# zcablii/SM3Det

Hardware: NVIDIA H100
Metric: backbone images/sec @1024^2 (fwd+bwd) (higher is better)
Workload: dtype f32 (bf16 hi+lo split operands on wgmma, fp32 accumulate; SIMT fp32 elsewhere)

## Files before the change

### include/sm3det_b200.h

```cpp
#ifndef SM3DET_B200_H_
#define SM3DET_B200_H_

#include <stddef.h>
#include <stdint.h>

#ifdef __cplusplus
extern "C" {
#endif

#define SM3_ABI_VERSION 1

#define SM3_OK 0
#define SM3_ERR_INVALID_ARG (-1)
#define SM3_ERR_UNSUPPORTED_SHAPE (-2)
#define SM3_ERR_CUDA (-3)
#define SM3_ERR_WORKSPACE (-4)

int sm3_abi_version(void);
const char* sm3_last_error(void);
int sm3_device_supported(void);

enum { SM3_SCHED_DENSE = 0, SM3_SCHED_GROUPED = 1, SM3_SCHED_SPLITK = 2 };
enum {
  SM3_EPI_BIAS = 1,
  SM3_EPI_GELU = 2,
  SM3_EPI_DGELU = 4,
  SM3_EPI_COLSCALE = 8,
  SM3_EPI_ROWSCALE = 16,
  SM3_EPI_RESID = 32,
  SM3_EPI_ATOMIC = 64,
  SM3_EPI_AUXSTORE = 128,
  SM3_EPI_COLSUM = 256
};
typedef struct sm3_gemm_args {
  const float* A; int64_t a_stride_mn, a_stride_k;
  const float* B; int64_t b_stride_mn, b_stride_k, b_group_stride;
  const int32_t* a_row_index;
  const int32_t* b_k_index;
  const uint16_t* b_packed;
  int64_t b_packed_group_stride;
  const uint16_t* a_packed;
  int32_t M, N, K;
  int32_t tile_n;
  int32_t sched;
  int32_t k_splits, num_groups;
  const int32_t* tile_group;
  const int32_t* num_m_tiles;
  const int32_t* seg_begin;
  const int32_t* seg_end;
  float* D; int64_t ldd, d_group_stride;
  const float* bias; int64_t bias_group_stride;
  int32_t epilogue;
  float* aux_out; const float* aux_in; int64_t ld_aux;
  const float* col_scale; const float* row_scale;
  const float* resid; int64_t ld_resid;
  float* colsum; int64_t colsum_group_stride;
  int32_t mma_passes;
} sm3_gemm_args;
int sm3_gemm(const sm3_gemm_args* args, void* stream);
int64_t sm3_gemm_packed_elems(int32_t N, int32_t K);
int sm3_gemm_pack_b(const float* B, int64_t stride_mn, int64_t stride_k, int64_t group_stride, int32_t groups,
                    int32_t N, int32_t K, uint16_t* out, void* stream);
int64_t sm3_gemm_packed_act_elems(int64_t rows, int32_t cols, int32_t mn_major, int32_t tile);
int sm3_gemm_pack_act(const float* X, int64_t ld, const int32_t* row_index, int64_t rows, int32_t cols,
                      int32_t mn_major, int32_t tile, uint16_t* out, void* stream);
int32_t sm3_gemm_tile_n(int32_t N);
int sm3_gemm_pack_b_tile(const float* B, int64_t stride_mn, int64_t stride_k, int64_t group_stride, int32_t groups,
                         int32_t N, int32_t K, int32_t tile, uint16_t* out, void* stream);
size_t sm3_gemm_workspace_bytes(const sm3_gemm_args* args);

typedef struct sm3_ffn_args {
  const uint16_t* a1; const uint16_t* a2;
  const uint16_t* wa1; const uint16_t* wa2; const uint16_t* wb;
  const float* bias1;
  const float* bias2;
  const float* col_scale;
  const float* row_scale;
  const float* resid;
  float* out;
  float* aux_out;
  float* h_out;
  int32_t M, C, H4, chunk, mma_passes, mode;
  uint16_t* dh_mn; uint16_t* act_mn;
  float* db1;
  const float* h_in;
} sm3_ffn_args;
int32_t sm3_ffn_fused_chunk(int32_t mode, int32_t C);
int sm3_ffn_fused(const sm3_ffn_args* args, void* stream);
size_t sm3_ffn_fused_workspace_bytes(const sm3_ffn_args* args);

enum { SM3_LN_NHWC = 0, SM3_LN_PATCH2 = 1, SM3_LN_NCHW = 2 };
int sm3_layernorm_fwd(const float* x, const float* weight, const float* bias, float* y, float* stats,
                      int64_t tokens, int32_t C, float eps, int32_t out_mode, int32_t H, int32_t W, void* stream);
int sm3_layernorm_fwd_img(const float* x, const float* weight, const float* bias, uint16_t* img, float* y, float* stats,
                          int64_t T, int32_t C, float eps, void* stream);
int sm3_layernorm_bwd(const float* dy, const float* x, const float* stats, const float* weight, float* dx,
                      float* dweight, float* dbias, int64_t tokens, int32_t C, int32_t in_mode, int32_t H,
                      int32_t W, int32_t dx_accumulate, void* stream);

int sm3_stem_fwd(const float* x_nchw, const float* weight_t, const float* bias, const float* ln_weight,
                 const float* ln_bias, float* y, float* conv_out, float* stats, int32_t N, int32_t Cin,
                 int32_t H, int32_t W, int32_t ps, int32_t C0, float eps, void* stream);
int sm3_stem_wgrad(const float* x_nchw, const float* dconv, float* dweight_t, float* dbias, int32_t N,
                   int32_t Cin, int32_t H, int32_t W, int32_t ps, int32_t C0, void* stream);

int sm3_dwconv7_fwd(const float* x, const float* weight_t, const float* bias, const float* resid, float* y,
                    int32_t N, int32_t H, int32_t W, int32_t C, void* stream);
int sm3_dwconv7_wgrad(const float* x, const float* dy, float* dweight_t, float* dbias, int32_t N, int32_t H,
                      int32_t W, int32_t C, void* stream);
int sm3_dwconv7_ln_fwd(const float* x, const float* weight_t, const float* bias, const float* ln_weight,
                       const float* ln_bias, float* u, float* stats, float* v, uint16_t* img, int32_t N, int32_t H,
                       int32_t W, int32_t C, float eps, void* stream);

typedef struct sm3_router_args {
  const float* v; const float* proj_weight; const float* proj_bias; const float* sim_matrix;
  const float* temperature; const float* w_noise; const float* noise;
  int32_t T, C, P, E, k;
  int32_t* top_idx; float* top_gate; float* logits; float* top_vals; float* p_out;
  float* sigma; int32_t* top_idx_m;
  float* partials;
} sm3_router_args;
int sm3_moe_router_blocks(int32_t T);
int sm3_moe_router(const sm3_router_args* args, void* stream);
size_t sm3_moe_router_workspace_bytes(const sm3_router_args* args);

typedef struct sm3_plan_args {
  const float* partials; int32_t T, E, k, max_m_tiles;
  float* importance; float* load; float* loss;
  int32_t* counts; int32_t* seg_begin; int32_t* seg_end; int32_t* cursor;
  int32_t* tile_group; int32_t* num_m_tiles;
} sm3_plan_args;
int sm3_moe_plan(const sm3_plan_args* args, void* stream);
size_t sm3_moe_plan_workspace_bytes(const sm3_plan_args* args);
int sm3_moe_assign(const int32_t* top_idx, int32_t T, int32_t k, int32_t E, const int32_t* seg_begin,
                   int32_t* cursor, int32_t* slot_of, int32_t* pair_token, void* stream);
int sm3_moe_combine(const float* expert_out, const int32_t* slot_of, const int32_t* top_idx, const float* gate,
                    const float* gamma, const float* resid, const float* row_scale, float* out, float* y_opt,
                    int32_t T, int32_t C, int32_t k, void* stream);

typedef struct sm3_act_pack_args {
  const float* h; const float* da; int64_t R; int32_t W; int32_t mode;
  const int32_t* live_tiles; const int32_t* tile_group;
  float* out_f32; uint16_t* pack_k; uint16_t* pack_mn; int32_t mn_tile; float* colsum;
  uint16_t* pack_mn2; int32_t mn_tile2;
} sm3_act_pack_args;
int sm3_act_pack(const sm3_act_pack_args* args, void* stream);

int sm3_moe_combine_bwd(const float* dout, const float* expert_out, const int32_t* slot_of, const int32_t* top_idx,
                        const float* gate, const float* gamma, const float* row_scale, float* d_expert_out,
                        float* dgate, float* dgamma, int32_t T, int32_t C, int32_t k, void* stream);
typedef struct sm3_router_bwd_args {
  const float* p; const float* sim_matrix; const float* temperature;
  const int32_t* top_idx; const float* top_gate; const float* dgate; const float* logits;
  const float* importance; const float* loss_scale;
  int32_t T, P, E, k;
  float* dp; float* dsim_hat; float* dtemperature;
  const float* noise; const float* sigma; const float* top_vals; const int32_t* top_idx_m; const float* load;
  float* dr;
} sm3_router_bwd_args;
int sm3_moe_router_bwd(const sm3_router_bwd_args* args, void* stream);
int sm3_moe_router_bwd_finalize(const float* dsim_hat, const float* sim_matrix, float* dsim, int32_t P, int32_t E,
                                void* stream);
int sm3_colsum(const float* a, const float* b, const float* row_scale, const int32_t* seg_begin,
               const int32_t* seg_end, int32_t groups, float* out, int64_t rows, int32_t C, void* stream);
int sm3_gather_sum(const float* src, const int32_t* slot_of, const float* add, float* out, int32_t T, int32_t C,
                   int32_t k, void* stream);
int sm3_scale_rows(const float* x, const float* row_scale, const float* col_scale, float* out, int64_t rows,
                   int32_t C, void* stream);

int sm3_gather_rows_peer(const float* const* bases, const int32_t* const* token_lists, const int32_t* src_rank,
                         const int32_t* src_row, const float* scale, float* out, int64_t rows, int32_t C, void* stream);

typedef struct sm3_ep_plan_args {
  const int32_t* allm; const int32_t* tile_group_s; const int32_t* num_tiles_s; const int32_t* pair_token;
  int32_t W, me, E, R_s, cap;
  int32_t* src_rank; int32_t* src_slot; int32_t* tile_group; int32_t* num_tiles; int32_t* seg_begin; int32_t* seg_end;
  int32_t* comb_rank; int32_t* comb_row; int32_t* overflow;
} sm3_ep_plan_args;
int sm3_ep_plan(const sm3_ep_plan_args* args, void* stream);

int sm3_dwconv_fwd(const float* x, const float* weight_t, const float* bias, const float* resid, float* y, int32_t N,
                   int32_t H, int32_t W, int32_t C, int32_t ks, int32_t dil, void* stream);
int sm3_dwconv_wgrad(const float* x, const float* dy, float* dweight_t, float* dbias, int32_t N, int32_t H, int32_t W,
                     int32_t C, int32_t ks, int32_t dil, void* stream);
int sm3_colstat(const float* x, const float* sh1, const float* y, const float* sh2, const float* sc2, float* s1, float* s2,
                int64_t rows, int32_t C, void* stream);
int sm3_affine(const float* x1, const float* a1, const float* x2, const float* a2, const float* b, const float* add,
               float* out, int64_t rows, int32_t C, void* stream);
int sm3_mul(const float* a, const float* b, const float* add, float* out, int64_t n, void* stream);
int sm3_dropout(const float* x, float* out, int64_t n, float p, uint64_t seed, void* stream);
int sm3_dropout_dev(const float* x, float* out, int64_t n, float p, const uint64_t* seed_dev, void* stream);
int sm3_mlp_mid_fwd(const float* h, const float* weight_t, const float* bias, const float* mask, float* a, int32_t N,
                    int32_t H, int32_t W, int32_t C, float p, uint64_t seed, const uint64_t* seed_dev, void* stream);
int sm3_mlp_mid_bwd(const float* h, const float* weight_t, const float* bias, const float* da, const float* mask, float* dh,
                    float* dweight_t, float* dbias, int32_t N, int32_t H, int32_t W, int32_t C, float p, uint64_t seed,
                    const uint64_t* seed_dev, void* stream);
int sm3_lsk_agg(const float* a1, const float* a2, float* agg, int32_t* amax, int64_t T, int32_t Ch, void* stream);
int sm3_conv7_c2(const float* x, const float* w, const float* b, float* y, int32_t N, int32_t H, int32_t W, int32_t act,
                 void* stream);
int sm3_conv7_c2_wgrad(const float* x, const float* dpre, float* dw, float* db, int32_t N, int32_t H, int32_t W, void* stream);
int sm3_lsk_mix(const float* a1, const float* a2, const float* sig, float* out, int64_t T, int32_t Ch, void* stream);
int sm3_lsk_mix_bwd_sig(const float* dout, const float* a1, const float* a2, const float* sig, float* dpre, int64_t T,
                        int32_t Ch, void* stream);
int sm3_lsk_mix_bwd_in(const float* dout, const float* sig, const float* dagg, const int32_t* amax, float* da1, float* da2,
                       int64_t T, int32_t Ch, void* stream);
int sm3_im2col(const float* x, float* col, int32_t N, int32_t H, int32_t W, int32_t Cin, int32_t ks, int32_t stride,
               int32_t pad, int32_t Kp, int32_t nchw, void* stream);
int sm3_col2im(const float* dcol, float* dx, int32_t N, int32_t H, int32_t W, int32_t Cin, int32_t ks, int32_t stride,
               int32_t pad, int32_t Kp, int32_t nchw, void* stream);

// ... 11 lines not shown
```

### sm3det_b200/_lib.py

```python
import ctypes as C
import os
import threading

_LIB_PATH = os.path.join(os.path.dirname(os.path.abspath(__file__)), 'lib', 'libsm3det_b200.so')
_lock = threading.Lock()
_lib = None
LAUNCHES = 0

c_f32p = C.c_void_p
c_i32p = C.c_void_p
c_stream = C.c_void_p


class GemmArgs(C.Structure):
    _fields_ = [
        ('A', c_f32p), ('a_stride_mn', C.c_int64), ('a_stride_k', C.c_int64),
        ('B', c_f32p), ('b_stride_mn', C.c_int64), ('b_stride_k', C.c_int64), ('b_group_stride', C.c_int64),
        ('a_row_index', c_i32p), ('b_k_index', c_i32p), ('b_packed', C.c_void_p), ('b_packed_group_stride', C.c_int64), ('a_packed', C.c_void_p),
        ('M', C.c_int32), ('N', C.c_int32), ('K', C.c_int32),
        ('tile_n', C.c_int32), ('sched', C.c_int32), ('k_splits', C.c_int32), ('num_groups', C.c_int32),
        ('tile_group', c_i32p), ('num_m_tiles', c_i32p), ('seg_begin', c_i32p), ('seg_end', c_i32p),
        ('D', c_f32p), ('ldd', C.c_int64), ('d_group_stride', C.c_int64),
        ('bias', c_f32p), ('bias_group_stride', C.c_int64),
        ('epilogue', C.c_int32),
        ('aux_out', c_f32p), ('aux_in', c_f32p), ('ld_aux', C.c_int64),
        ('col_scale', c_f32p), ('row_scale', c_f32p),
        ('resid', c_f32p), ('ld_resid', C.c_int64),
        ('colsum', c_f32p), ('colsum_group_stride', C.c_int64),
        ('mma_passes', C.c_int32),
    ]


class RouterArgs(C.Structure):
    _fields_ = [
        ('v', c_f32p), ('proj_weight', c_f32p), ('proj_bias', c_f32p), ('sim_matrix', c_f32p),
        ('temperature', c_f32p), ('w_noise', c_f32p), ('noise', c_f32p),
        ('T', C.c_int32), ('C', C.c_int32), ('P', C.c_int32), ('E', C.c_int32), ('k', C.c_int32),
        ('top_idx', c_i32p), ('top_gate', c_f32p), ('logits', c_f32p), ('top_vals', c_f32p), ('p_out', c_f32p),
        ('sigma', c_f32p), ('top_idx_m', c_i32p),
        ('partials', c_f32p),
    ]


class PlanArgs(C.Structure):
    _fields_ = [
        ('partials', c_f32p), ('T', C.c_int32), ('E', C.c_int32), ('k', C.c_int32), ('max_m_tiles', C.c_int32),
        ('importance', c_f32p), ('load', c_f32p), ('loss', c_f32p),
        ('counts', c_i32p), ('seg_begin', c_i32p), ('seg_end', c_i32p), ('cursor', c_i32p),
        ('tile_group', c_i32p), ('num_m_tiles', c_i32p),
    ]


class FfnArgs(C.Structure):
    _fields_ = [
        ('a1', C.c_void_p), ('a2', C.c_void_p), ('wa1', C.c_void_p), ('wa2', C.c_void_p), ('wb', C.c_void_p),
        ('bias1', c_f32p), ('bias2', c_f32p), ('col_scale', c_f32p), ('row_scale', c_f32p), ('resid', c_f32p),
        ('out', c_f32p), ('aux_out', c_f32p), ('h_out', c_f32p),
        ('M', C.c_int32), ('C', C.c_int32), ('H4', C.c_int32), ('chunk', C.c_int32), ('mma_passes', C.c_int32),
        ('mode', C.c_int32),
        ('dh_mn', C.c_void_p), ('act_mn', C.c_void_p), ('db1', c_f32p), ('h_in', c_f32p),
    ]


class EpPlanArgs(C.Structure):
    _fields_ = [
        ('allm', c_i32p), ('tile_group_s', c_i32p), ('num_tiles_s', c_i32p), ('pair_token', c_i32p),
        ('W', C.c_int32), ('me', C.c_int32), ('E', C.c_int32), ('R_s', C.c_int32), ('cap', C.c_int32),
        ('src_rank', c_i32p), ('src_slot', c_i32p), ('tile_group', c_i32p), ('num_tiles', c_i32p),
        ('seg_begin', c_i32p), ('seg_end', c_i32p), ('comb_rank', c_i32p), ('comb_row', c_i32p), ('overflow', c_i32p),
    ]


_I32, _I64, _F32, _P = C.c_int32, C.c_int64, C.c_float, C.c_void_p
SIGNATURES = {
    'sm3_abi_version': [],
    'sm3_last_error': [],
    'sm3_device_supported': [],
    'sm3_gemm': [C.POINTER(GemmArgs), _P],
    'sm3_gemm_packed_elems': [_I32, _I32],
    'sm3_gemm_pack_b': [_P, _I64, _I64, _I64, _I32, _I32, _I32, _P, _P],
    'sm3_gemm_packed_act_elems': [_I64, _I32, _I32, _I32],
    'sm3_gemm_pack_act': [_P, _I64, _P, _I64, _I32, _I32, _I32, _P, _P],
    'sm3_gemm_tile_n': [_I32],
    'sm3_gemm_pack_b_tile': [_P, _I64, _I64, _I64, _I32, _I32, _I32, _I32, _P, _P],
    'sm3_gemm_workspace_bytes': [C.POINTER(GemmArgs)],
    'sm3_ffn_fused_chunk': [_I32, _I32],
    'sm3_ffn_fused': [C.POINTER(FfnArgs), _P],
    'sm3_ffn_fused_workspace_bytes': [C.POINTER(FfnArgs)],
    'sm3_moe_router_workspace_bytes': [C.POINTER(RouterArgs)],
    'sm3_moe_plan_workspace_bytes': [C.POINTER(PlanArgs)],
    'sm3_layernorm_fwd': [_P, _P, _P, _P, _P, _I64, _I32, _F32, _I32, _I32, _I32, _P],
    'sm3_layernorm_fwd_img': [_P, _P, _P, _P, _P, _P, _I64, _I32, _F32, _P],
    'sm3_layernorm_bwd': [_P, _P, _P, _P, _P, _P, _P, _I64, _I32, _I32, _I32, _I32, _I32, _P],
    'sm3_stem_fwd': [_P, _P, _P, _P, _P, _P, _P, _P, _I32, _I32, _I32, _I32, _I32, _I32, _F32, _P],
    'sm3_stem_wgrad': [_P, _P, _P, _P, _I32, _I32, _I32, _I32, _I32, _I32, _P],
    'sm3_dwconv7_fwd': [_P, _P, _P, _P, _P, _I32, _I32, _I32, _I32, _P],
    'sm3_dwconv7_wgrad': [_P, _P, _P, _P, _I32, _I32, _I32, _I32, _P],
    'sm3_dwconv7_ln_fwd': [_P, _P, _P, _P, _P, _P, _P, _P, _P, _I32, _I32, _I32, _I32, _F32, _P],
    'sm3_moe_router_bwd_finalize': [_P, _P, _P, _I32, _I32, _P],
    'sm3_moe_router_blocks': [_I32],
    'sm3_moe_router': [C.POINTER(RouterArgs), _P],
    'sm3_moe_plan': [C.POINTER(PlanArgs), _P],
    'sm3_moe_assign': [_P, _I32, _I32, _I32, _P, _P, _P, _P, _P],
    'sm3_moe_combine': [_P, _P, _P, _P, _P, _P, _P, _P, _P, _I32, _I32, _I32, _P],
    'sm3_moe_combine_bwd': [_P, _P, _P, _P, _P, _P, _P, _P, _P, _P, _I32, _I32, _I32, _P],
    'sm3_colsum': [_P, _P, _P, _P, _P, _I32, _P, _I64, _I32, _P],
    'sm3_gather_sum': [_P, _P, _P, _P, _I32, _I32, _I32, _P],
    'sm3_scale_rows': [_P, _P, _P, _P, _I64, _I32, _P],
    'sm3_moe_router_bwd': [_P, _P],
    'sm3_ep_plan': [C.POINTER(EpPlanArgs), _P],
    'sm3_gather_rows_peer': [_P, _P, _P, _P, _P, _P, _I64, _I32, _P],
    'sm3_upsample_add': [_P, _P, _P, _I32, _I32, _I32, _I32, _I32, _I32, _P],
    'sm3_upsample_add_bwd': [_P, _P, _I32, _I32, _I32, _I32, _I32, _I32, _P],
    'sm3_transpose_batched': [_P, _P, _I32, _I32, _I32, _P],
    'sm3_dwconv_fwd': [_P, _P, _P, _P, _P, _I32, _I32, _I32, _I32, _I32, _I32, _P],
    'sm3_dwconv_wgrad': [_P, _P, _P, _P, _I32, _I32, _I32, _I32, _I32, _I32, _P],
    'sm3_colstat': [_P, _P, _P, _P, _P, _P, _P, _I64, _I32, _P],
    'sm3_affine': [_P, _P, _P, _P, _P, _P, _P, _I64, _I32, _P],
    'sm3_mul': [_P, _P, _P, _P, _I64, _P],
    'sm3_dropout': [_P, _P, _I64, _F32, C.c_uint64, _P],
    'sm3_dropout_dev': [_P, _P, _I64, _F32, _P, _P],
    'sm3_mlp_mid_fwd': [_P, _P, _P, _P, _P, _I32, _I32, _I32, _I32, _F32, C.c_uint64, _P, _P],
    'sm3_mlp_mid_bwd': [_P, _P, _P, _P, _P, _P, _P, _P, _I32, _I32, _I32, _I32, _F32, C.c_uint64, _P, _P],
    'sm3_lsk_agg': [_P, _P, _P, _P, _I64, _I32, _P],
    'sm3_conv7_c2': [_P, _P, _P, _P, _I32, _I32, _I32, _I32, _P],
    'sm3_conv7_c2_wgrad': [_P, _P, _P, _P, _I32, _I32, _I32, _P],
    'sm3_lsk_mix': [_P, _P, _P, _P, _I64, _I32, _P],
    'sm3_lsk_mix_bwd_sig': [_P, _P, _P, _P, _P, _I64, _I32, _P],
    'sm3_lsk_mix_bwd_in': [_P, _P, _P, _P, _P, _P, _I64, _I32, _P],
    'sm3_im2col': [_P, _P, _I32, _I32, _I32, _I32, _I32, _I32, _I32, _I32, _I32, _P],
    'sm3_col2im': [_P, _P, _I32, _I32, _I32, _I32, _I32, _I32, _I32, _I32, _I32, _P],
}
_RESTYPES = {'sm3_last_error': C.c_char_p, 'sm3_gemm_packed_elems': C.c_int64, 'sm3_gemm_packed_act_elems': C.c_int64,
             'sm3_gemm_workspace_bytes': C.c_size_t, 'sm3_ffn_fused_workspace_bytes': C.c_size_t,
             'sm3_moe_router_workspace_bytes': C.c_size_t, 'sm3_moe_plan_workspace_bytes': C.c_size_t}


class ActPackArgs(C.Structure):
    _fields_ = [
        ('h', c_f32p), ('da', c_f32p), ('R', C.c_int64), ('W', C.c_int32), ('mode', C.c_int32),
        ('live_tiles', c_i32p), ('tile_group', c_i32p),
        ('out_f32', c_f32p), ('pack_k', C.c_void_p), ('pack_mn', C.c_void_p), ('mn_tile', C.c_int32), ('colsum', c_f32p),
        ('pack_mn2', C.c_void_p), ('mn_tile2', C.c_int32),
    ]


class RouterBwdArgs(C.Structure):
    _fields_ = [
        ('p', c_f32p), ('sim_matrix', c_f32p), ('temperature', c_f32p),
        ('top_idx', c_i32p), ('top_gate', c_f32p), ('dgate', c_f32p), ('logits', c_f32p),
        ('importance', c_f32p), ('loss_scale', c_f32p),
        ('T', C.c_int32), ('P', C.c_int32), ('E', C.c_int32), ('k', C.c_int32),
        ('dp', c_f32p), ('dsim_hat', c_f32p), ('dtemperature', c_f32p),
        ('noise', c_f32p), ('sigma', c_f32p), ('top_vals', c_f32p), ('top_idx_m', c_i32p), ('load', c_f32p),
        ('dr', c_f32p),
    ]


SIGNATURES['sm3_moe_router_bwd'] = [C.POINTER(RouterBwdArgs), _P]
SIGNATURES['sm3_act_pack'] = [C.POINTER(ActPackArgs), _P]


def library_path() -> str:
    return _LIB_PATH


def load():
    global _lib
    if _lib is not None:
        return _lib
    with _lock:
        if _lib is not None:
            return _lib
        if not os.path.isfile(_LIB_PATH):
            raise RuntimeError(
                f'sm3det_b200: CUDA library not built ({_LIB_PATH} missing). Run `make` at the repo root or '
                f'`python -c "import __graft_entry__ as g; g.build()"`. There is no CPU/PyTorch fallback.')
        lib = C.CDLL(_LIB_PATH)
        for name, argtypes in SIGNATURES.items():
            fn = getattr(lib, name)
            fn.argtypes = argtypes
            fn.restype = _RESTYPES.get(name, C.c_int)
# ... 13 lines not shown
```

### sm3det_b200/csrc/capi.cu

```cuda
#include "../../include/sm3det_b200.h"
#include "common.cuh"
#include "gemm_tc.cuh"
#include "kernels.h"
#include "ffn_fused.cuh"

using namespace sm3;

static inline cudaStream_t S(void* s) { return reinterpret_cast<cudaStream_t>(s); }

extern "C" {

int sm3_abi_version(void) { return SM3_ABI_VERSION; }
const char* sm3_last_error(void) { return sm3::last_error(); }

int sm3_device_supported(void) {
  int dev = 0, major = 0, minor = 0;
  if (cudaGetDevice(&dev) != cudaSuccess) return 0;
  if (cudaDeviceGetAttribute(&major, cudaDevAttrComputeCapabilityMajor, dev) != cudaSuccess) return 0;
  if (cudaDeviceGetAttribute(&minor, cudaDevAttrComputeCapabilityMinor, dev) != cudaSuccess) return 0;
  return (major == 9 && minor == 0) ? 1 : 0;
}

int sm3_gemm(const sm3_gemm_args* a, void* stream) {
  if (!a) { set_last_error("sm3_gemm: null args"); return SM3_ERR_INVALID_ARG; }
  gemm::Params p{};
  p.A = a->A; p.a_smn = a->a_stride_mn; p.a_sk = a->a_stride_k;
  p.B = a->B; p.b_smn = a->b_stride_mn; p.b_sk = a->b_stride_k; p.b_group_stride = a->b_group_stride;
  p.a_row_index = a->a_row_index; p.b_k_index = a->b_k_index;
  p.b_packed = a->b_packed; p.b_packed_group_stride = a->b_packed_group_stride; p.a_packed = a->a_packed;
  p.M = a->M; p.N = a->N; p.K = a->K; p.BN = a->tile_n;
  p.sched = a->sched; p.k_splits = a->k_splits; p.num_groups = a->num_groups;
  p.tile_group = a->tile_group; p.num_m_tiles_dev = a->num_m_tiles;
  p.seg_begin = a->seg_begin; p.seg_end = a->seg_end;
  p.D = a->D; p.ldd = a->ldd; p.d_group_stride = a->d_group_stride;
  p.bias = a->bias; p.bias_group_stride = a->bias_group_stride;
  p.epi = a->epilogue;
  p.aux_out = a->aux_out; p.aux_in = a->aux_in; p.ld_aux = a->ld_aux;
  p.col_scale = a->col_scale; p.row_scale = a->row_scale;
  p.resid = a->resid; p.ld_resid = a->ld_resid;
  p.colsum = a->colsum; p.colsum_group_stride = a->colsum_group_stride;
  p.passes = (a->mma_passes == 1) ? 1 : 3;
  return gemm::launch(p, S(stream));
}

int64_t sm3_gemm_packed_elems(int32_t N, int32_t K) { return gemm::packed_elems(N, K); }
int sm3_gemm_pack_b(const float* B, int64_t s_mn, int64_t s_k, int64_t group_stride, int32_t groups, int32_t N, int32_t K,
                    uint16_t* out, void* stream) {
  return gemm::pack_b(B, s_mn, s_k, group_stride, groups, N, K, out, S(stream));
}

int64_t sm3_gemm_packed_act_elems(int64_t rows, int32_t cols, int32_t mn_major, int32_t tile) {
  return gemm::packed_act_elems(rows, cols, mn_major, tile);
}
int sm3_gemm_pack_act(const float* X, int64_t ld, const int32_t* row_index, int64_t rows, int32_t cols, int32_t mn_major,
                      int32_t tile, uint16_t* out, void* stream) {
  return gemm::pack_act(X, ld, row_index, rows, cols, mn_major, tile, out, S(stream));
}
int32_t sm3_gemm_tile_n(int32_t N) { return gemm::pick_bn(N); }
int sm3_gemm_pack_b_tile(const float* B, int64_t s_mn, int64_t s_k, int64_t group_stride, int32_t groups, int32_t N, int32_t K,
                         int32_t tile, uint16_t* out, void* stream) {
  return gemm::pack_b(B, s_mn, s_k, group_stride, groups, N, K, out, S(stream), tile);
}
size_t sm3_gemm_workspace_bytes(const sm3_gemm_args*) { return 0; }

int32_t sm3_ffn_fused_chunk(int32_t mode, int32_t C) { return (mode >= 0 && mode <= 3) ? ffn::chain_chunk(mode, C) : 0; }
size_t sm3_ffn_fused_workspace_bytes(const sm3_ffn_args*) { return 0; }
int sm3_ffn_fused(const sm3_ffn_args* a, void* stream) {
  if (!a) { set_last_error("sm3_ffn_fused: null args"); return SM3_ERR_INVALID_ARG; }
  ffn::ChainParams p{};
  p.a1 = a->a1; p.a2 = a->a2; p.wa1 = a->wa1; p.wa2 = a->wa2; p.wb = a->wb;
  p.bias1 = a->bias1; p.bias2 = a->bias2; p.col_scale = a->col_scale; p.row_scale = a->row_scale; p.resid = a->resid;
  p.out = a->out; p.aux_out = a->aux_out; p.h_out = a->h_out;
  p.dh_mn = a->dh_mn; p.act_mn = a->act_mn; p.db1 = a->db1; p.h_in = a->h_in;
  p.M = a->M; p.C = a->C; p.H4 = a->H4; p.HC = a->chunk; p.passes = a->mma_passes; p.mode = a->mode;
  return ffn::chain(p, S(stream));
}

int sm3_layernorm_fwd(const float* x, const float* w, const float* b, float* y, float* stats, int64_t T, int32_t C,
                      float eps, int32_t out_mode, int32_t H, int32_t W, void* stream) {
  return layernorm_fwd(x, w, b, y, stats, T, C, eps, out_mode, H, W, S(stream));
}
int sm3_layernorm_fwd_img(const float* x, const float* w, const float* b, uint16_t* img, float* y, float* stats, int64_t T,
                          int32_t C, float eps, void* stream) {
  return layernorm_fwd_img(x, w, b, img, y, stats, T, C, eps, S(stream));
}
int sm3_layernorm_bwd(const float* dy, const float* x, const float* stats, const float* w, float* dx, float* dw,
                      float* db, int64_t T, int32_t C, int32_t in_mode, int32_t H, int32_t W, int32_t dx_accum,
                      void* stream) {
  return layernorm_bwd(dy, x, stats, w, dx, dw, db, T, C, in_mode, H, W, dx_accum, S(stream));
}
int sm3_stem_fwd(const float* x, const float* wt, const float* bias, const float* lnw, const float* lnb, float* y,
                 float* conv_out, float* stats, int32_t N, int32_t Cin, int32_t H, int32_t W, int32_t ps, int32_t C0,
                 float eps, void* stream) {
  return stem_fwd(x, wt, bias, lnw, lnb, y, conv_out, stats, N, Cin, H, W, ps, C0, eps, S(stream));
}
int sm3_stem_wgrad(const float* x, const float* du, float* dwt, float* dbias, int32_t N, int32_t Cin, int32_t H,
                   int32_t W, int32_t ps, int32_t C0, void* stream) {
  return stem_wgrad(x, du, dwt, dbias, N, Cin, H, W, ps, C0, S(stream));
}
int sm3_dwconv7_fwd(const float* x, const float* wt, const float* bias, const float* resid, float* y, int32_t N,
                    int32_t H, int32_t W, int32_t C, void* stream) {
  return dwconv7_fwd(x, wt, bias, resid, y, N, H, W, C, S(stream));
}
int sm3_dwconv7_wgrad(const float* x, const float* dy, float* dwt, float* dbias, int32_t N, int32_t H, int32_t W,
                      int32_t C, void* stream) {
  return dwconv7_wgrad(x, dy, dwt, dbias, N, H, W, C, S(stream));
}
int sm3_dwconv7_ln_fwd(const float* x, const float* wt, const float* bias, const float* lnw, const float* lnb, float* u,
                       float* stats, float* v, uint16_t* img, int32_t N, int32_t H, int32_t W, int32_t C, float eps,
                       void* stream) {
  return dwconv7_ln_fwd(x, wt, bias, lnw, lnb, u, stats, v, img, N, H, W, C, eps, S(stream));
}

int sm3_moe_router_blocks(int32_t T) { return router_blocks(T); }
int sm3_moe_router(const sm3_router_args* a, void* stream) {
  if (!a) { set_last_error("sm3_moe_router: null args"); return SM3_ERR_INVALID_ARG; }
  RouterArgs r{};
  r.v = a->v; r.wp = a->proj_weight; r.bp = a->proj_bias; r.sim = a->sim_matrix; r.temperature = a->temperature;
  r.w_noise = a->w_noise; r.noise = a->noise;
  r.T = a->T; r.C = a->C; r.P = a->P; r.E = a->E; r.k = a->k;
  r.top_idx = a->top_idx; r.top_gate = a->top_gate; r.logits = a->logits; r.top_vals = a->top_vals; r.p_out = a->p_out; r.sigma = a->sigma; r.top_idx_m = a->top_idx_m;
  r.partials = a->partials; r.nblocks = router_blocks(a->T);
  return moe_router(r, S(stream));
}
size_t sm3_moe_router_workspace_bytes(const sm3_router_args* a) {
  return a ? (size_t)router_blocks(a->T) * 3u * (size_t)a->E * sizeof(float) : 0;
}
size_t sm3_moe_plan_workspace_bytes(const sm3_plan_args* a) {
  return a ? (size_t)(2 * a->E + 1) * sizeof(float) + (size_t)(4 * a->E + a->max_m_tiles + 1) * sizeof(int32_t) : 0;
}
int sm3_moe_plan(const sm3_plan_args* a, void* stream) {
  if (!a) { set_last_error("sm3_moe_plan: null args"); return SM3_ERR_INVALID_ARG; }
  PlanArgs p{};
  p.partials = a->partials; p.nblocks = router_blocks(a->T);
  p.T = a->T; p.E = a->E; p.k = a->k; p.max_m_tiles = a->max_m_tiles;
  p.importance = a->importance; p.load = a->load; p.loss = a->loss;
  p.counts = a->counts; p.seg_begin = a->seg_begin; p.seg_end = a->seg_end; p.cursor = a->cursor;
  p.tile_group = a->tile_group; p.num_m_tiles = a->num_m_tiles;
  return moe_plan(p, S(stream));
}
int sm3_moe_assign(const int32_t* top_idx, int32_t T, int32_t k, int32_t E, const int32_t* seg_begin, int32_t* cursor,
                   int32_t* slot_of, int32_t* pair_token, void* stream) {
  return moe_assign(top_idx, T, k, E, seg_begin, cursor, slot_of, pair_token, S(stream));
}
int sm3_moe_combine(const float* o, const int32_t* slot_of, const int32_t* top_idx, const float* gate,
                    const float* gamma, const float* resid, const float* row_scale, float* out, float* y_opt,
                    int32_t T, int32_t C, int32_t k, void* stream) {
  return moe_combine(o, slot_of, top_idx, gate, gamma, resid, row_scale, out, y_opt, T, C, k, S(stream));
}

int sm3_act_pack(const sm3_act_pack_args* a, void* stream) {
  if (!a) { set_last_error("sm3_act_pack: null args"); return SM3_ERR_INVALID_ARG; }
  ActPackArgs r{};
  r.h = a->h; r.da = a->da; r.R = a->R; r.W = a->W; r.mode = a->mode; r.live_tiles = a->live_tiles; r.tile_group = a->tile_group;
  r.out_f32 = a->out_f32; r.pack_k = a->pack_k; r.pack_mn = a->pack_mn; r.mn_tile = a->mn_tile; r.colsum = a->colsum;
  r.pack_mn2 = a->pack_mn2; r.mn_tile2 = a->mn_tile2;
  return act_pack(r, S(stream));
}
int sm3_moe_combine_bwd(const float* dout, const float* o, const int32_t* slot_of, const int32_t* top_idx,
                        const float* gate, const float* gamma, const float* row_scale, float* d_o, float* dgate,
                        float* dgamma, int32_t T, int32_t C, int32_t k, void* stream) {
  return moe_combine_bwd(dout, o, slot_of, top_idx, gate, gamma, row_scale, d_o, dgate, dgamma, T, C, k, S(stream));
}
int sm3_moe_router_bwd(const sm3_router_bwd_args* a, void* stream) {
  if (!a) { set_last_error("sm3_moe_router_bwd: null args"); return SM3_ERR_INVALID_ARG; }
  RouterBwdArgs r{};
  r.p = a->p; r.sim = a->sim_matrix; r.temperature = a->temperature; r.top_idx = a->top_idx; r.top_gate = a->top_gate;
  r.dgate = a->dgate; r.logits = a->logits; r.importance = a->importance; r.loss_scale = a->loss_scale;
  r.T = a->T; r.P = a->P; r.E = a->E; r.k = a->k; r.dp = a->dp; r.dsim_hat = a->dsim_hat; r.dtemperature = a->dtemperature;
  r.noise = a->noise; r.sigma = a->sigma; r.top_vals = a->top_vals; r.top_idx_m = a->top_idx_m; r.load = a->load; r.dr = a->dr;
  return moe_router_bwd(r, S(stream));
}
int sm3_moe_router_bwd_finalize(const float* dsim_hat, const float* sim, float* dsim, int32_t P, int32_t E, void* stream) {
  return moe_router_bwd_finalize(dsim_hat, sim, dsim, P, E, S(stream));
}
int sm3_colsum(const float* a, const float* b, const float* rs, const int32_t* seg_begin, const int32_t* seg_end,
               int32_t G, float* out, int64_t rows, int32_t C, void* stream) {
  return colsum(a, b, rs, seg_begin, seg_end, G, out, rows, C, S(stream));
}
int sm3_gather_sum(const float* src, const int32_t* slot_of, const float* add, float* out, int32_t T, int32_t C,
                   int32_t k, void* stream) {
  return gather_sum(src, slot_of, add, out, T, C, k, S(stream));
}
int sm3_scale_rows(const float* x, const float* rs, const float* cs, float* out, int64_t rows, int32_t C, void* stream) {
  return scale_rows(x, rs, cs, out, rows, C, S(stream));
}

int sm3_gather_rows_peer(const float* const* bases, const int32_t* const* token_lists, const int32_t* src_rank,
                         const int32_t* src_row, const float* scale, float* out, int64_t rows, int32_t C, void* stream) {
  return gather_rows_peer(bases, reinterpret_cast<const int* const*>(token_lists), src_rank, src_row, scale, out, rows, C, S(stream));
}
int sm3_dwconv_fwd(const float* x, const float* wt, const float* bias, const float* resid, float* y, int32_t N, int32_t H,
                   int32_t W, int32_t C, int32_t ks, int32_t dil, void* stream) {
// ... 88 lines not shown
```

### sm3det_b200/csrc/ffn_fused.cu

```cuda
#define SM3_GEMM_KERNEL_IMPL
#include "gemm_tc.cuh"
#include "ffn_fused.cuh"
#include "kernels.h"

namespace sm3 {
namespace ffn {
using namespace gemm;

constexpr int THREADS = 384;
constexpr int W_PROD_A = 0, W_PROD_B = 1, EPI0 = 4, NE = 8;
constexpr int CONS_REGS = 232, PROD_REGS = 40;
constexpr uint32_t SMEM_LIMIT = 232448u - 1024u;
constexpr uint32_t STAGING = NE * EPI_STAGE_BYTES;
constexpr uint32_t BARS = 256;

struct Layout {
  uint32_t a, ones, a2, wa, wb, act, act2, stage, cs, bar, total;
  uint32_t a_tile, wa_chunk, wa_stage, wb_stage, act_bytes;
  int sa, sb;
};

struct ChainK { ChainParams p; Layout L; int m_tiles, nch; };

__device__ __forceinline__ void bulk_g2s(uint32_t dst, const void* src, uint32_t bytes, uint32_t bar) {
// ... 48 lines not shown
  auto wa_empty = [&](int s) { return bar + 32u + 8u * s; };
  auto wb_full = [&](int s) { return bar + 48u + 8u * s; };
  auto wb_empty = [&](int s) { return bar + 64u + 8u * s; };
  const int warp = threadIdx.x >> 5, lane = threadIdx.x & 31;
  constexpr int NA = (MODE == 1 || MODE == 2) ? 2 : 1;
  constexpr bool WGRAD_IMG = MODE >= 2;

  if (threadIdx.x == 0) {
    mbar_init(a_full, 1); mbar_init(a_empty, NE);
    for (int s = 0; s < 2; ++s) { mbar_init(wa_full(s), 1); mbar_init(wa_empty(s), NE); mbar_init(wb_full(s), 1); mbar_init(wb_empty(s), NE); }
    asm volatile("fence.mbarrier_init.release.cluster;" ::: "memory");
  }
  __syncthreads();
  const int nch = k.nch;
  constexpr int kbc = C / 32;

  if (warp < EPI0) {
    asm volatile("setmaxnreg.dec.sync.aligned.u32 %0;" ::"n"(PROD_REGS));
    if (warp == W_PROD_A && lane == 0) {
      uint32_t n_t = 0, n_w = 0;
      for (int t = blockIdx.x; t < k.m_tiles; t += gridDim.x, ++n_t) {
        mbar_wait(a_empty, (n_t & 1u) ^ 1u);
        if ((p.debug & 8) && n_t > 0) { mbar_arrive(a_full); goto weights; }
        expect_tx(a_full, NA * L.a_tile);
        bulk_g2s(sb0 + L.a, reinterpret_cast<const uint8_t*>(MODE == 3 ? p.a2 : p.a1) + (long long)t * L.a_tile, L.a_tile, a_full);
        if (NA == 2) bulk_g2s(sb0 + L.a + L.a_tile, reinterpret_cast<const uint8_t*>(p.a2) + (long long)t * L.a_tile, L.a_tile, a_full);
      weights:
        for (int j = 0; j < nch; ++j, ++n_w) {
          const int s = n_w % L.sa;
          mbar_wait(wa_empty(s), ((n_w / L.sa) & 1u) ^ 1u);
          if ((p.debug & 4) && n_w >= (uint32_t)L.sa) { mbar_arrive(wa_full(s)); continue; }
          expect_tx(wa_full(s), L.wa_stage);
          const uint32_t dst = sb0 + L.wa + s * L.wa_stage;
          bulk_g2s(dst, reinterpret_cast<const uint8_t*>(MODE == 3 ? p.wa2 : p.wa1) + (long long)j * L.wa_chunk, L.wa_chunk, wa_full(s));
          if (NA == 2) bulk_g2s(dst + L.wa_chunk, reinterpret_cast<const uint8_t*>(p.wa2) + (long long)j * L.wa_chunk, L.wa_chunk, wa_full(s));
        }
      }
    } else if (warp == W_PROD_B && lane == 0) {
      uint32_t n = 0;
      for (int t = blockIdx.x; t < k.m_tiles; t += gridDim.x) {
        for (int j = 0; j < nch; ++j, ++n) {
          const int s = n % L.sb;
          mbar_wait(wb_empty(s), ((n / L.sb) & 1u) ^ 1u);
          if ((p.debug & 4) && n >= (uint32_t)L.sb) { mbar_arrive(wb_full(s)); continue; }
          expect_tx(wb_full(s), L.wb_stage);
          bulk_g2s(sb0 + L.wb + s * L.wb_stage, reinterpret_cast<const uint8_t*>(p.wb) + (long long)j * L.wb_stage, L.wb_stage, wb_full(s));
        }
      }
    }
  } else {
    asm volatile("setmaxnreg.inc.sync.aligned.u32 %0;" ::"n"(CONS_REGS));
    const int e = warp - EPI0, g = e >> 2, wq = warp & 3;
    const uint32_t slab = (uint32_t)g * WG_A_BYTES;
    const uint32_t stage_base = sb0 + L.stage + (uint32_t)e * EPI_STAGE_BYTES;
    const int rl = lane >> 2, c4 = (lane & 3) * 4;
    const int r_lo = g * 64 + wq * 16 + rl;
    auto wg_bar = [&]() { asm volatile("bar.sync %0, 128;" ::"r"(1 + g) : "memory"); };
    float acc_h[HC / 2], acc_d[HC / 2], acc_o[C / 2];
    uint32_t n_c = 0, n_b = 0, n_t = 0;
    auto gemm_a = [&](uint32_t nc) {
      const int s = nc % L.sa;
      mbar_wait(wa_full(s), (nc / L.sa) & 1u);
      const uint32_t wst = sb0 + L.wa + s * L.wa_stage;
#pragma unroll
      for (int q = 0; q < NA; ++q) {
        uint64_t da = make_smem_desc(sb0 + L.a + q * L.a_tile + slab, false), db = make_smem_desc(wst + q * L.wa_chunk, false);
        for (int kb = 0; kb < kbc; ++kb) {
          if (q == 0 && MODE != 3) {
            mma3<HC>(acc_h, da, da + 512u, db, db + HC * 4u, kb > 0 ? 1u : 0u, p.passes);
            mma3<HC>(acc_h, da + 2u, da + 514u, db + 2u, db + HC * 4u + 2u, 1u, p.passes);
          } else {
            mma3<HC>(acc_d, da, da + 512u, db, db + HC * 4u, kb > 0 ? 1u : 0u, p.passes);
            mma3<HC>(acc_d, da + 2u, da + 514u, db + 2u, db + HC * 4u + 2u, 1u, p.passes);
          }
          da += 1024u; db += HC * 8u;
        }
      }
    };
    const uint32_t cs_base = sb0 + L.cs;
    auto cons_bar = [&]() { asm volatile("bar.sync 3, 256;" ::: "memory"); };
    if constexpr (WGRAD_IMG) {
      for (int i = threadIdx.x - EPI0 * 32; i < p.H4; i += 256) asm volatile("st.shared.f32 [%0], %1;" ::"r"(cs_base + 4u * i), "f"(0.f) : "memory");
      cons_bar();
    }
    const long long R_pad = ((long long)p.M + 31) / 32 * 32;
    for (int t = blockIdx.x; t < k.m_tiles; t += gridDim.x, ++n_t) {
      mbar_wait(a_full, n_t & 1u);
      wg::fence();
      gemm_a(n_c);
      wg::commit();
      for (int j = 0; j < nch; ++j, ++n_c) {
        if constexpr (MODE == 3) {
#pragma unroll
          for (int q = 0; q < HC / 8; ++q)
#pragma unroll
            for (int h = 0; h < 2; ++h) {
              const long long row = (long long)t * 128 + r_lo + 8 * h;
              const float2 x = row < p.M ? __ldg(reinterpret_cast<const float2*>(p.h_in + row * p.H4 + (long long)j * HC + 8 * q + 2 * (lane & 3)))
                                         : make_float2(0.f, 0.f);
              acc_h[4 * q + 2 * h] = x.x; acc_h[4 * q + 2 * h + 1] = x.y;
            }
        }
        wg::wait<0>();
        if constexpr (MODE != 3) wg::fence_operand(acc_h);
        if constexpr (MODE != 0) wg::fence_operand(acc_d);
        __syncwarp();
        if (lane == 0) {
          mbar_arrive(wa_empty(n_c % L.sa));
          if (j > 0) mbar_arrive(wb_empty((n_b - 1) % L.sb));
          if (j == nch - 1) mbar_arrive(a_empty);
        }
        const float* b1 = p.bias1 + (long long)j * HC;
        if constexpr (WGRAD_IMG) {
          const long long wrow0 = (long long)t * 128 + g * 64 + wq * 16;
#pragma unroll
          for (int qp = 0; qp < HC / 16; ++qp) {
            float cs4[4];
#pragma unroll
            for (int qq = 0; qq < 2; ++qq) {
              const int q = 2 * qp + qq;
              const int kk = 8 * q + 2 * (lane & 3);
              const float2 bv = MODE == 3 ? make_float2(0.f, 0.f) : __ldg(reinterpret_cast<const float2*>(b1 + kk));
              cs4[2 * qq] = 0.f; cs4[2 * qq + 1] = 0.f;
#pragma unroll
              for (int h = 0; h < 2; ++h) {
                const int r = r_lo + 8 * h;
                float y[2], a[2];
#pragma unroll
                for (int e = 0; e < 2; ++e) {
                  const float x = MODE == 3 ? acc_h[4 * q + 2 * h + e] : acc_h[4 * q + 2 * h + e] + (e ? bv.y : bv.x);
                  float Phi, ex;
                  phi_parts(x, Phi, ex);
                  a[e] = x * Phi;
                  y[e] = acc_d[4 * q + 2 * h + e] * fmaf(x * 0.39894228040143267794f, ex, Phi);
                }
                if (wrow0 + rl + 8 * h < p.M) { cs4[2 * qq] += y[0]; cs4[2 * qq + 1] += y[1]; }
                uint32_t hi, lo;
                split2(y[0], y[1], hi, lo);
                const uint32_t o = sb0 + L.act + (uint32_t)(kk >> 5) * 16384u + kmajor_sw64_offset((uint32_t)r, (uint32_t)((kk & 31) >> 3)) +
                                   (uint32_t)(kk & 7) * 2u;
                asm volatile("st.shared.b32 [%0], %1;" ::"r"(o), "r"(hi) : "memory");
                asm volatile("st.shared.b32 [%0], %1;" ::"r"(o + 8192u), "r"(lo) : "memory");
                const uint32_t so = stage_base + (uint32_t)((rl + 8 * h) * EPI_STAGE_ROW_FLOATS + 8 * qq + 2 * (lane & 3)) * 4u;
                asm volatile("st.shared.v2.f32 [%0], {%1, %2};" ::"r"(so), "f"(y[0]), "f"(y[1]) : "memory");
                asm volatile("st.shared.v2.f32 [%0], {%1, %2};" ::"r"(so + 16u * EPI_STAGE_ROW_FLOATS * 4u), "f"(a[0]), "f"(a[1]) : "memory");
              }
            }
            const float csum = colsum16(cs4, lane);
            const int col = j * HC + 16 * qp;
            if ((lane & 4) == 0)
              asm volatile("red.shared.add.f32 [%0], %1;" ::"r"(cs_base + 4u * (uint32_t)(col + 8 * ((lane >> 4) & 1) + 2 * (lane & 3) + ((lane >> 3) & 1))),
                           "f"(csum) : "memory");
            __syncwarp();
            const int sr = lane >> 1, sc = 8 * (lane & 1);
            const long long row = wrow0 + sr;
            if (row < R_pad) {
              float dv8[8], av8[8];
              float4 x0, x1, z0, z1;
              const uint32_t ro = stage_base + (uint32_t)(sr * EPI_STAGE_ROW_FLOATS + sc) * 4u;
              asm volatile("ld.shared.v4.f32 {%0, %1, %2, %3}, [%4];" : "=f"(x0.x), "=f"(x0.y), "=f"(x0.z), "=f"(x0.w) : "r"(ro) : "memory");
              asm volatile("ld.shared.v4.f32 {%0, %1, %2, %3}, [%4];" : "=f"(x1.x), "=f"(x1.y), "=f"(x1.z), "=f"(x1.w) : "r"(ro + 16u) : "memory");
              asm volatile("ld.shared.v4.f32 {%0, %1, %2, %3}, [%4];" : "=f"(z0.x), "=f"(z0.y), "=f"(z0.z), "=f"(z0.w)
                           : "r"(ro + 16u * EPI_STAGE_ROW_FLOATS * 4u) : "memory");
              asm volatile("ld.shared.v4.f32 {%0, %1, %2, %3}, [%4];" : "=f"(z1.x), "=f"(z1.y), "=f"(z1.z), "=f"(z1.w)
                           : "r"(ro + 16u * EPI_STAGE_ROW_FLOATS * 4u + 16u) : "memory");
              const bool live = row < p.M;
              dv8[0] = x0.x; dv8[1] = x0.y; dv8[2] = x0.z; dv8[3] = x0.w; dv8[4] = x1.x; dv8[5] = x1.y; dv8[6] = x1.z; dv8[7] = x1.w;
              av8[0] = z0.x; av8[1] = z0.y; av8[2] = z0.z; av8[3] = z0.w; av8[4] = z1.x; av8[5] = z1.y; av8[6] = z1.z; av8[7] = z1.w;
              uint32_t dh_[4], dl_[4], ah_[4], al_[4];
#pragma unroll
              for (int e = 0; e < 4; ++e) {
                split2(live ? dv8[2 * e] : 0.f, live ? dv8[2 * e + 1] : 0.f, dh_[e], dl_[e]);
                split2(live ? av8[2 * e] : 0.f, live ? av8[2 * e + 1] : 0.f, ah_[e], al_[e]);
              }
              constexpr uint32_t PB = 8192u;
              const int n = col + sc;
              const long long blk = ((long long)(n >> 7) * (R_pad >> 5) + (row >> 5)) * (2LL * PB);
              const uint32_t o = mnmajor_sw128_offset((uint32_t)(row & 31), (uint32_t)((n & 127) >> 3));
              uint8_t* dimg = reinterpret_cast<uint8_t*>(p.dh_mn) + blk + o;
              uint8_t* aimg = reinterpret_cast<uint8_t*>(p.act_mn) + blk + o;
              *reinterpret_cast<uint4*>(dimg) = make_uint4(dh_[0], dh_[1], dh_[2], dh_[3]);
              *reinterpret_cast<uint4*>(dimg + PB) = make_uint4(dl_[0], dl_[1], dl_[2], dl_[3]);
              *reinterpret_cast<uint4*>(aimg) = make_uint4(ah_[0], ah_[1], ah_[2], ah_[3]);
              *reinterpret_cast<uint4*>(aimg + PB) = make_uint4(al_[0], al_[1], al_[2], al_[3]);
            }
            __syncwarp();
          }
        } else {
#pragma unroll
          for (int q = 0; q < HC / 8; ++q) {
            const int kk = 8 * q + 2 * (lane & 3);
            const float2 bv = __ldg(reinterpret_cast<const float2*>(b1 + kk));
#pragma unroll
            for (int h = 0; h < 2; ++h) {
              const int r = r_lo + 8 * h;
              const float x0 = acc_h[4 * q + 2 * h] + bv.x, x1 = acc_h[4 * q + 2 * h + 1] + bv.y;
              if (MODE == 0 && p.h_out) {
                const long long row = (long long)t * 128 + r;
                if (row < p.M) *reinterpret_cast<float2*>(p.h_out + row * p.H4 + (long long)j * HC + kk) = make_float2(x0, x1);
              }
              float y0, y1;
              if (p.debug & 1) { y0 = x0; y1 = x1; }
              else if constexpr (MODE == 0) { y0 = gelu_fast(x0); y1 = gelu_fast(x1); }
              else { y0 = acc_d[4 * q + 2 * h] * gelu_grad_fast(x0); y1 = acc_d[4 * q + 2 * h + 1] * gelu_grad_fast(x1); }
              if (p.debug & 2) continue;
              uint32_t hi, lo;
              split2(y0, y1, hi, lo);
              const uint32_t o = sb0 + L.act + (uint32_t)(kk >> 5) * 16384u + kmajor_sw64_offset((uint32_t)r, (uint32_t)((kk & 31) >> 3)) +
                                 (uint32_t)(kk & 7) * 2u;
              asm volatile("st.shared.b32 [%0], %1;" ::"r"(o), "r"(hi) : "memory");
              asm volatile("st.shared.b32 [%0], %1;" ::"r"(o + 8192u), "r"(lo) : "memory");
            }
          }
        }
        fence_proxy_async_smem();
        wg_bar();
        const int s = n_b % L.sb;
        mbar_wait(wb_full(s), (n_b / L.sb) & 1u);
        wg::fence();
        {
          uint64_t da = make_smem_desc(sb0 + L.act + slab, false), db = make_smem_desc(sb0 + L.wb + s * L.wb_stage, false);
          const uint64_t blo = (uint64_t)(C * 4);
#pragma unroll
          for (int kb = 0; kb < HC / 32; ++kb) {
            mma3<C>(acc_o, da, da + 512u, db, db + blo, (j > 0 || kb > 0) ? 1u : 0u, p.passes);
            mma3<C>(acc_o, da + 2u, da + 514u, db + 2u, db + blo + 2u, 1u, p.passes);
            da += 1024u; db += 2u * blo;
          }
        }
        ++n_b;
        if (j + 1 < nch) gemm_a(n_c + 1);
        wg::commit();
      }
      wg::wait<0>();
      wg::fence_operand(acc_o);
      __syncwarp();
      if (lane == 0) mbar_arrive(wb_empty((n_b - 1) % L.sb));
      const long long row0 = (long long)t * 128 + g * 64 + wq * 16;
#pragma unroll
      for (int c = 0; c < C / 16; ++c) {
        const int n = c * 16 + c4;
        float4 rr[2];
#pragma unroll
        for (int it = 0; it < 2; ++it) {
          const long long row = row0 + it * 8 + rl;
          rr[it] = (p.resid && row < p.M) ? ldg_f4(p.resid + row * C + n) : make_float4(0.f, 0.f, 0.f, 0.f);
        }
        __syncwarp();
#pragma unroll
        for (int qq = 0; qq < 2; ++qq)
#pragma unroll
          for (int h = 0; h < 2; ++h)
            asm volatile("st.shared.v2.f32 [%0], {%1, %2};"
                         ::"r"(stage_base + (uint32_t)((rl + 8 * h) * EPI_STAGE_ROW_FLOATS + 8 * qq + 2 * (lane & 3)) * 4u),
                           "f"(acc_o[8 * c + 4 * qq + 2 * h]), "f"(acc_o[8 * c + 4 * qq + 2 * h + 1]) : "memory");
        __syncwarp();
        float4 bv = make_float4(0.f, 0.f, 0.f, 0.f), sv = make_float4(1.f, 1.f, 1.f, 1.f);
        if (p.bias2) bv = ldg_f4(p.bias2 + n);
        if (p.col_scale) sv = ldg_f4(p.col_scale + n);
#pragma unroll
        for (int it = 0; it < 2; ++it) {
          const int rr_ = it * 8 + rl;
          const long long row = row0 + rr_;
          if (row >= p.M) continue;
          float4 x;
          asm volatile("ld.shared.v4.f32 {%0, %1, %2, %3}, [%4];" : "=f"(x.x), "=f"(x.y), "=f"(x.z), "=f"(x.w)
                       : "r"(stage_base + (uint32_t)(rr_ * EPI_STAGE_ROW_FLOATS + c4) * 4u) : "memory");
          x.x += bv.x; x.y += bv.y; x.z += bv.z; x.w += bv.w;
          if (p.aux_out) *reinterpret_cast<float4*>(p.aux_out + row * C + n) = x;
          x.x *= sv.x; x.y *= sv.y; x.z *= sv.z; x.w *= sv.w;
          if (p.row_scale) { const float rs = __ldg(p.row_scale + row); x.x *= rs; x.y *= rs; x.z *= rs; x.w *= rs; }
          x.x += rr[it].x; x.y += rr[it].y; x.z += rr[it].z; x.w += rr[it].w;
          *reinterpret_cast<float4*>(p.out + row * C + n) = x;
        }
      }
    }
    if constexpr (WGRAD_IMG) {
      cons_bar();
      for (int i = threadIdx.x - EPI0 * 32; i < p.H4; i += 256) {
        float v;
        asm volatile("ld.shared.f32 %0, [%1];" : "=f"(v) : "r"(cs_base + 4u * i) : "memory");
        atomicAdd(p.db1 + i, v);
      }
    }
  }
}

static bool chain_layout(int mode, int C, int HC, int sa, int sb, Layout& L) {
  const uint32_t nA = (mode == 1 || mode == 2) ? 2 : 1;
  L.a_tile = (uint32_t)(C / 32) * 16384u;
  L.wa_chunk = (uint32_t)(C / 32) * HC * 128u;
  L.wa_stage = nA * L.wa_chunk;
  L.wb_stage = (uint32_t)(HC / 32) * C * 128u;
  L.act_bytes = (uint32_t)(HC / 32) * 16384u;
  L.sa = sa; L.sb = sb;
  uint32_t o = 0;
  L.a = o; o += nA * L.a_tile;
  L.ones = 0; L.a2 = L.a + L.a_tile;
  L.wa = o; o += sa * L.wa_stage;
  L.wb = o; o += sb * L.wb_stage;
  L.act = o; o += L.act_bytes;
  L.act2 = 0;
  L.stage = o; o += STAGING;
  L.cs = o; o += mode >= 2 ? (uint32_t)(4 * C) * 4u : 0u;
  L.bar = o; o += BARS;
  L.total = o + 1024u;
  return L.total <= SMEM_LIMIT + 1024u;
}

static bool pick_chain(int mode, int C, int HC_req, int& HC, Layout& L) {
  static const int cand[][3] = {{64, 2, 2}, {32, 2, 2}, {64, 2, 1}, {32, 2, 1}, {32, 1, 1}};
  if (C % 32 != 0 || C < 32 || C > 256) return false;
  if ((mode == 2 && C > 128) || (mode == 3 && C != 192)) return false;
  for (auto& c : cand)
    if ((HC_req == 0 || c[0] == HC_req) && chain_layout(mode, C, c[0], c[1], c[2], L)) { HC = c[0]; return true; }
  return false;
}

int chain_chunk(int mode, int C) {
  int HC = 0; Layout L;
  return pick_chain(mode, C, 0, HC, L) ? HC : 0;
}

static bool aligned16(const void* q) { return (reinterpret_cast<uintptr_t>(q) & 15u) == 0; }

int chain(const ChainParams& p, cudaStream_t stream) {
  SM3_REQUIRE(p.mode >= 0 && p.mode <= 3, SM3_ERR_INVALID_ARG, "ffn chain: mode");
  SM3_REQUIRE((p.mode == 3 || (p.a1 && p.wa1)) && p.wb && p.bias1 && p.out && (p.mode == 0 || (p.a2 && p.wa2)), SM3_ERR_INVALID_ARG,
              "ffn chain: null operand");
  SM3_REQUIRE(p.mode < 2 || (p.dh_mn && p.act_mn && p.db1 && (p.mode == 2 || p.h_in)), SM3_ERR_INVALID_ARG,
              "ffn chain: modes 2 / 3 need dh_mn, act_mn, db1 (and h_in in mode 3)");
  SM3_REQUIRE(p.M > 0 && p.H4 > 0 && p.C > 0, SM3_ERR_INVALID_ARG, "ffn chain: bad shape");
  ChainK k{};
  k.p = p;
  int HC = 0;
  SM3_REQUIRE(p.HC == 32 || p.HC == 64, SM3_ERR_INVALID_ARG, "ffn chain: chunk must be 32 or 64 (sm3_ffn_fused_chunk), got %d", p.HC);
  SM3_REQUIRE(pick_chain(p.mode, p.C, p.HC, HC, k.L), SM3_ERR_UNSUPPORTED_SHAPE, "ffn chain: C=%d with chunk %d does not fit shared memory (mode %d)", p.C, p.HC, p.mode);
  SM3_REQUIRE(p.H4 % HC == 0 && p.C % 16 == 0, SM3_ERR_UNSUPPORTED_SHAPE, "ffn chain: H4=%d not a multiple of the chunk %d", p.H4, HC);
// ... 43 lines not shown
```

### sm3det_b200/csrc/gemm_tc.cu

```cuda
#define SM3_GEMM_KERNEL_IMPL
#include "gemm_tc.cuh"
#include <mutex>

namespace sm3 {
const char* last_error();
namespace gemm {

int pick_bn(int N) {
  static const int cand[] = {128, 96, 64, 32};
  for (int bn : cand)
    if (N % bn == 0) return bn;
  if (N <= 0 || N % 8) return 0;
  int best = 0, best_tiles = 0;
  for (int bn : cand) {
    const int tiles = (N + bn - 1) / bn;
    if (!best || tiles < best_tiles || (tiles == best_tiles && tiles * bn < best_tiles * best)) { best = bn; best_tiles = tiles; }
  }
  return best;
}

static bool aligned16(const void* p) { return (reinterpret_cast<uintptr_t>(p) & 15u) == 0; }

long long packed_elems(int N, int K) {
  const long long kblocks = (K + BK - 1) / BK;
// ... 4 lines not shown

__global__ void __launch_bounds__(256) pack_b_kernel(const float* __restrict__ B, long long s_mn, long long s_k,
                                                    long long group_stride, int N, int rows, int K, int BN,
                                                    uint16_t* __restrict__ out, long long out_group_stride,
                                                    long long chunks_per_group) {
  const long long i = (long long)blockIdx.x * blockDim.x + threadIdx.x;
  if (i >= chunks_per_group) return;
  const int g = blockIdx.y;
  const int kblocks = (K + BK - 1) / BK;
  const int n = (int)(i % rows);
  const long long r = i / rows;
  const int c = (int)(r % 4), kb = (int)(r / 4);
  const bool live = n < N;
  const float* src = B + (long long)g * group_stride + (long long)n * s_mn;
  uint32_t hi[4], lo[4];
#pragma unroll
  for (int e = 0; e < 8; e += 2) {
    float v[2];
#pragma unroll
    for (int q = 0; q < 2; ++q) {
      const int k = kb * BK + c * 8 + e + q;
      v[q] = (live && k < K) ? __ldg(src + (long long)k * s_k) : 0.f;
    }
    const uint32_t u0 = __float_as_uint(v[0]), u1 = __float_as_uint(v[1]);
    hi[e / 2] = __byte_perm(u0, u1, 0x7632);
    const uint32_t r0 = __float_as_uint(v[0] - __uint_as_float(u0 & 0xFFFF0000u)) + 0x8000u;
    const uint32_t r1 = __float_as_uint(v[1] - __uint_as_float(u1 & 0xFFFF0000u)) + 0x8000u;
    lo[e / 2] = __byte_perm(r0, r1, 0x7632);
  }
  const int nt = n / BN, row = n % BN;
  uint8_t* tile = reinterpret_cast<uint8_t*>(out + (long long)g * out_group_stride) +
                  ((long long)nt * kblocks + kb) * ((long long)BN * 128);
  const uint32_t o = kmajor_sw64_offset((uint32_t)row, (uint32_t)c);
  *reinterpret_cast<uint4*>(tile + o) = make_uint4(hi[0], hi[1], hi[2], hi[3]);
  *reinterpret_cast<uint4*>(tile + (long long)BN * 64 + o) = make_uint4(lo[0], lo[1], lo[2], lo[3]);
}

int pack_b(const float* B, long long s_mn, long long s_k, long long group_stride, int groups, int N, int K,
           uint16_t* out, cudaStream_t stream, int tile) {
  SM3_REQUIRE(B && out && N > 0 && K > 0 && groups >= 1, SM3_ERR_INVALID_ARG, "gemm pack: bad argument");
  const int BN = tile > 0 ? tile : pick_bn(N);
  SM3_REQUIRE(BN > 0 && BN % 8 == 0 && BN <= 256 && (tile > 0 ? N % BN == 0 : N % 8 == 0), SM3_ERR_UNSUPPORTED_SHAPE,
              "gemm pack: N=%d has no tile width (tile=%d)", N, tile);
  SM3_REQUIRE((reinterpret_cast<uintptr_t>(out) & 15u) == 0, SM3_ERR_INVALID_ARG, "gemm pack: output must be 16B aligned");
  const long long kblocks = (K + BK - 1) / BK;
  const int rows = (N + BN - 1) / BN * BN;
  const long long chunks = (long long)rows * kblocks * 4;
  dim3 grid((unsigned)((chunks + 255) / 256), (unsigned)groups);
  pack_b_kernel<<<grid, 256, 0, stream>>>(B, s_mn, s_k, group_stride, N, rows, K, BN, out, packed_elems(N, K), chunks);
  return check_launch("pack_b_kernel");
}

long long packed_act_elems(long long rows, int cols, int mn_major, int tile) {
  if (!mn_major) {
    const long long rt = (rows + tile - 1) / tile, kb = (cols + BK - 1) / BK;
    return rt * kb * 2 * (long long)tile * BK;
  }
  const long long ct = (cols + tile - 1) / tile, kb = (rows + BK - 1) / BK;
  return ct * kb * 2 * (long long)(plane_bytes(tile, true) / 2);
}

__global__ void __launch_bounds__(256) pack_act_k_kernel(const float* __restrict__ X, long long ld, const int* __restrict__ row_index,
                                                        long long rows, int K, int tile, uint16_t* __restrict__ out,
                                                        long long chunks) {
  const long long i = (long long)blockIdx.x * blockDim.x + threadIdx.x;
  if (i >= chunks) return;
  const int kblocks = (K + BK - 1) / BK;
  const int cpr = kblocks * 4;
  const long long row = i / cpr;
  const int cc = (int)(i % cpr), kb = cc >> 2, c = cc & 3;
  long long src_row = row < rows ? row : -1;
  if (src_row >= 0 && row_index) src_row = __ldg(row_index + row);
  float v[8];
#pragma unroll
  for (int e = 0; e < 8; ++e) v[e] = 0.f;
  if (src_row >= 0) {
    const int k = kb * BK + c * 8;
    const float* src = X + src_row * ld + k;
    if (k + 8 <= K) { const float4 a = ldg_f4(src), b = ldg_f4(src + 4); v[0] = a.x; v[1] = a.y; v[2] = a.z; v[3] = a.w; v[4] = b.x; v[5] = b.y; v[6] = b.z; v[7] = b.w; }
    else { for (int e = 0; e < 8; ++e) if (k + e < K) v[e] = __ldg(src + e); }
  }
  uint32_t hi[4], lo[4];
#pragma unroll
  for (int e = 0; e < 8; e += 2) {
    const uint32_t u0 = __float_as_uint(v[e]), u1 = __float_as_uint(v[e + 1]);
    hi[e / 2] = __byte_perm(u0, u1, 0x7632);
    const uint32_t r0 = __float_as_uint(v[e] - __uint_as_float(u0 & 0xFFFF0000u)) + 0x8000u;
    const uint32_t r1 = __float_as_uint(v[e + 1] - __uint_as_float(u1 & 0xFFFF0000u)) + 0x8000u;
    lo[e / 2] = __byte_perm(r0, r1, 0x7632);
  }
  const long long rt = row / tile; const int rr = (int)(row % tile);
  uint8_t* img = reinterpret_cast<uint8_t*>(out) + (rt * kblocks + kb) * ((long long)tile * 128);
  const uint32_t o = kmajor_sw64_offset((uint32_t)rr, (uint32_t)c);
  *reinterpret_cast<uint4*>(img + o) = make_uint4(hi[0], hi[1], hi[2], hi[3]);
  *reinterpret_cast<uint4*>(img + (long long)tile * 64 + o) = make_uint4(lo[0], lo[1], lo[2], lo[3]);
}

__global__ void __launch_bounds__(256) pack_act_mn_kernel(const float* __restrict__ X, long long ld, const int* __restrict__ row_index,
                                                         long long rows, int W, int tile, uint16_t* __restrict__ out,
                                                         long long chunks, long long rows_pad) {
  const long long i = (long long)blockIdx.x * blockDim.x + threadIdx.x;
  if (i >= chunks) return;
  const int ct = (W + tile - 1) / tile;
  const int cpr = ct * (tile / 8);
  const long long r = i / cpr;
  const int cc = (int)(i % cpr);
  const int mt = cc / (tile / 8), mc = cc % (tile / 8);
  const int col = mt * tile + mc * 8;
  long long src_row = r < rows ? r : -1;
  if (src_row >= 0 && row_index) src_row = __ldg(row_index + r);
  float4 a = make_float4(0.f, 0.f, 0.f, 0.f), b = a;
  if (src_row >= 0 && col + 8 <= W) { const float* src = X + src_row * ld + col; a = ldg_f4(src); b = ldg_f4(src + 4); }
  const float v[8] = {a.x, a.y, a.z, a.w, b.x, b.y, b.z, b.w};
  uint32_t hi[4], lo[4];
#pragma unroll
  for (int e = 0; e < 8; e += 2) {
    const uint32_t u0 = __float_as_uint(v[e]), u1 = __float_as_uint(v[e + 1]);
    hi[e / 2] = __byte_perm(u0, u1, 0x7632);
    const uint32_t r0 = __float_as_uint(v[e] - __uint_as_float(u0 & 0xFFFF0000u)) + 0x8000u;
    const uint32_t r1 = __float_as_uint(v[e + 1] - __uint_as_float(u1 & 0xFFFF0000u)) + 0x8000u;
    lo[e / 2] = __byte_perm(r0, r1, 0x7632);
  }
  const long long kblocks = rows_pad / BK;
  const long long kb = r / BK; const uint32_t k = (uint32_t)(r % BK);
  const uint32_t pb = plane_bytes(tile, true);
  uint8_t* img = reinterpret_cast<uint8_t*>(out) + ((long long)mt * kblocks + kb) * (2LL * pb);
  const uint32_t o = mnmajor_sw128_offset(k, (uint32_t)mc);
  *reinterpret_cast<uint4*>(img + o) = make_uint4(hi[0], hi[1], hi[2], hi[3]);
  *reinterpret_cast<uint4*>(img + pb + o) = make_uint4(lo[0], lo[1], lo[2], lo[3]);
}

int pack_act(const float* X, long long ld, const int* row_index, long long rows, int cols, int mn_major, int tile,
             uint16_t* out, cudaStream_t stream) {
  SM3_REQUIRE(X && out && rows > 0 && cols > 0, SM3_ERR_INVALID_ARG, "gemm pack_act: bad argument");
  SM3_REQUIRE(tile >= 32 && tile <= 256 && tile % 32 == 0, SM3_ERR_INVALID_ARG, "gemm pack_act: tile=%d", tile);
  SM3_REQUIRE(aligned16(X) && aligned16(out) && ld % 4 == 0 && cols % 4 == 0, SM3_ERR_INVALID_ARG, "gemm pack_act: alignment");
  if (!mn_major) {
    const long long rt = (rows + tile - 1) / tile, kb = (cols + BK - 1) / BK;
    const long long chunks = rt * tile * kb * 4;
    pack_act_k_kernel<<<(unsigned)((chunks + 255) / 256), 256, 0, stream>>>(X, ld, row_index, rows, cols, tile, out, chunks);
  } else {
    SM3_REQUIRE(cols % 8 == 0, SM3_ERR_UNSUPPORTED_SHAPE, "gemm pack_act: MN-major needs cols%%8==0");
    const long long rows_pad = (rows + BK - 1) / BK * BK;
    const long long ct = (cols + tile - 1) / tile;
    const long long chunks = rows_pad * ct * (tile / 8);
    pack_act_mn_kernel<<<(unsigned)((chunks + 255) / 256), 256, 0, stream>>>(X, ld, row_index, rows, cols, tile, out, chunks, rows_pad);
  }
  return check_launch("pack_act");
}

int launch(Params p, cudaStream_t stream) {
  if (p.b_packed && !p.B) p.B = reinterpret_cast<const float*>(p.b_packed);
  if (p.a_packed && !p.A) p.A = reinterpret_cast<const float*>(p.a_packed);
  SM3_REQUIRE(p.A && p.B && p.D, SM3_ERR_INVALID_ARG, "gemm: null operand");
  SM3_REQUIRE(p.M > 0 && p.N > 0 && p.K >= 0, SM3_ERR_INVALID_ARG, "gemm: bad shape %d %d %d", p.M, p.N, p.K);
  SM3_REQUIRE((p.a_smn == 1) != (p.a_sk == 1) || (p.a_smn == 1 && p.M == 1), SM3_ERR_INVALID_ARG,
              "gemm: A needs exactly one unit stride");
  const bool packed = p.b_packed != nullptr;
  const bool apacked = p.a_packed != nullptr;
  if (packed && !apacked) { p.b_smn = p.K; p.b_sk = 1; }
  if (apacked) {
    const bool amn = (p.a_smn == 1 && p.a_sk != 1);
    if (amn) { p.b_smn = 1; p.b_sk = p.N; } else { p.b_smn = p.K; p.b_sk = 1; }
  }
  SM3_REQUIRE((p.b_smn == 1) != (p.b_sk == 1), SM3_ERR_INVALID_ARG, "gemm: B needs exactly one unit stride");
  const bool a_mn = (p.a_smn == 1 && p.a_sk != 1), b_mn = (p.b_smn == 1 && p.b_sk != 1);
  if (p.BN == 0) p.BN = pick_bn(p.N);
  SM3_REQUIRE(p.BN >= 32 && p.BN <= MAX_BN && p.BN % 32 == 0 && p.N % 8 == 0, SM3_ERR_UNSUPPORTED_SHAPE,
              "gemm: N=%d has no tile width (N a multiple of 8, tile width a multiple of 32 <= 128)", p.N);
  SM3_REQUIRE(aligned16(p.A) && aligned16(p.B) && aligned16(p.D), SM3_ERR_INVALID_ARG, "gemm: pointers must be 16B aligned");
  if (!a_mn) SM3_REQUIRE(p.a_smn % 4 == 0 && p.K % 4 == 0, SM3_ERR_UNSUPPORTED_SHAPE, "gemm: K-major A needs K%%4==0, lda%%4==0");
  else       SM3_REQUIRE(p.a_sk % 4 == 0 && p.M % 8 == 0, SM3_ERR_UNSUPPORTED_SHAPE, "gemm: MN-major A needs M%%8==0, lda%%4==0");
  if (!b_mn) SM3_REQUIRE(p.b_smn % 4 == 0 && p.K % 4 == 0, SM3_ERR_UNSUPPORTED_SHAPE, "gemm: K-major B needs K%%4==0, ldb%%4==0");
  else       SM3_REQUIRE(p.b_sk % 4 == 0, SM3_ERR_UNSUPPORTED_SHAPE, "gemm: MN-major B needs ldb%%4==0");
  SM3_REQUIRE(!(p.a_row_index && a_mn), SM3_ERR_INVALID_ARG, "gemm: row gather needs K-major A");
  SM3_REQUIRE(!(p.b_k_index && !b_mn), SM3_ERR_INVALID_ARG, "gemm: k gather needs MN-major B");
  SM3_REQUIRE(p.ldd % 4 == 0, SM3_ERR_UNSUPPORTED_SHAPE, "gemm: ldd%%4");
  if (p.epi & (EPI_GELU | EPI_AUXSTORE)) SM3_REQUIRE(!p.aux_out || (aligned16(p.aux_out) && p.ld_aux % 4 == 0), SM3_ERR_INVALID_ARG, "gemm: aux_out");
  if (p.epi & EPI_DGELU) SM3_REQUIRE(p.aux_in && aligned16(p.aux_in) && p.ld_aux % 4 == 0, SM3_ERR_INVALID_ARG, "gemm: aux_in");
  if (p.epi & EPI_BIAS) SM3_REQUIRE(p.bias && aligned16(p.bias) && p.bias_group_stride % 4 == 0, SM3_ERR_INVALID_ARG, "gemm: bias");
  if (p.epi & EPI_COLSCALE) SM3_REQUIRE(p.col_scale && aligned16(p.col_scale), SM3_ERR_INVALID_ARG, "gemm: col_scale");
  if (p.epi & EPI_ROWSCALE) SM3_REQUIRE(p.row_scale, SM3_ERR_INVALID_ARG, "gemm: row_scale");
  if (p.epi & EPI_COLSUM) SM3_REQUIRE(p.colsum && aligned16(p.colsum) && p.colsum_group_stride % 4 == 0, SM3_ERR_INVALID_ARG, "gemm: colsum");
  if (p.epi & EPI_RESID) SM3_REQUIRE(p.resid && aligned16(p.resid) && p.ld_resid % 4 == 0, SM3_ERR_INVALID_ARG, "gemm: resid");

  p.n_tiles = (p.N + p.BN - 1) / p.BN;
  p.m_tiles = (p.M + BM - 1) / BM;
  if (p.sched == SCHED_DENSE) {
    p.k_splits = 1; p.num_groups = 1;
    p.num_tiles = p.m_tiles * p.n_tiles;
  } else if (p.sched == SCHED_GROUPED) {
    SM3_REQUIRE(p.tile_group && p.num_m_tiles_dev, SM3_ERR_INVALID_ARG, "gemm: grouped schedule needs tile map");
    p.k_splits = 1;
    p.num_tiles = p.m_tiles * p.n_tiles;
  } else if (p.sched == SCHED_SPLITK) {
    SM3_REQUIRE(p.k_splits >= 1 && p.num_groups >= 1, SM3_ERR_INVALID_ARG, "gemm: split-K needs k_splits/num_groups");
    SM3_REQUIRE((p.epi & EPI_ATOMIC) || p.k_splits == 1, SM3_ERR_INVALID_ARG, "gemm: split-K>1 needs EPI_ATOMIC");
    p.num_tiles = p.num_groups * p.m_tiles * p.n_tiles * p.k_splits;
  } else {
    SM3_REQUIRE(false, SM3_ERR_INVALID_ARG, "gemm: bad schedule %d", p.sched);
  }
  {
    const long long a_ext = apacked ? 0 : a_mn ? (long long)p.K * p.a_sk : (long long)(p.a_row_index ? (1LL << 31) / (p.a_smn ? p.a_smn : 1) : p.M) * p.a_smn;
    const long long b_ext = packed ? 0 : b_mn ? (long long)(p.b_k_index ? 1 : p.K) * p.b_sk + p.N : (long long)p.N * p.b_smn;
    SM3_REQUIRE(a_ext < (1LL << 32) && b_ext < (1LL << 32), SM3_ERR_UNSUPPORTED_SHAPE, "gemm: operand larger than 2^32 elements");
  }
  p.nstages = STAGES; p.stage_bytes = STAGE_BYTES;
  if (apacked) {
    const unsigned sb = (16384u + 2u * plane_bytes(p.BN, b_mn) + 1023u) & ~1023u;
    int ns = (int)((unsigned)(STAGES * STAGE_BYTES) / sb);
    if (ns > MAX_STAGES) ns = MAX_STAGES;
    if (ns >= STAGES) { p.nstages = ns; p.stage_bytes = sb; }
  }
  int grid = persistent_grid_sms();
  if (grid > p.num_tiles) grid = p.num_tiles;
  if (grid < 1) grid = 1;
#define SM3_GEMM_LAUNCH_E(AMN, BMN, BPK, APK, EPIT)                                                                             \
  do {                                                                                                                          \
    cudaFuncSetAttribute(gemm_bf16x3_kernel<AMN, BMN, BPK, APK, EPIT>, cudaFuncAttributeMaxDynamicSharedMemorySize, (int)SMEM_BYTES); \
    gemm_bf16x3_kernel<AMN, BMN, BPK, APK, EPIT><<<grid, NUM_THREADS, SMEM_BYTES, stream>>>(p);                                     \
  } while (0)
#define SM3_GEMM_LAUNCH(AMN, BMN, BPK, APK) SM3_GEMM_LAUNCH_E(AMN, BMN, BPK, APK, -1)
  if (apacked) {
    SM3_REQUIRE(packed && a_mn == b_mn && p.BN == pick_bn(p.N) && !p.a_row_index && !p.b_k_index, SM3_ERR_INVALID_ARG,
                "gemm: packed A needs packed B of the same majorness (gathers are applied by the pack kernels)");
    SM3_REQUIRE(aligned16(p.a_packed) && aligned16(p.b_packed) && (p.b_packed_group_stride % 8) == 0, SM3_ERR_INVALID_ARG,
                "gemm: packed operands must be 16B aligned");
    constexpr int E_FFN2_TRAIN = EPI_BIAS | EPI_COLSCALE | EPI_RESID | EPI_AUXSTORE, E_FFN2_EVAL = EPI_BIAS | EPI_COLSCALE | EPI_RESID;
    if (a_mn) {
      if (p.epi == EPI_ATOMIC) SM3_GEMM_LAUNCH_E(true, true, true, true, EPI_ATOMIC);
      else if (p.epi == (EPI_ATOMIC | EPI_ROWSCALE)) SM3_GEMM_LAUNCH_E(true, true, true, true, EPI_ATOMIC | EPI_ROWSCALE);
      else SM3_GEMM_LAUNCH(true, true, true, true);
    } else {
      if (p.epi == 0) SM3_GEMM_LAUNCH_E(false, false, true, true, 0);
      else if (p.epi == EPI_BIAS) SM3_GEMM_LAUNCH_E(false, false, true, true, EPI_BIAS);
      else if (p.epi == E_FFN2_TRAIN) SM3_GEMM_LAUNCH_E(false, false, true, true, E_FFN2_TRAIN);
      else if (p.epi == E_FFN2_EVAL) SM3_GEMM_LAUNCH_E(false, false, true, true, E_FFN2_EVAL);
      else SM3_GEMM_LAUNCH(false, false, true, true);
    }
  }
  else if (packed) {
    SM3_REQUIRE(!a_mn && p.sched != SCHED_SPLITK && p.BN == pick_bn(p.N), SM3_ERR_INVALID_ARG,
                "gemm: packed B needs K-major A, a dense/grouped schedule and the default tile width");
    SM3_REQUIRE((reinterpret_cast<uintptr_t>(p.b_packed) & 15u) == 0 && (p.b_packed_group_stride % 8) == 0,
                SM3_ERR_INVALID_ARG, "gemm: packed B must be 16B aligned");
    SM3_GEMM_LAUNCH(false, false, true, false);
  }
  else if (!a_mn && !b_mn) SM3_GEMM_LAUNCH(false, false, false, false);
  else if (!a_mn && b_mn) SM3_GEMM_LAUNCH(false, true, false, false);
  else if (a_mn && b_mn) SM3_GEMM_LAUNCH(true, true, false, false);
  else SM3_REQUIRE(false, SM3_ERR_UNSUPPORTED_SHAPE, "gemm: MN-major A with K-major B is not instantiated");
#undef SM3_GEMM_LAUNCH_E
#undef SM3_GEMM_LAUNCH
  return check_launch("gemm_bf16x3_kernel");
}

}
}
```

### sm3det_b200/csrc/gemm_tc.cuh

```cuda
#pragma once
#include <type_traits>
#include "common.cuh"

namespace sm3 {
namespace gemm {

constexpr int BM = 128;
constexpr int BK = 32;
constexpr int MAX_BN = 128;
constexpr int STAGES = 6;
constexpr int NUM_CONS_WARPS = 8;
constexpr int NUM_PROD_WARPS = 8;
constexpr int FIRST_PROD_WARP = 8;
constexpr int NUM_THREADS = (NUM_CONS_WARPS + NUM_PROD_WARPS) * 32;
constexpr int CONS_REGS = 144, PROD_REGS = 112;
constexpr int MAX_UNITS = 4;

constexpr uint32_t OFF_A_HI = 0;
constexpr uint32_t OFF_A_LO = 8192;
constexpr uint32_t OFF_B_HI = 16384;
constexpr uint32_t OFF_B_LO = 24576;
constexpr uint32_t STAGE_BYTES = 32768;
constexpr uint32_t WG_A_BYTES = 4096;
constexpr int MAX_STAGES = 8;
constexpr uint32_t BAR_BYTES = 256;
constexpr int EPI_CW = 16;
constexpr uint32_t EPI_STAGE_ROW_FLOATS = EPI_CW + 4;
constexpr uint32_t EPI_STAGE_BYTES = 32 * EPI_STAGE_ROW_FLOATS * 4;
constexpr int MAX_EPI_WARPS = 8;
constexpr int COLSUM_SMEM_COLS = 3072;
constexpr uint32_t SMEM_BYTES = STAGES * STAGE_BYTES + BAR_BYTES + MAX_EPI_WARPS * EPI_STAGE_BYTES + COLSUM_SMEM_COLS * 4 + 1024;

enum Sched : int { SCHED_DENSE = 0, SCHED_GROUPED = 1, SCHED_SPLITK = 2 };

enum Epi : int {
  EPI_BIAS = 1,
  EPI_GELU = 2,
  EPI_DGELU = 4,
  EPI_COLSCALE = 8,
  EPI_ROWSCALE = 16,
  EPI_RESID = 32,
  EPI_ATOMIC = 64,
  EPI_AUXSTORE = 128,
  EPI_COLSUM = 256,
};

struct Params {
  const float* A; long long a_smn, a_sk;
  const float* B; long long b_smn, b_sk; long long b_group_stride;
  const int* a_row_index;
  const int* b_k_index;
  const uint16_t* b_packed; long long b_packed_group_stride;
  const uint16_t* a_packed;
  int M, N, K, BN;
  int sched;
  int num_tiles;
  int m_tiles, n_tiles, k_splits, num_groups;
  const int* tile_group;
  const int* num_m_tiles_dev;
  const int* seg_begin;
  const int* seg_end;
  float* D; long long ldd; long long d_group_stride;
  const float* bias; long long bias_group_stride;
  int epi;
  float* aux_out; const float* aux_in; long long ld_aux;
  const float* col_scale; const float* row_scale;
  const float* resid; long long ld_resid;
  float* colsum; long long colsum_group_stride;
  int passes;
  int nstages; unsigned stage_bytes;
  int debug;
};

__host__ __device__ inline uint32_t kmajor_sw64_offset(uint32_t row, uint32_t chunk) {
  return (row >> 3) * 512u + (row & 7u) * 64u + ((chunk ^ ((row >> 1) & 3u)) << 4);
}
__host__ __device__ inline uint32_t mnmajor_sw128_offset(uint32_t k, uint32_t mn_chunk ) {
  const uint32_t g = mn_chunk >> 3, cc = mn_chunk & 7u;
  return (g * 4u + (k >> 3)) * 1024u + (k & 7u) * 128u + ((cc ^ (k & 7u)) << 4);
}
constexpr uint32_t MN_LBO_BYTES = 4096;
constexpr uint32_t MN_SBO_BYTES = 1024;
constexpr uint32_t K_SBO_BYTES = 512;
__host__ __device__ inline uint32_t plane_bytes(int width, bool mn_major) {
  return mn_major ? (uint32_t)((width + 63) / 64) * 4096u : (uint32_t)width * 64u;
}

__host__ __device__ inline uint64_t make_smem_desc(uint32_t smem_addr, bool mn_major) {
  uint64_t d = 0;
  d |= (uint64_t)((smem_addr >> 4) & 0x3FFFu);
  if (mn_major) {
    d |= (uint64_t)((MN_LBO_BYTES >> 4) & 0x3FFFu) << 16;
    d |= (uint64_t)((MN_SBO_BYTES >> 4) & 0x3FFFu) << 32;
    d |= (uint64_t)1 << 62;
  } else {
    d |= (uint64_t)1 << 16;
    d |= (uint64_t)((K_SBO_BYTES >> 4) & 0x3FFFu) << 32;
    d |= (uint64_t)2 << 62;
  }
  return d;
}
#if defined(__CUDACC__) && defined(SM3_GEMM_KERNEL_IMPL)
}
}
#include "wgmma.cuh"
namespace sm3 {
namespace gemm {
__device__ __forceinline__ uint32_t smem_u32(const void* p) {
  return static_cast<uint32_t>(__cvta_generic_to_shared(p));
}
__device__ __forceinline__ void mbar_init(uint32_t bar, uint32_t count) {
  asm volatile("mbarrier.init.shared::cta.b64 [%0], %1;" ::"r"(bar), "r"(count) : "memory");
}
__device__ __forceinline__ void mbar_arrive(uint32_t bar) {
  asm volatile("mbarrier.arrive.shared::cta.b64 _, [%0];" ::"r"(bar) : "memory");
}
__device__ __forceinline__ bool mbar_try_wait(uint32_t bar, uint32_t parity) {
  uint32_t ok;
  asm volatile(
      "{\n\t.reg .pred p;\n\t"
      "mbarrier.try_wait.parity.shared::cta.b64 p, [%1], %2;\n\t"
      "selp.u32 %0, 1, 0, p;\n\t}"
      : "=r"(ok) : "r"(bar), "r"(parity) : "memory");
  return ok != 0;
}
__device__ __forceinline__ void mbar_wait(uint32_t bar, uint32_t parity) {
  if (mbar_try_wait(bar, parity)) return;
  const long long t0 = clock64();
  while (!mbar_try_wait(bar, parity)) {
    if (clock64() - t0 > 20000000000LL) __trap();
  }
}
__device__ __forceinline__ void fence_proxy_async_smem() {
  asm volatile("fence.proxy.async.shared::cta;" ::: "memory");
}
struct Tile {
  int m0, n0, group, k_begin, k_end;
  __device__ __forceinline__ int nkb() const { return (k_end - k_begin + BK - 1) / BK; }
};

__device__ __forceinline__ int total_tiles(const Params& p) {
  if (p.sched == SCHED_GROUPED) return __ldg(p.num_m_tiles_dev) * p.n_tiles;
  return p.num_tiles;
}

__device__ __forceinline__ Tile decode_tile(const Params& p, int t) {
  Tile tl;
  if (p.sched == SCHED_SPLITK) {
    const int s = t % p.k_splits;
    int rest = t / p.k_splits;
    const int nt = rest % p.n_tiles; rest /= p.n_tiles;
    const int mt = rest % p.m_tiles;
    tl.group = rest / p.m_tiles;
    tl.m0 = mt * BM; tl.n0 = nt * p.BN;
    int b = 0, e = p.K;
    if (p.seg_begin) { b = __ldg(p.seg_begin + tl.group); e = __ldg(p.seg_end + tl.group); }
    int len = e - b; if (len < 0) len = 0;
    int chunk = (len + p.k_splits - 1) / p.k_splits;
    chunk = (chunk + BK - 1) / BK * BK;
    tl.k_begin = b + s * chunk;
    tl.k_end = min(e, tl.k_begin + chunk);
    if (tl.k_end < tl.k_begin) tl.k_end = tl.k_begin;
  } else {
    const int mt = t / p.n_tiles, nt = t % p.n_tiles;
    tl.m0 = mt * BM; tl.n0 = nt * p.BN;
    tl.group = (p.sched == SCHED_GROUPED) ? __ldg(p.tile_group + mt) : 0;
    tl.k_begin = 0; tl.k_end = p.K;
  }
  return tl;
}

__device__ __forceinline__ void split4(const float4& x, uint32_t& h01, uint32_t& h23, uint32_t& l01,
                                       uint32_t& l23) {
  const uint32_t u0 = __float_as_uint(x.x), u1 = __float_as_uint(x.y);
  const uint32_t u2 = __float_as_uint(x.z), u3 = __float_as_uint(x.w);
  h01 = __byte_perm(u0, u1, 0x7632);
  h23 = __byte_perm(u2, u3, 0x7632);
  const uint32_t r0 = __float_as_uint(x.x - __uint_as_float(u0 & 0xFFFF0000u)) + 0x8000u;
  const uint32_t r1 = __float_as_uint(x.y - __uint_as_float(u1 & 0xFFFF0000u)) + 0x8000u;
  const uint32_t r2 = __float_as_uint(x.z - __uint_as_float(u2 & 0xFFFF0000u)) + 0x8000u;
  const uint32_t r3 = __float_as_uint(x.w - __uint_as_float(u3 & 0xFFFF0000u)) + 0x8000u;
  l01 = __byte_perm(r0, r1, 0x7632);
  l23 = __byte_perm(r2, r3, 0x7632);
}

template <bool A_MN, bool B_MN, bool B_PACKED, bool A_PACKED, int EPI_T>
__global__ void __launch_bounds__(NUM_THREADS, 1) gemm_bf16x3_kernel(const __grid_constant__ Params p) {
  const int EPI = (EPI_T >= 0) ? EPI_T : p.epi;
  extern __shared__ uint8_t smem_raw[];
  const uint32_t smem_base = (smem_u32(smem_raw) + 1023u) & ~1023u;
  const uint32_t bar_base = smem_base + STAGES * STAGE_BYTES;
  auto full_bar = [&](int s) { return bar_base + 8u * s; };
  auto empty_bar = [&](int s) { return bar_base + 64u + 8u * s; };
  const int NST = p.nstages;
  const uint32_t STB = p.stage_bytes;

  const int warp = threadIdx.x >> 5, lane = threadIdx.x & 31;

  if (threadIdx.x == 0) {
    for (int s = 0; s < NST; ++s) { mbar_init(full_bar(s), A_PACKED ? 1 : NUM_PROD_WARPS + (B_PACKED ? 1 : 0)); mbar_init(empty_bar(s), NUM_CONS_WARPS); }
    asm volatile("fence.mbarrier_init.release.cluster;" ::: "memory");
  }
  __syncthreads();

  const int ntiles = total_tiles(p);

  if (warp < NUM_CONS_WARPS) {
    asm volatile("setmaxnreg.inc.sync.aligned.u32 %0;" ::"n"(CONS_REGS));
    constexpr int NE = NUM_CONS_WARPS;
    const int wg = warp >> 2;
    const int nchunks = p.BN / EPI_CW;
    const uint32_t stage_base = bar_base + BAR_BYTES + (uint32_t)warp * EPI_STAGE_BYTES;
    const int rl = lane >> 2, c4 = (lane & 3) * 4;
    const uint32_t cs_base = bar_base + BAR_BYTES + MAX_EPI_WARPS * EPI_STAGE_BYTES;
    const bool cs_smem = (EPI & EPI_COLSUM) && p.N <= COLSUM_SMEM_COLS;
    int cs_group = -1;
    const int e_tid = warp * 32 + lane;
    auto epi_bar = []() { asm volatile("bar.sync 1, %0;" ::"n"(NE * 32) : "memory"); };
    auto cs_flush = [&](int group) {
      epi_bar();
      if (group >= 0) {
        float* cd = p.colsum + (long long)group * p.colsum_group_stride;
        for (int n = e_tid; n < p.N; n += NE * 32) {
          float sv;
          asm volatile("ld.shared.f32 %0, [%1];" : "=f"(sv) : "r"(cs_base + 4u * n) : "memory");
          if (sv != 0.f) atomicAdd(cd + n, sv);
        }
      }
      for (int n = e_tid; n < p.N; n += NE * 32)
        asm volatile("st.shared.f32 [%0], %1;" ::"r"(cs_base + 4u * n), "f"(0.f) : "memory");
      epi_bar();
    };
    if (cs_smem) cs_flush(-1);
    int stage = 0; uint32_t phase = 0;
    constexpr uint32_t a_kstep = A_MN ? 2u * MN_SBO_BYTES : 32u;
    constexpr uint32_t b_kstep = B_MN ? 2u * MN_SBO_BYTES : 32u;
    const uint32_t b_lo_off = B_PACKED ? OFF_B_HI + plane_bytes(p.BN, B_MN) : OFF_B_LO;
    float acc[MAX_BN / 2];
    for (int t = blockIdx.x; t < ntiles; t += gridDim.x) {
      const Tile tl = decode_tile(p, t);
      const int nkb = tl.nkb();
      if (nkb == 0) continue;
      if (cs_smem && tl.group != cs_group) { if (cs_group >= 0) cs_flush(cs_group); cs_group = tl.group; }
      const int row0 = tl.m0 + wg * 64 + (warp & 3) * 16;
      float4 rr[2], rn[2];
      auto load_resid = [&](int c_, float4 (&dst)[2]) {
        const int n_ = tl.n0 + c_ * EPI_CW + c4;
#pragma unroll
        for (int it = 0; it < 2; ++it) {
          const int row = row0 + it * 8 + rl;
          dst[it] = (row < p.M && n_ < p.N) ? ldg_f4(p.resid + (long long)row * p.ld_resid + n_) : make_float4(0.f, 0.f, 0.f, 0.f);
        }
      };
      if (EPI & EPI_RESID) load_resid(0, rr);

      int prev = -1;
      auto mainloop = [&](auto bn_c) {
        constexpr int N = decltype(bn_c)::value;
        for (int kb = 0; kb < nkb; ++kb) {
          mbar_wait(full_bar(stage), phase);
          wg::fence();
          const uint32_t sb = smem_base + stage * STB + (uint32_t)wg * WG_A_BYTES;
          const uint32_t sbb = smem_base + stage * STB;
#pragma unroll
          for (int j = 0; j < BK / 16; ++j) {
            const uint64_t ahi = make_smem_desc(sb + OFF_A_HI + j * a_kstep, A_MN);
            const uint64_t alo = make_smem_desc(sb + OFF_A_LO + j * a_kstep, A_MN);
            const uint64_t bhi = make_smem_desc(sbb + OFF_B_HI + j * b_kstep, B_MN);
            const uint64_t blo = make_smem_desc(sbb + b_lo_off + j * b_kstep, B_MN);
            if (!(p.debug & 4)) {
              const uint32_t accum = (kb > 0 || j > 0) ? 1u : 0u;
              if (p.passes == 1) {
                wg::mma<N, A_MN, B_MN>(acc, ahi, bhi, accum);
              } else {
                wg::mma<N, A_MN, B_MN>(acc, alo, bhi, accum);
                wg::mma<N, A_MN, B_MN>(acc, ahi, blo, 1u);
                wg::mma<N, A_MN, B_MN>(acc, ahi, bhi, 1u);
              }
            }
          }
          wg::commit();
          if (prev >= 0) {
            wg::wait<1>();
            __syncwarp();
            if (lane == 0) mbar_arrive(empty_bar(prev));
          }
          prev = stage;
          if (++stage == NST) { stage = 0; phase ^= 1u; }
        }
      };
      switch (p.BN) {
        case 32: mainloop(std::integral_constant<int, 32>{}); break;
        case 64: mainloop(std::integral_constant<int, 64>{}); break;
        case 96: mainloop(std::integral_constant<int, 96>{}); break;
        default: mainloop(std::integral_constant<int, 128>{}); break;
      }
      wg::wait<0>();
      wg::fence_operand(acc);
      __syncwarp();
      if (lane == 0) mbar_arrive(empty_bar(prev));
      if (p.debug & 4) {
#pragma unroll
        for (int i = 0; i < MAX_BN / 2; ++i) acc[i] = 0.f;
      }

      float* dbase = p.D + (long long)tl.group * p.d_group_stride;
      const float* bias = p.bias ? p.bias + (long long)tl.group * p.bias_group_stride : nullptr;
#pragma unroll
      for (int c = 0; c < MAX_BN / EPI_CW; ++c) {
        if (c >= nchunks) break;
        __syncwarp();
#pragma unroll
        for (int qq = 0; qq < 2; ++qq)
#pragma unroll
          for (int h = 0; h < 2; ++h)
            asm volatile("st.shared.v2.f32 [%0], {%1, %2};"
                         ::"r"(stage_base + (uint32_t)((rl + 8 * h) * EPI_STAGE_ROW_FLOATS + 8 * qq + 2 * (lane & 3)) * 4u),
                           "f"(acc[8 * c + 4 * qq + 2 * h]), "f"(acc[8 * c + 4 * qq + 2 * h + 1]) : "memory");
        if ((EPI & EPI_RESID) && c + 1 < nchunks) load_resid(c + 1, rn);
        __syncwarp();
        const int n = tl.n0 + c * EPI_CW + c4;
        const bool n_ok = n < p.N;
        float4 bv = make_float4(0.f, 0.f, 0.f, 0.f), sv = make_float4(1.f, 1.f, 1.f, 1.f);
        if ((EPI & EPI_BIAS) && n_ok) bv = ldg_f4(bias + n);
        if ((EPI & EPI_COLSCALE) && n_ok) sv = ldg_f4(p.col_scale + n);
        float4 cs = make_float4(0.f, 0.f, 0.f, 0.f);
#pragma unroll
        for (int it = 0; it < 2; ++it) {
          const int r = it * 8 + rl;
          const int row = row0 + r;
          if (row >= p.M || !n_ok) continue;
          float4 x;
          asm volatile("ld.shared.v4.f32 {%0, %1, %2, %3}, [%4];"
                       : "=f"(x.x), "=f"(x.y), "=f"(x.z), "=f"(x.w)
                       : "r"(stage_base + (uint32_t)(r * EPI_STAGE_ROW_FLOATS + c4) * 4u) : "memory");
          x.x += bv.x; x.y += bv.y; x.z += bv.z; x.w += bv.w;
          if ((EPI & (EPI_AUXSTORE | EPI_GELU)) && p.aux_out)
            *reinterpret_cast<float4*>(p.aux_out + (long long)row * p.ld_aux + n) = x;
          if (EPI & EPI_GELU) { x.x = gelu_fast(x.x); x.y = gelu_fast(x.y); x.z = gelu_fast(x.z); x.w = gelu_fast(x.w); }
          if (EPI & EPI_DGELU) {
            const float4 h = ldg_f4(p.aux_in + (long long)row * p.ld_aux + n);
            x.x *= gelu_grad_fast(h.x); x.y *= gelu_grad_fast(h.y); x.z *= gelu_grad_fast(h.z); x.w *= gelu_grad_fast(h.w);
          }
          x.x *= sv.x; x.y *= sv.y; x.z *= sv.z; x.w *= sv.w;
          if (EPI & EPI_ROWSCALE) { const float rs = __ldg(p.row_scale + row); x.x *= rs; x.y *= rs; x.z *= rs; x.w *= rs; }
          if (EPI & EPI_RESID) { x.x += rr[it].x; x.y += rr[it].y; x.z += rr[it].z; x.w += rr[it].w; }
          cs.x += x.x; cs.y += x.y; cs.z += x.z; cs.w += x.w;
          float* dst = dbase + (long long)row * p.ldd + n;
          if (EPI & EPI_ATOMIC) {
            asm volatile("red.global.add.v4.f32 [%0], {%1, %2, %3, %4};" ::"l"(dst), "f"(x.x), "f"(x.y), "f"(x.z), "f"(x.w) : "memory");
          } else {
            *reinterpret_cast<float4*>(dst) = x;
          }
        }
        if (EPI & EPI_RESID) {
#pragma unroll
          for (int it = 0; it < 2; ++it) rr[it] = rn[it];
        }
        if (EPI & EPI_COLSUM) {
#pragma unroll
          for (int o = 4; o < 32; o <<= 1) {
            cs.x += __shfl_xor_sync(0xffffffffu, cs.x, o); cs.y += __shfl_xor_sync(0xffffffffu, cs.y, o);
            cs.z += __shfl_xor_sync(0xffffffffu, cs.z, o); cs.w += __shfl_xor_sync(0xffffffffu, cs.w, o);
          }
          if (lane < 4 && n_ok) {
            if (cs_smem) {
              const uint32_t sa = cs_base + 4u * (uint32_t)n;
              asm volatile("red.shared.add.f32 [%0], %1;" ::"r"(sa), "f"(cs.x) : "memory");
              asm volatile("red.shared.add.f32 [%0], %1;" ::"r"(sa + 4u), "f"(cs.y) : "memory");
              asm volatile("red.shared.add.f32 [%0], %1;" ::"r"(sa + 8u), "f"(cs.z) : "memory");
              asm volatile("red.shared.add.f32 [%0], %1;" ::"r"(sa + 12u), "f"(cs.w) : "memory");
            } else {
              float* cd = p.colsum + (long long)tl.group * p.colsum_group_stride + n;
              asm volatile("red.global.add.v4.f32 [%0], {%1, %2, %3, %4};" ::"l"(cd), "f"(cs.x), "f"(cs.y), "f"(cs.z), "f"(cs.w) : "memory");
            }
          }
        }
      }
    }
    if (cs_smem && cs_group >= 0) cs_flush(cs_group);
  } else {
    asm volatile("setmaxnreg.dec.sync.aligned.u32 %0;" ::"n"(PROD_REGS));
    if (A_PACKED) {
      if (warp == FIRST_PROD_WARP && lane == 0) {
        const uint32_t a_bytes = 2u * plane_bytes(BM, A_MN), b_bytes = 2u * plane_bytes(p.BN, B_MN);
        const long long kblocks = (p.K + BK - 1) / BK;
        int stage = 0; uint32_t phase = 0;
        for (int t = blockIdx.x; t < ntiles; t += gridDim.x) {
          const Tile tl = decode_tile(p, t);
          const int nkb = tl.nkb();
          if (nkb == 0) continue;
          const long long kb0 = tl.k_begin / BK;
          const uint8_t* srcA = reinterpret_cast<const uint8_t*>(p.a_packed) + ((long long)(tl.m0 / BM) * kblocks + kb0) * a_bytes;
          const uint8_t* srcB = reinterpret_cast<const uint8_t*>(p.b_packed + (long long)tl.group * p.b_packed_group_stride) +
                                ((long long)(tl.n0 / p.BN) * kblocks + kb0) * b_bytes;
          for (int kb = 0; kb < nkb; ++kb) {
            mbar_wait(empty_bar(stage), phase ^ 1u);
            const uint32_t sb = smem_base + stage * STB;
            asm volatile("mbarrier.arrive.expect_tx.shared::cta.b64 _, [%0], %1;" ::"r"(full_bar(stage)), "r"(a_bytes + b_bytes) : "memory");
            asm volatile("cp.async.bulk.shared::cluster.global.mbarrier::complete_tx::bytes [%0], [%1], %2, [%3];"
                         ::"r"(sb + OFF_A_HI), "l"(srcA + (long long)kb * a_bytes), "r"(a_bytes), "r"(full_bar(stage)) : "memory");
            asm volatile("cp.async.bulk.shared::cluster.global.mbarrier::complete_tx::bytes [%0], [%1], %2, [%3];"
                         ::"r"(sb + OFF_B_HI), "l"(srcB + (long long)kb * b_bytes), "r"(b_bytes), "r"(full_bar(stage)) : "memory");
            if (++stage == NST) { stage = 0; phase ^= 1u; }
          }
        }
      }
    } else {
    const int wq = warp - FIRST_PROD_WARP;
    constexpr int units_a = 16;
    const int segs_b = (p.BN + 127) / 128;
    const int units_b = B_PACKED ? 0 : (B_MN ? 16 * segs_b : p.BN / 8);
    const int units = units_a + units_b;
    const uint32_t st_k = (uint32_t)((lane >> 2) * 64 + ((((uint32_t)lane & 3u) ^ (((uint32_t)lane >> 3) & 3u)) << 4));
    const uint32_t kr_lane = (uint32_t)lane >> 4, j_lane = (uint32_t)lane & 15u;

    constexpr int MU = B_PACKED ? (16 + NUM_PROD_WARPS - 1) / NUM_PROD_WARPS : MAX_UNITS;
    uint32_t off[MU];
    uint32_t vmask = 0;
    const float* baseB = p.B;
    const uint16_t* packB = nullptr;
    int t_cur = blockIdx.x - gridDim.x, kb_cur = 0, nkb_cur = 0, k_begin = 0, k_end = 0;
    const uint32_t adv_a = A_MN ? (uint32_t)(BK * p.a_sk) : (uint32_t)BK;
    const uint32_t adv_b = B_MN ? (uint32_t)(BK * p.b_sk) : (uint32_t)BK;
    const bool b_gather = B_MN && (p.b_k_index != nullptr);

    auto setup_tile = [&](const Tile& tl) {
      k_begin = tl.k_begin; k_end = tl.k_end;
      baseB = p.B + (long long)tl.group * p.b_group_stride;
      if (B_PACKED) {
        const long long kblocks = (p.K + BK - 1) / BK;
        packB = p.b_packed + (long long)tl.group * p.b_packed_group_stride +
                ((long long)(tl.n0 / p.BN) * kblocks) * (2LL * p.BN * BK);
      }
      vmask = 0;
#pragma unroll
      for (int i = 0; i < MU; ++i) {
        const int u = wq + NUM_PROD_WARPS * i;
        off[i] = 0;
        if (u >= units) continue;
        const bool is_a = u < units_a;
        const int ul = is_a ? u : u - units_a;
        const int mn0 = is_a ? tl.m0 : tl.n0;
        const int mn_lim = is_a ? p.M : p.N;
        if (is_a ? !A_MN : !B_MN) {
          const long long s_mn = is_a ? p.a_smn : p.b_smn;
          const int row = mn0 + 8 * ul + (lane >> 2);
          if (row >= mn_lim) continue;
          long long ridx = row;
          if (is_a && p.a_row_index) { ridx = __ldg(p.a_row_index + row); if (ridx < 0) continue; }
          off[i] = (uint32_t)(ridx * s_mn + tl.k_begin + 8 * (lane & 3));
          vmask |= 1u << i;
        } else {
          const int segs = is_a ? 1 : segs_b;
          const int pi = (segs == 2) ? (ul >> 1) : ul, seg = (segs == 2) ? (ul & 1) : 0;
          const int mnl = seg * 128 + 8 * (int)j_lane;
          const int tile_w = is_a ? BM : p.BN;
          if (mnl + 8 > tile_w || mn0 + mnl + 8 > mn_lim) continue;
          const long long s_k = is_a ? p.a_sk : p.b_sk;
          const int koff = 2 * pi + (int)kr_lane;
          off[i] = (!is_a && b_gather) ? (uint32_t)(mn0 + mnl)
                                       : (uint32_t)((long long)(tl.k_begin + koff) * s_k + mn0 + mnl);
          vmask |= 1u << i;
        }
      }
    };
    auto advance = [&]() -> bool {
      if (kb_cur + 1 < nkb_cur) { ++kb_cur; return true; }
      for (t_cur += gridDim.x; t_cur < ntiles; t_cur += gridDim.x) {
        const Tile tl = decode_tile(p, t_cur);
        nkb_cur = tl.nkb();
        if (nkb_cur > 0) { kb_cur = 0; setup_tile(tl); return true; }
      }
      return false;
    };

    auto load_kb = [&](float4 (&r)[MU][2]) {
      const int k0 = k_begin + kb_cur * BK;
      const int kl = k0 + 8 * (lane & 3);
      const bool kin0 = (kl + 4 <= k_end), kin1 = (kl + 8 <= k_end);
#pragma unroll
      for (int i = 0; i < MU; ++i) {
        r[i][0] = make_float4(0.f, 0.f, 0.f, 0.f);
        r[i][1] = make_float4(0.f, 0.f, 0.f, 0.f);
        const int u = wq + NUM_PROD_WARPS * i;
        if (u >= units) continue;
        const bool is_a = u < units_a;
        const float* base = is_a ? p.A : baseB;
        const bool ok = (vmask >> i) & 1u;
        if (is_a ? !A_MN : !B_MN) {
          if (ok && kin0) r[i][0] = ldg_f4(base + off[i]);
          if (ok && kin1) r[i][1] = ldg_f4(base + off[i] + 4);
        } else {
          const int ul = is_a ? u : u - units_a;
          const int pi = (!is_a && segs_b == 2) ? (ul >> 1) : ul;
          const int k = k0 + 2 * pi + (int)kr_lane;
          if (ok && k < k_end) {
            const float* src = base + off[i];
            if (!is_a && b_gather) {
              const int kk = __ldg(p.b_k_index + k);
              src = (kk >= 0) ? base + (long long)kk * p.b_sk + off[i] : nullptr;
            }
            if (src) { r[i][0] = ldg_f4(src); r[i][1] = ldg_f4(src + 4); }
          }
        }
        off[i] += is_a ? adv_a : ((!is_a && b_gather) ? 0u : adv_b);
      }
    };

    auto store_kb = [&](const float4 (&r)[MU][2], uint32_t sb) {
#pragma unroll
      for (int i = 0; i < MU; ++i) {
        const int u = wq + NUM_PROD_WARPS * i;
        if (u >= units) continue;
        const bool is_a = u < units_a;
        const int ul = is_a ? u : u - units_a;
        uint4 hi, lo;
        split4(r[i][0], hi.x, hi.y, lo.x, lo.y);
        split4(r[i][1], hi.z, hi.w, lo.z, lo.w);
        uint32_t o;
        if (is_a ? !A_MN : !B_MN) {
          o = (uint32_t)ul * 512u + st_k;
        } else {
          const int segs = is_a ? 1 : segs_b;
          const uint32_t pi = (segs == 2) ? (uint32_t)(ul >> 1) : (uint32_t)ul;
          const uint32_t seg = (segs == 2) ? (uint32_t)(ul & 1) : 0u;
          const uint32_t k = 2u * pi + kr_lane;
          const uint32_t mc = seg * 16u + j_lane;
          o = ((mc >> 3) * 4u + (k >> 3)) * 1024u + (k & 7u) * 128u + (((mc & 7u) ^ (k & 7u)) << 4);
        }
        const uint32_t dst_hi = sb + (is_a ? OFF_A_HI : OFF_B_HI) + o;
        const uint32_t dst_lo = sb + (is_a ? OFF_A_LO : OFF_B_LO) + o;
        asm volatile("st.shared.v4.b32 [%0], {%1, %2, %3, %4};"
                     ::"r"(dst_hi), "r"(hi.x), "r"(hi.y), "r"(hi.z), "r"(hi.w) : "memory");
        asm volatile("st.shared.v4.b32 [%0], {%1, %2, %3, %4};"
// ... 73 lines not shown
```

### sm3det_b200/functional.py

```python
import torch
from torch.autograd import Function

from . import ops
from .moe_routing import Routing, route, router_backward
from .ops import (EPI_AUXSTORE, EPI_COLSCALE, EPI_DGELU, EPI_GELU, EPI_RESID, EPI_ROWSCALE, LN_NCHW, LN_NHWC, LN_PATCH2)


def _zeros_like_param(p):
    return torch.zeros(p.shape, device=p.device, dtype=torch.float32)


def _taps(w):
    return w.reshape(w.shape[0], -1).t().contiguous()


def _taps_flipped(w):
    return w.flip(2, 3).reshape(w.shape[0], -1).t().contiguous()


@ops.captures_precision
class StemFn(Function):
    @staticmethod
    def forward(ctx, x, w, b, lnw, lnb, eps, ps):
        C0 = w.shape[0]
        wt = w.reshape(C0, -1).t().contiguous()
        train = any(ctx.needs_input_grad)
        x = x.contiguous().float()
        y, conv, stats = ops.stem_fwd(x, wt, b, lnw, lnb, eps, ps, save=train)
        if train:
            ctx.save_for_backward(x, conv, stats, lnw)
            ctx.ps = ps
            ctx.wshape = tuple(w.shape)
        return y

    @staticmethod
    def backward(ctx, dy):
        x, conv, stats, lnw = ctx.saved_tensors
        dy = dy.contiguous()
        C0 = lnw.shape[0]
        T = conv.numel() // C0
        dlnw, dlnb = _zeros_like_param(lnw), _zeros_like_param(lnw)
        du = ops.layernorm_bwd(dy, conv, stats, lnw, dlnw, dlnb, tokens=T, C=C0)
        N, Cin, H, W = x.shape
        ps = ctx.ps
        K = Cin * ps * ps
        Kp = (K + 31) // 32 * 32
        if C0 % 8 == 0:
            col, _, _ = ops.im2col(x, N=N, H=H, W=W, Cin=Cin, ks=ps, stride=ps, pad=0, Kp=Kp, nchw=True)
            dw2 = torch.zeros((C0, Kp), device=x.device, dtype=torch.float32)
            ops.linear_wgrad(du, col, dw2)
            db = torch.zeros((C0,), device=x.device, dtype=torch.float32)
            ops.colsum(du, db, rows=T, Cc=C0)
            dw = dw2[:, :K].reshape(C0, ps, ps, Cin).permute(0, 3, 1, 2).contiguous()
            return None, dw, db, dlnw, dlnb, None, None
        dwt = torch.zeros((K, C0), device=x.device, dtype=torch.float32)
        db = torch.zeros((C0,), device=x.device, dtype=torch.float32)
        ops.stem_wgrad(x, du, dwt, db, ctx.ps)
        dw = dwt.t().reshape(ctx.wshape).contiguous()
        return None, dw, db, dlnw, dlnb, None, None


@ops.captures_precision
class DownsampleFn(Function):
    @staticmethod
    def forward(ctx, x, lnw, lnb, w, b, eps):
        N, H, W, C = x.shape
        Co = w.shape[0]
        T = N * H * W
        train = any(ctx.needs_input_grad)
        xn = torch.empty((T // 4, 4 * C), device=x.device, dtype=torch.float32)
        _, stats = ops.layernorm_fwd(x, lnw, lnb, eps, tokens=T, C=C, out=xn, out_mode=LN_PATCH2, H=H, W=W,
                                     save_stats=train)
        w2 = w.permute(0, 2, 3, 1).reshape(Co, 4 * C).contiguous()
        y = ops.linear_fwd(xn, w2, b, packed=ops.pack_weight(w2, transposed=False))
        if train:
            ctx.save_for_backward(x, stats, xn, lnw, w2)
            ctx.dims = (N, H, W, C, Co)
        return y.view(N, H // 2, W // 2, Co)

    @staticmethod
    def backward(ctx, dy):
        x, stats, xn, lnw, w2 = ctx.saved_tensors
        N, H, W, C, Co = ctx.dims
        T = N * H * W
        dy2 = dy.contiguous().view(T // 4, Co)
        dxn = ops.linear_dgrad(dy2, w2, packed=ops.pack_weight(w2, transposed=True))
        dw2 = torch.zeros_like(w2)
        ops.linear_wgrad(dy2, xn, dw2)
        db = torch.zeros((Co,), device=x.device, dtype=torch.float32)
        ops.colsum(dy2, db, rows=T // 4, Cc=Co)
        dlnw, dlnb = _zeros_like_param(lnw), _zeros_like_param(lnw)
        dx = ops.layernorm_bwd(dxn, x, stats, lnw, dlnw, dlnb, tokens=T, C=C, in_mode=LN_PATCH2, H=H, W=W)
        dw = dw2.view(Co, 2, 2, C).permute(0, 3, 1, 2).contiguous()
        return dx.view(N, H, W, C), dlnw, dlnb, dw, db, None


@ops.captures_precision
class OutNormFn(Function):
    @staticmethod
    def forward(ctx, x, w, b, eps):
        N, H, W, C = x.shape
        T = N * H * W
        train = any(ctx.needs_input_grad)
        y = torch.empty((N, C, H, W), device=x.device, dtype=torch.float32)
        _, stats = ops.layernorm_fwd(x, w, b, eps, tokens=T, C=C, out=y, out_mode=LN_NCHW, H=H, W=W, save_stats=train)
        if train:
            ctx.save_for_backward(x, stats, w)
        return y

    @staticmethod
    def backward(ctx, dy):
        x, stats, w = ctx.saved_tensors
        N, H, W, C = x.shape
        dw, db = _zeros_like_param(w), _zeros_like_param(w)
        dx = ops.layernorm_bwd(dy.contiguous(), x, stats, w, dw, db, tokens=N * H * W, C=C, in_mode=LN_NCHW, H=H, W=W)
        return dx.view(N, H, W, C), dw, db, None


def _block_front(x, dww, dwb, lnw, lnb, eps, train):
    N, H, W, C = x.shape
    u = ops.dwconv7(x, _taps(dww), dwb)
    v, stats = ops.layernorm_fwd(u, lnw, lnb, eps, tokens=N * H * W, C=C, save_stats=train)
    return u, v.view(N * H * W, C), stats


def _block_front_bwd(dv, dout, x, u, stats, dww, lnw):
    N, H, W, C = x.shape
    T = N * H * W
    dlnw, dlnb = _zeros_like_param(lnw), _zeros_like_param(lnw)
    du = ops.layernorm_bwd(dv, u, stats, lnw, dlnw, dlnb, tokens=T, C=C).view(N, H, W, C)
    dx = ops.dwconv7(du, _taps_flipped(dww), None, resid=dout)
    ddwt = torch.zeros((49, C), device=x.device, dtype=torch.float32)
    ddwb = torch.zeros((C,), device=x.device, dtype=torch.float32)
    ops.dwconv7_wgrad(x, du, ddwt, ddwb)
    ddww = ddwt.t().reshape(C, 1, 7, 7).contiguous()
    return dx, ddww, ddwb, dlnw, dlnb


def _dense_ffn(x, v, v_img, b1, w1, w2, b2, gamma, row_scale, resid, packs, keep):
    N, H, W, C = x.shape
    T = N * H * W
    fused = packs.get('fused')
    if fused is not None:
        want_h = keep and fused.get('bwd_mode') != 2
        res = ops.ffn_fused_fwd(v_img, packs['w1_c'][0], packs['w2_n'][0], b1, b2, T=T, C=C, chunk=fused['fwd'],
                                gamma=gamma, row_scale=row_scale, resid=resid, want_aux=keep, want_h=want_h)
        return res[0], (res[2] if want_h else None), res[1]
    h = ops.linear_fwd(v, w1, b1, packed=packs.get('w1'))
    a_k, _, _ = ops.act_pack(h, rows=T, width=4 * C, mode=ops.ACT_GELU, want_k=True)
    y2 = torch.empty((T, C), device=x.device, dtype=torch.float32) if keep else None
    epi = (EPI_COLSCALE | (EPI_RESID if resid is not None else 0) | (EPI_ROWSCALE if row_scale is not None else 0)
           | (EPI_AUXSTORE if keep else 0))
    out = ops.linear_fwd(None, w2, b2, rows=T, a_packed=a_k, epilogue=epi, aux_out=y2, col_scale=gamma,
                         row_scale=row_scale, resid=resid, packed=packs.get('w2'))
    return out, (h if keep else None), y2


@ops.captures_precision
class DenseBlockFn(Function):

    @staticmethod
    def forward(ctx, x, dww, dwb, lnw, lnb, w1, b1, w2, b2, gamma, row_scale, eps, packs):
        N, H, W, C = x.shape
        T = N * H * W
        train = any(ctx.needs_input_grad) and packs.get('grad', True)
        fused = packs.get('fused')
        ctx.shortcut = packs.get('shortcut', True)
        resid = x.view(T, C) if ctx.shortcut else None
        ctx.checkpoint = train and packs.get('checkpoint', False)
        if ctx.checkpoint:
            _, _, v, v_img = ops.dwconv7_ln(x, _taps(dww), dwb, lnw, lnb, eps, want_v=fused is None, want_img=fused is not None)
            out, _, _ = _dense_ffn(x, v, v_img, b1, w1, w2, b2, gamma, row_scale, resid, packs, keep=False)
            ctx.save_for_backward(x, dww, dwb, lnw, lnb, w1, b1, w2, b2, gamma, row_scale)
            ctx.eps = eps
            ctx.packs = packs
            return out.view(N, H, W, C)
        if fused is not None:
            u = ops.dwconv7(x, _taps(dww), dwb)
            v_img, v, stats = ops.layernorm_fwd_img(u, lnw, lnb, eps, tokens=T, C=C, save_stats=train, want_f32=train)
        else:
            u, v, stats = _block_front(x, dww, dwb, lnw, lnb, eps, train)
            v_img = None
        out, h, y2 = _dense_ffn(x, v, v_img, b1, w1, w2, b2, gamma, row_scale, resid, packs, keep=train)
        if train:
            if (fused or {}).get('bwd_mode') != 2:
                v_img = None
            ctx.save_for_backward(x, u, stats, v, v_img, h, y2, dww, lnw, w1, b1, w2, gamma, row_scale)
            ctx.packs = packs
        return out.view(N, H, W, C)

    @staticmethod
    def _recompute(ctx, x, dww, dwb, lnw, lnb, w1, b1, w2, b2, gamma, rs):
        N, H, W, C = x.shape
        want_img = ctx.packs.get('fused') is not None
        u, stats, v, v_img = ops.dwconv7_ln(x, _taps(dww), dwb, lnw, lnb, ctx.eps, want_u=True, want_stats=True, want_v=True,
                                            want_img=want_img)
        resid = x.view(N * H * W, C) if ctx.shortcut else None
        _, h, y2 = _dense_ffn(x, v, v_img, b1, w1, w2, b2, gamma, rs, resid, ctx.packs, keep=True)
        return u, stats, v, v_img, h, y2

    @staticmethod
    def backward(ctx, dout):
        if ctx.checkpoint:
            x, dww, dwb, lnw, lnb, w1, b1, w2, b2, gamma, rs = ctx.saved_tensors
            u, stats, v, v_img, h, y2 = DenseBlockFn._recompute(ctx, x, dww, dwb, lnw, lnb, w1, b1, w2, b2, gamma, rs)
        else:
            x, u, stats, v, v_img, h, y2, dww, lnw, w1, b1, w2, gamma, rs = ctx.saved_tensors
        N, H, W, C = x.shape
        T = N * H * W
        dout = dout.contiguous()
        dz = dout.view(T, C)
        dev = x.device
        if rs is None:
            csum, dgamma = ops.colstat(dz, rows=T, Cc=C, y=y2)
        else:
            dgamma = torch.zeros((C,), device=dev, dtype=torch.float32)
            ops.colsum(dz, dgamma, rows=T, Cc=C, b=y2, row_scale=rs)
            csum = torch.zeros((C,), device=dev, dtype=torch.float32)
            ops.colsum(dz, csum, rows=T, Cc=C, row_scale=rs)
        db2 = csum * gamma
        db1 = torch.zeros((4 * C,), device=dev, dtype=torch.float32)
        dzs = dz if rs is None else ops.scale_rows(dz, row_scale=rs)
        fused = ctx.packs.get('fused') or {}
        if fused.get('bwd_mode'):
            dz_img = ops.pack_act(dzs, rows=T, cols=C, mn_major=False)
            w1_cb = ctx.packs.get('w1_cb')
            dv, dh_mn, a_mn = ops.ffn_fused_bwd(v_img, dz_img, None if w1_cb is None else w1_cb[0], ctx.packs['w2g_t'][0],
                                                ctx.packs['w1_tn'][0], b1, T=T, C=C, chunk=fused['bwd'],
                                                want_wgrad_images=True, db1=db1, h=h if fused['bwd_mode'] == 3 else None)
            del dz_img, h
        else:
            w2g = ops.scale_rows(w2, row_scale=gamma)
            da = ops.linear_dgrad(dz, w2g, epilogue=(EPI_ROWSCALE if rs is not None else 0), row_scale=rs,
                                  packed=ops.pack_weight(w2g, transposed=True))
            dh_k, dh_mn, a_mn = ops.act_pack(h, rows=T, width=4 * C, mode=ops.ACT_BWD, da=da, want_k=True, mn_tile=128,
                                          mn_tile2=ops._pick_bn(4 * C), colsum=db1)
            del da
        dw2 = torch.zeros_like(w2)
        ops.linear_wgrad(dzs, None, dw2, rows=T, row_scale=gamma, x_packed=a_mn)
        del a_mn
        dw1 = torch.zeros_like(w1)
        ops.linear_wgrad(None, v, dw1, rows=T, dy_packed=dh_mn)
        if not fused.get('bwd_mode'):
            dv = ops.linear_dgrad(None, w1, rows=T, a_packed=dh_k, packed=ctx.packs.get('w1_t'))
        dx, ddww, ddwb, dlnw, dlnb = _block_front_bwd(dv, dout if ctx.shortcut else None, x, u, stats, dww, lnw)
        return dx, ddww, ddwb, dlnw, dlnb, dw1, db1, dw2, db2, dgamma, None, None, None


def stack_expert_params(params):
    base = params[0]
    step = base.numel() * base.element_size()
    if all(p.is_contiguous() and p.data_ptr() == base.data_ptr() + i * step for i, p in enumerate(params)):
        return
    with torch.no_grad():
        flat = torch.stack([p.data for p in params]).contiguous()
        for i, p in enumerate(params):
            p.data = flat[i]


def _moe_experts(v, row_index, grouped, w1, b1, w2, b2, R, packs, out=None):
    C = v.shape[1]
    h = ops.linear_fwd(v, w1, b1, row_index=row_index, rows=R, grouped=grouped, w_group_stride=4 * C * C,
                       bias_group_stride=4 * C, packed=packs.get('w1'))
    a_k, _, _ = ops.act_pack(h, rows=R, width=4 * C, mode=ops.ACT_GELU, want_k=True, live_tiles=grouped[1])
    o = ops.linear_fwd(None, w2, b2, rows=R, a_packed=a_k, grouped=grouped, w_group_stride=4 * C * C,
                       bias_group_stride=C, packed=packs.get('w2'), out=out)
    return h, o


def _moe_experts_bwd(d_o, v, h, row_index, grouped, segs, w1, w2, G, packs, dx_out=None):
    R, C = d_o.shape
    dev = d_o.device
    da = ops.linear_dgrad(d_o, w2, grouped=grouped, w_group_stride=4 * C * C, packed=packs.get('w2_t'))
    db1s = torch.zeros((G, 4 * C), device=dev, dtype=torch.float32)
    dh_k, dh_mn, a_mn = ops.act_pack(h, rows=R, width=4 * C, mode=ops.ACT_BWD, da=da, want_k=True, mn_tile=128,
                                      mn_tile2=ops._pick_bn(4 * C), colsum=db1s, live_tiles=grouped[1], tile_group=grouped[0])
    del da
    dw2s = torch.zeros((G, C, 4 * C), device=dev, dtype=torch.float32)
    ops.linear_wgrad(d_o, None, dw2s, rows=R, segs=segs, num_groups=G, x_packed=a_mn)
    del a_mn
    db2s = torch.zeros((G, C), device=dev, dtype=torch.float32)
    ops.colsum(d_o, db2s, rows=R, Cc=C, segs=segs, groups=G)
    dw1s = torch.zeros((G, 4 * C, C), device=dev, dtype=torch.float32)
    ops.linear_wgrad(None, v, dw1s, rows=R, x_row_index=row_index, segs=segs, num_groups=G, dy_packed=dh_mn)
    dxp = torch.empty((R, C), device=dev, dtype=torch.float32) if dx_out is None else dx_out
    ops.linear_dgrad(None, w1, rows=R, a_packed=dh_k, out=dxp, grouped=grouped, w_group_stride=4 * C * C,
                     packed=packs.get('w1_t'))
    return dxp, dw1s, db1s, dw2s, db2s


@ops.captures_precision
class MoEBlockFn(Function):

    @staticmethod
    def forward(ctx, x, dww, dwb, lnw, lnb, gamma, wp, bp, sim, tau, w_noise, row_scale, noise, eps, E, k, record, packs,
                *experts):
        N, H, W, C = x.shape
        T = N * H * W
        w1s, b1s, w2s, b2s = experts[0:E], experts[E:2 * E], experts[2 * E:3 * E], experts[3 * E:4 * E]
        train = any(ctx.needs_input_grad)
        ctx.checkpoint = train and packs.get('checkpoint', False)
        if ctx.checkpoint:
            _, _, v, _ = ops.dwconv7_ln(x, _taps(dww), dwb, lnw, lnb, eps, want_v=True)
        else:
            u, v, stats = _block_front(x, dww, dwb, lnw, lnb, eps, train)
        rt = route(v, wp, bp, sim, tau, w_noise, noise, E, k, save=train and not ctx.checkpoint)
        h, o = _moe_experts(v, rt.pair_token, rt.grouped, w1s[0], b1s[0], w2s[0], b2s[0], rt.rows, packs)
        ctx.shortcut = packs.get('shortcut', True)
        out, y = ops.moe_combine(o, rt.slot_of, rt.top_idx, rt.top_gate, gamma, x.view(T, C) if ctx.shortcut else None,
                                 row_scale, T=T, Cc=C, k=k, want_y=record is not None)
        if record is not None:
            record.append(dict(v=v, y=y, **rt.record()))
        if ctx.checkpoint:
            rt.save(ctx, x, dww, dwb, lnw, lnb, gamma, row_scale, w1s[0], b1s[0], w2s[0], b2s[0])
            ctx.eps = eps
        elif train:
            rt.save(ctx, x, u, stats, v, h, o, dww, lnw, gamma, row_scale, w1s[0], w2s[0])
        ctx.packs = packs
        return out.view(N, H, W, C), rt.loss.reshape(())

    @staticmethod
    def backward(ctx, dout, dloss):
        if ctx.checkpoint:
            (x, dww, dwb, lnw, lnb, gamma, rs, w1, b1, w2, b2), rt = Routing.load(ctx)
            u, stats, v, _ = ops.dwconv7_ln(x, _taps(dww), dwb, lnw, lnb, ctx.eps, want_u=True, want_stats=True, want_v=True)
            rt.rerun_router(v)
            h, o = _moe_experts(v, rt.pair_token, rt.grouped, w1, b1, w2, b2, rt.rows, ctx.packs)
        else:
            (x, u, stats, v, h, o, dww, lnw, gamma, rs, w1, w2), rt = Routing.load(ctx)
        N, H, W, C = x.shape
        T = N * H * W
        E, k = rt.E, rt.k
        dev = x.device
        dout = dout.contiguous()
        dz = dout.view(T, C)
        d_o = torch.zeros((rt.rows, C), device=dev, dtype=torch.float32)
        dgamma = torch.zeros((C,), device=dev, dtype=torch.float32)
        dgate = ops.moe_combine_bwd(dz, o, rt.slot_of, rt.top_idx, rt.top_gate, gamma, rs, d_o, dgamma, T=T, Cc=C, k=k)
        dxp, dw1s, db1s, dw2s, db2s = _moe_experts_bwd(d_o, v, h, rt.pair_token, rt.grouped, rt.segs, w1, w2, E, ctx.packs)
        dv_r, dwp, dbp, dsim, dtau, dwn = router_backward(rt, v, dgate, dloss, wp_t=ctx.packs.get('wp_t'))
        dv = ops.gather_sum(dxp, rt.slot_of, dv_r, T=T, Cc=C, k=k)
        dx, ddww, ddwb, dlnw, dlnb = _block_front_bwd(dv, dout if ctx.shortcut else None, x, u, stats, dww, lnw)
        grads_e = [dw1s[e] for e in range(E)] + [db1s[e] for e in range(E)] + [dw2s[e] for e in range(E)] + \
                  [db2s[e] for e in range(E)]
        return (dx, ddww, ddwb, dlnw, dlnb, dgamma, dwp, dbp, dsim, dtau, dwn, None, None, None, None, None, None, None,
                *grads_e)


@ops.captures_precision
class DAGateFn(Function):

    @staticmethod
    def forward(ctx, y, x, s, row_scale):
        N, H, W, C = y.shape
        y, x = y.contiguous(), x.contiguous()
        hw = H * W
        out = torch.empty_like(x)
        sc = s if row_scale is None else s * row_scale.view(N, hw)[:, :1]
        sc = sc.contiguous()
        for n in range(N):
            ops.affine(y[n].view(hw, C), a1=sc[n], add=x[n].view(hw, C), out=out[n].view(hw, C))
        ctx.save_for_backward(y, sc, s, row_scale)
        return out

    @staticmethod
    def backward(ctx, d):
        y, sc, s, rs = ctx.saved_tensors
        N, H, W, C = y.shape
        hw = H * W
        d = d.contiguous()
        dy = torch.empty_like(y)
        dsc = torch.zeros((N, C), device=y.device, dtype=torch.float32)
        for n in range(N):
            ops.affine(d[n].view(hw, C), a1=sc[n], out=dy[n].view(hw, C))
            ops.colsum(d[n].view(hw, C), dsc[n], rows=hw, Cc=C, b=y[n].view(hw, C))
        ds = dsc if rs is None else dsc * rs.view(N, hw)[:, :1]
        return dy, d, ds, None


@ops.captures_precision
class SampleMeanFn(Function):

    @staticmethod
    def forward(ctx, y):
        N, H, W, C = y.shape
        y = y.contiguous()
        m = torch.zeros((N, C), device=y.device, dtype=torch.float32)
        for n in range(N):
            ops.colsum(y[n].view(H * W, C), m[n], rows=H * W, Cc=C)
        ctx.shape = (N, H, W, C)
        return m / float(H * W)

    @staticmethod
    def backward(ctx, dm):
        N, H, W, C = ctx.shape
        return (dm / float(H * W)).view(N, 1, 1, C).expand(N, H, W, C).contiguous()
```

### sm3det_b200/ops.py

```python
import ctypes as C
import ctypes as _ct
from typing import Optional

import torch

from . import _lib

SCHED_DENSE, SCHED_GROUPED, SCHED_SPLITK = 0, 1, 2
EPI_BIAS, EPI_GELU, EPI_DGELU, EPI_COLSCALE, EPI_ROWSCALE, EPI_RESID, EPI_ATOMIC, EPI_AUXSTORE, EPI_COLSUM = 1, 2, 4, 8, 16, 32, 64, 128, 256
LN_NHWC, LN_PATCH2, LN_NCHW = 0, 1, 2


import contextlib
import threading

_tls = threading.local()


def current_passes() -> int:
    return getattr(_tls, 'passes', 3)


@contextlib.contextmanager
def precision_scope(passes: int):
    if passes not in (1, 3):
        raise ValueError('mma passes must be 3 (fp32-accurate split-bf16) or 1 (bf16 operands)')
    prev = current_passes()
    _tls.passes = passes
    try:
        yield
    finally:
        _tls.passes = prev


def autocast_passes(module=None) -> int:
    import torch as _t
    return 1 if (getattr(module, 'amp', False) or _t.is_autocast_enabled()) else 3


def captures_precision(cls):
    fwd, bwd = cls.forward, cls.backward

    def forward(ctx, *args, **kwargs):
        ctx._mma_passes = current_passes()
        return fwd(ctx, *args, **kwargs)

    def backward(ctx, *grads):
        with precision_scope(ctx._mma_passes):
            return bwd(ctx, *grads)

    cls.forward = staticmethod(forward)
    cls.backward = staticmethod(backward)
    return cls


def _stream():
    return torch.cuda.current_stream().cuda_stream


def _p(t: Optional[torch.Tensor], dtype=torch.float32):
    if t is None:
        return None
    if not t.is_cuda:
        raise RuntimeError('sm3det_b200 ops need CUDA tensors (no CPU fallback exists)')
    if t.dtype != dtype:
        raise TypeError(f'expected {dtype}, got {t.dtype}')
    if not t.is_contiguous():
        raise ValueError('expected a contiguous tensor')
    return t.data_ptr()


def _pi(t):
    return _p(t, torch.int32)


def _pick_bn(n: int) -> int:
    for bn in (128, 96, 64, 32):
        if n % bn == 0:
            return bn
    if n > 0 and n % 8 == 0:
        return min((128, 96, 64, 32), key=lambda bn: (-(-n // bn), -(-n // bn) * bn))
    raise ValueError(f'N={n} has no GEMM tile width (multiple of 8)')


def _n_tiles(n: int) -> int:
    return -(-n // _pick_bn(n))


def num_sms() -> int:
    return torch.cuda.get_device_properties(torch.cuda.current_device()).multi_processor_count


def gemm(*, A, a_smn, a_sk, B, b_smn, b_sk, M, N, K, D, ldd, b_group_stride=0, a_row_index=None, b_k_index=None,
         sched=SCHED_DENSE, k_splits=1, num_groups=1, tile_group=None, num_m_tiles=None, seg_begin=None,
         seg_end=None, d_group_stride=0, bias=None, bias_group_stride=0, epilogue=0, aux_out=None, aux_in=None,
         ld_aux=0, col_scale=None, row_scale=None, resid=None, ld_resid=0, tile_n=0, b_packed=None,
         b_packed_group_stride=0, colsum=None, colsum_group_stride=0, a_packed=None):
    lib = _lib.load()
    a = _lib.GemmArgs()
    a.A = _p(A); a.a_stride_mn = a_smn; a.a_stride_k = a_sk
    a.b_packed = None if b_packed is None else _p(b_packed, torch.int16); a.b_packed_group_stride = b_packed_group_stride
    a.a_packed = None if a_packed is None else _p(a_packed, torch.int16)
    a.B = _p(B); a.b_stride_mn = b_smn; a.b_stride_k = b_sk; a.b_group_stride = b_group_stride
    a.a_row_index = _pi(a_row_index); a.b_k_index = _pi(b_k_index)
    a.M, a.N, a.K = M, N, K
    a.tile_n = tile_n; a.sched = sched; a.k_splits = k_splits; a.num_groups = num_groups
    a.tile_group = _pi(tile_group); a.num_m_tiles = _pi(num_m_tiles)
    a.seg_begin = _pi(seg_begin); a.seg_end = _pi(seg_end)
    a.D = _p(D); a.ldd = ldd; a.d_group_stride = d_group_stride
    a.bias = _p(bias); a.bias_group_stride = bias_group_stride
    a.epilogue = epilogue
    a.aux_out = _p(aux_out); a.aux_in = _p(aux_in); a.ld_aux = ld_aux
    a.col_scale = _p(col_scale); a.row_scale = _p(row_scale)
    a.resid = _p(resid); a.ld_resid = ld_resid
    a.colsum = _p(colsum); a.colsum_group_stride = colsum_group_stride
    a.mma_passes = current_passes()
    _lib.check(lib.sm3_gemm(C.byref(a), _stream()), 'sm3_gemm')
    return D


def pack_weight(w, *, transposed: bool, groups: int = 1, out=None, tile: int = 0):
    lib = _lib.load()
    n_, k_ = w.shape[-2], w.shape[-1]
    if transposed:
        N, K, s_mn, s_k = k_, n_, 1, k_
    else:
        N, K, s_mn, s_k = n_, k_, k_, 1
    per = lib.sm3_gemm_packed_elems(N, K)
    if out is None or out.numel() != groups * per:
        out = torch.empty((groups * per,), device=w.device, dtype=torch.int16)
    if tile:
        _lib.check(lib.sm3_gemm_pack_b_tile(_p(w), s_mn, s_k, n_ * k_, groups, N, K, tile, out.data_ptr(), _stream()),
                   'sm3_gemm_pack_b_tile')
    else:
        _lib.check(lib.sm3_gemm_pack_b(_p(w), s_mn, s_k, n_ * k_, groups, N, K, out.data_ptr(), _stream()), 'sm3_gemm_pack_b')
    return out, per


def pack_act(x, *, rows, cols, mn_major, tile=128, row_index=None, ld=None):
    lib = _lib.load()
    n = lib.sm3_gemm_packed_act_elems(rows, cols, 1 if mn_major else 0, tile)
    out = torch.empty((n,), device=x.device, dtype=torch.int16)
    _lib.check(lib.sm3_gemm_pack_act(_p(x), cols if ld is None else ld, _pi(row_index), rows, cols, 1 if mn_major else 0, tile,
                                     out.data_ptr(), _stream()), 'sm3_gemm_pack_act')
    return out


ACT_GELU, ACT_DGELU, ACT_COPY, ACT_BWD = 0, 1, 2, 3


FFN_FWD, FFN_BWD_DX, FFN_BWD_IMG, FFN_BWD_IMG_H = 0, 1, 2, 3


def ffn_chunk(mode: int, C: int) -> int:
    import os
    if os.environ.get('SM3_FUSED_FFN', '1') == '0':
        return 0
    if mode >= FFN_BWD_IMG and os.environ.get('SM3_FUSED_FFN_BWD', '1') == '0':
        return 0
    return int(_lib.load().sm3_ffn_fused_chunk(mode, C))


def _ffn_args(*, T, C, chunk, mode, a1, wa1, b1, a2=None, wa2=None, wb=None):
    a = _lib.FfnArgs()
    a.a1 = _p(a1, torch.int16); a.a2 = None if a2 is None else _p(a2, torch.int16)
    a.wa1 = _p(wa1, torch.int16); a.wa2 = None if wa2 is None else _p(wa2, torch.int16)
    a.wb = None if wb is None else _p(wb, torch.int16)
    a.bias1 = _p(b1)
    a.M, a.C, a.H4, a.chunk, a.mma_passes, a.mode = T, C, 4 * C, chunk, current_passes(), mode
    return a


def ffn_fused_fwd(v_img, w1_img, w2_img, b1, b2, *, T, C, chunk, gamma=None, row_scale=None, resid=None, want_aux=False,
                  want_h=False):
    lib = _lib.load()
    out = torch.empty((T, C), device=b1.device, dtype=torch.float32)
    aux = torch.empty((T, C), device=b1.device, dtype=torch.float32) if want_aux else None
    h = torch.empty((T, 4 * C), device=b1.device, dtype=torch.float32) if want_h else None
    a = _ffn_args(T=T, C=C, chunk=chunk, mode=FFN_FWD, a1=v_img, wa1=w1_img, b1=b1, wb=w2_img)
    a.bias2 = _p(b2); a.col_scale = _p(gamma); a.row_scale = _p(row_scale); a.resid = _p(resid)
    a.out = _p(out); a.aux_out = _p(aux); a.h_out = _p(h)
    _lib.check(lib.sm3_ffn_fused(_ct.byref(a), _stream()), 'sm3_ffn_fused(fwd)')
    return (out, aux, h) if want_h else (out, aux)


def ffn_fused_bwd(v_img, dz_img, w1_img, w2gt_img, w1t_img, b1, *, T, C, chunk, want_wgrad_images=False, db1=None, h=None):
    lib = _lib.load()
    out = torch.empty((T, C), device=b1.device, dtype=torch.float32)
    if not want_wgrad_images:
        a = _ffn_args(T=T, C=C, chunk=chunk, mode=FFN_BWD_DX, a1=v_img, a2=dz_img, wa1=w1_img, wa2=w2gt_img, b1=b1, wb=w1t_img)
        a.out = _p(out)
        _lib.check(lib.sm3_ffn_fused(_ct.byref(a), _stream()), 'sm3_ffn_fused(bwd)')
        return out
    if db1 is None:
        raise ValueError('ffn_fused_bwd: want_wgrad_images needs db1')
    n = lib.sm3_gemm_packed_act_elems(T, 4 * C, 1, 128)
    dh_mn = torch.empty((n,), device=b1.device, dtype=torch.int16)
    a_mn = torch.empty((n,), device=b1.device, dtype=torch.int16)
    mode = FFN_BWD_IMG if h is None else FFN_BWD_IMG_H
    a = _ffn_args(T=T, C=C, chunk=chunk, mode=mode, a1=v_img if h is None else dz_img, a2=dz_img,
                  wa1=w1_img if h is None else w2gt_img, wa2=w2gt_img, b1=b1, wb=w1t_img)
    a.out = _p(out); a.dh_mn = dh_mn.data_ptr(); a.act_mn = a_mn.data_ptr(); a.db1 = _p(db1); a.h_in = _p(h)
    _lib.check(lib.sm3_ffn_fused(_ct.byref(a), _stream()), 'sm3_ffn_fused(bwd)')
    return out, dh_mn, a_mn


def fused_cost(name, *a, **kw):
    T, Cc = kw['T'], kw['C']
    unit = 2.0 * T * Cc * 4 * Cc
    wbytes = 2 * 4.0 * 4 * Cc * Cc
    if name == 'ffn_fused_fwd':
        return 2 * unit, (3 + (1 if kw.get('want_aux') else 0) + (4 if kw.get('want_h') else 0)) * 4.0 * T * Cc + wbytes, (T, Cc, 'fwd')
    if not kw.get('want_wgrad_images'):
        return 2 * unit, 3 * 4.0 * T * Cc + 2 * wbytes, (T, Cc, 'bwd-dv')
    h = kw.get('h') is not None
    return 2 * unit, (8 + (16 if h else 4) + 32) * float(T * Cc) + 2 * wbytes, (T, Cc, 'bwd-img-h' if h else 'bwd-img')


def act_pack(h, *, rows, width, mode, da=None, want_k=False, mn_tile=0, want_f32=False, colsum=None, live_tiles=None,
             tile_group=None, mn_tile2=0):
    lib = _lib.load()
    dev = h.device
    a = _lib.ActPackArgs()
    pk = pm = of = None
    if want_k:
        pk = torch.empty((lib.sm3_gemm_packed_act_elems(rows, width, 0, 128),), device=dev, dtype=torch.int16)
    if mn_tile:
        pm = torch.empty((lib.sm3_gemm_packed_act_elems(rows, width, 1, mn_tile),), device=dev, dtype=torch.int16)
    if want_f32:
        of = torch.empty((rows, width), device=dev, dtype=torch.float32)
    a.h = _p(h); a.da = _p(da); a.R = rows; a.W = width; a.mode = mode
    a.live_tiles = _pi(live_tiles); a.tile_group = _pi(tile_group)
    a.out_f32 = _p(of); a.pack_k = None if pk is None else pk.data_ptr(); a.pack_mn = None if pm is None else pm.data_ptr()
    a.mn_tile = mn_tile; a.colsum = _p(colsum)
    pm2 = None
    if mode == ACT_BWD:
        pm2 = torch.empty((lib.sm3_gemm_packed_act_elems(rows, width, 1, mn_tile2),), device=dev, dtype=torch.int16)
        a.pack_mn2 = pm2.data_ptr(); a.mn_tile2 = mn_tile2
    _lib.check(lib.sm3_act_pack(C.byref(a), _stream()), 'sm3_act_pack')
    if mode == ACT_BWD:
        return pk, pm, pm2
    return pk, pm, of


import os as _os
PACK_A_MIN_K = int(_os.environ.get('SM3_PACK_A_MIN_K', '96'))
PACK_W_MIN_TILES = int(_os.environ.get('SM3_PACK_W_MIN_TILES', '2'))


def _pack_a_pays(N, K):
    return K >= PACK_A_MIN_K and _n_tiles(N) >= 2 or K >= 4 * PACK_A_MIN_K


def linear_fwd(x, w, bias=None, *, epilogue=0, out=None, aux_out=None, col_scale=None, row_scale=None, resid=None,
               row_index=None, rows=None, grouped=None, w_group_stride=0, bias_group_stride=0, packed=None,
               a_packed=None):
    K = w.shape[-1]
    N = w.shape[-2]
    M = rows if rows is not None else x.shape[0]
    if out is None:
        out = torch.empty((M, N), device=w.device, dtype=torch.float32)
    epi = epilogue | (EPI_BIAS if bias is not None else 0)
    kw = {}
    if grouped is not None:
        kw = dict(sched=SCHED_GROUPED, tile_group=grouped[0], num_m_tiles=grouped[1])
    if packed is not None:
        kw.update(b_packed=packed[0], b_packed_group_stride=packed[1])
        if a_packed is not None:
            kw.update(a_packed=a_packed)
            row_index = None
        elif _pack_a_pays(N, K):
            kw.update(a_packed=pack_act(x, rows=M, cols=K, mn_major=False, row_index=row_index))
            row_index = None
    gemm(A=x, a_smn=K, a_sk=1, B=w, b_smn=K, b_sk=1, b_group_stride=w_group_stride, M=M, N=N, K=K, D=out, ldd=N,
         a_row_index=row_index, bias=bias, bias_group_stride=bias_group_stride, epilogue=epi, aux_out=aux_out,
         ld_aux=N, col_scale=col_scale, row_scale=row_scale, resid=resid, ld_resid=N, **kw)
    return out


def linear_dgrad(dy, w, *, epilogue=0, out=None, aux_in=None, row_scale=None, resid=None, grouped=None,
                 w_group_stride=0, packed=None, colsum=None, colsum_group_stride=0, a_packed=None, rows=None):
    N = w.shape[-2]
    M = rows if rows is not None else dy.shape[0]
    K = w.shape[-1]
    if out is None:
        out = torch.empty((M, K), device=w.device, dtype=torch.float32)
    kw = {}
    if grouped is not None:
        kw = dict(sched=SCHED_GROUPED, tile_group=grouped[0], num_m_tiles=grouped[1])
    if packed is not None:
        kw.update(b_packed=packed[0], b_packed_group_stride=packed[1])
        if a_packed is not None:
            kw.update(a_packed=a_packed)
        elif _pack_a_pays(K, N):
            kw.update(a_packed=pack_act(dy, rows=M, cols=N, mn_major=False))
    gemm(A=dy, a_smn=N, a_sk=1, B=w, b_smn=1, b_sk=K, b_group_stride=w_group_stride, M=M, N=K, K=N, D=out, ldd=K,
         epilogue=epilogue | (EPI_COLSUM if colsum is not None else 0), aux_in=aux_in, ld_aux=K, row_scale=row_scale,
         resid=resid, ld_resid=K, colsum=colsum, colsum_group_stride=colsum_group_stride, **kw)
    return out


def linear_wgrad(dy, x, dw, *, rows=None, x_row_index=None, row_scale=None, segs=None, num_groups=1, dy_packed=None,
                 x_packed=None):
    R = rows if rows is not None else dy.shape[0]
    N = dw.shape[-2]
    K = dw.shape[-1]
    tiles = ((N + 127) // 128) * _n_tiles(K) * num_groups
    splits = -(-3 * num_sms() // max(1, tiles))
    splits = max(1, min(64 if tiles > 1 else 2 * num_sms(), splits, max(1, (R // num_groups) // 1024)))
    epi = EPI_ATOMIC | (EPI_ROWSCALE if row_scale is not None else 0)
    kw = {}
    if dy_packed is not None or x_packed is not None or ((N + 127) // 128) * _n_tiles(K) >= PACK_W_MIN_TILES:
        if dy_packed is None:
            dy_packed = pack_act(dy, rows=R, cols=N, mn_major=True, tile=128)
        if x_packed is None:
            x_packed = pack_act(x, rows=R, cols=K, mn_major=True, tile=_pick_bn(K), row_index=x_row_index)
        kw = dict(a_packed=dy_packed, b_packed=x_packed)
        x_row_index = None
    gemm(A=dy, a_smn=1, a_sk=N, B=x, b_smn=1, b_sk=K, M=N, N=K, K=R, D=dw, ldd=K, d_group_stride=N * K,
         b_k_index=x_row_index, **kw, sched=SCHED_SPLITK, k_splits=splits, num_groups=num_groups,
         seg_begin=None if segs is None else segs[0], seg_end=None if segs is None else segs[1],
         epilogue=epi, row_scale=row_scale)
    return dw


def layernorm_fwd(x, w, b, eps, *, tokens, C, out=None, out_mode=LN_NHWC, H=0, W=0, save_stats=False):
    lib = _lib.load()
    if out is None:
        out = torch.empty_like(x)
    stats = torch.empty((tokens, 2), device=x.device, dtype=torch.float32) if save_stats else None
    _lib.check(lib.sm3_layernorm_fwd(_p(x), _p(w), _p(b), _p(out), _p(stats), tokens, C, float(eps), out_mode, H, W,
                                     _stream()), 'sm3_layernorm_fwd')
    return out, stats


def layernorm_fwd_img(x, w, b, eps, *, tokens, C, save_stats=False, want_f32=False):
    lib = _lib.load()
    img = torch.empty((lib.sm3_gemm_packed_act_elems(tokens, C, 0, 128),), device=x.device, dtype=torch.int16)
    y = torch.empty((tokens, C), device=x.device, dtype=torch.float32) if want_f32 else None
    stats = torch.empty((tokens, 2), device=x.device, dtype=torch.float32) if save_stats else None
    _lib.check(lib.sm3_layernorm_fwd_img(_p(x), _p(w), _p(b), img.data_ptr(), _p(y), _p(stats), tokens, C, float(eps), _stream()),
               'sm3_layernorm_fwd_img')
    return img, y, stats


def layernorm_bwd(dy, x, stats, w, dw, db, *, tokens, C, in_mode=LN_NHWC, H=0, W=0, dx=None, accumulate=False):
    lib = _lib.load()
    if dx is None:
        dx = torch.empty((tokens, C), device=x.device, dtype=torch.float32)
    _lib.check(lib.sm3_layernorm_bwd(_p(dy), _p(x), _p(stats), _p(w), _p(dx), _p(dw), _p(db), tokens, C, in_mode, H, W,
                                     1 if accumulate else 0, _stream()), 'sm3_layernorm_bwd')
    return dx


def stem_fwd(x, wt, bias, lnw, lnb, eps, ps, *, save=False):
    lib = _lib.load()
    N, Cin, H, W = x.shape
    C0 = wt.shape[1]
    y = torch.empty((N, H // ps, W // ps, C0), device=x.device, dtype=torch.float32)
    conv = torch.empty_like(y) if save else None
    stats = torch.empty((N * (H // ps) * (W // ps), 2), device=x.device, dtype=torch.float32) if save else None
    _lib.check(lib.sm3_stem_fwd(_p(x), _p(wt), _p(bias), _p(lnw), _p(lnb), _p(y), _p(conv), _p(stats), N, Cin, H, W,
                                ps, C0, float(eps), _stream()), 'sm3_stem_fwd')
    return y, conv, stats


def stem_wgrad(x, du, dwt, dbias, ps):
    lib = _lib.load()
    N, Cin, H, W = x.shape
    _lib.check(lib.sm3_stem_wgrad(_p(x), _p(du), _p(dwt), _p(dbias), N, Cin, H, W, ps, dwt.shape[1], _stream()),
               'sm3_stem_wgrad')


def dwconv7(x, wt, bias=None, resid=None, out=None):
    lib = _lib.load()
    N, H, W, Cc = x.shape
    if out is None:
        out = torch.empty_like(x)
    _lib.check(lib.sm3_dwconv7_fwd(_p(x), _p(wt), _p(bias), _p(resid), _p(out), N, H, W, Cc, _stream()), 'sm3_dwconv7_fwd')
    return out


def dwconv7_ln(x, wt, bias, lnw, lnb, eps, *, want_u=False, want_stats=False, want_v=False, want_img=False):
    lib = _lib.load()
    N, H, W, Cc = x.shape
    T = N * H * W
    dev = x.device
    u = torch.empty((N, H, W, Cc), device=dev, dtype=torch.float32) if want_u else None
    stats = torch.empty((T, 2), device=dev, dtype=torch.float32) if want_stats else None
    v = torch.empty((T, Cc), device=dev, dtype=torch.float32) if want_v else None
    img = torch.empty((lib.sm3_gemm_packed_act_elems(T, Cc, 0, 128),), device=dev, dtype=torch.int16) if want_img else None
    _lib.check(lib.sm3_dwconv7_ln_fwd(_p(x), _p(wt), _p(bias), _p(lnw), _p(lnb), _p(u), _p(stats), _p(v),
                                      None if img is None else img.data_ptr(), N, H, W, Cc, float(eps), _stream()),
               'sm3_dwconv7_ln_fwd')
    return u, stats, v, img


def dwconv7_wgrad(x, dy, dwt, dbias):
    lib = _lib.load()
    N, H, W, Cc = x.shape
    _lib.check(lib.sm3_dwconv7_wgrad(_p(x), _p(dy), _p(dwt), _p(dbias), N, H, W, Cc, _stream()), 'sm3_dwconv7_wgrad')


def moe_router(v, wp, bp, sim, tau, *, T, Cc, E, k, w_noise=None, noise=None, save=False):
    lib = _lib.load()
    P = wp.shape[0]
    dev = v.device
    a = _lib.RouterArgs()
    top_idx = torch.empty((T, k), device=dev, dtype=torch.int32)
    top_gate = torch.empty((T, k), device=dev, dtype=torch.float32)
    logits = torch.empty((T, E), device=dev, dtype=torch.float32) if save else None
    p_out = torch.empty((T, P), device=dev, dtype=torch.float32) if save else None
    m = min(k + 1, E)
    noisy_save = save and noise is not None
    top_vals = torch.empty((T, m), device=dev, dtype=torch.float32) if noisy_save else None
    top_idx_m = torch.empty((T, m), device=dev, dtype=torch.int32) if noisy_save else None
    sigma = torch.empty((T, E), device=dev, dtype=torch.float32) if noisy_save else None
    nb = lib.sm3_moe_router_blocks(T)
    partials = torch.empty((nb, 3 * E), device=dev, dtype=torch.float32)
    a.v = _p(v); a.proj_weight = _p(wp); a.proj_bias = _p(bp); a.sim_matrix = _p(sim); a.temperature = _p(tau)
    a.w_noise = _p(w_noise) if noise is not None else None
    a.noise = _p(noise)
    a.T, a.C, a.P, a.E, a.k = T, Cc, P, E, k
    a.top_idx = _pi(top_idx); a.top_gate = _p(top_gate); a.logits = _p(logits); a.top_vals = _p(top_vals)
    a.p_out = _p(p_out); a.partials = _p(partials); a.sigma = _p(sigma); a.top_idx_m = _pi(top_idx_m)
    _lib.check(lib.sm3_moe_router(C.byref(a), _stream()), 'sm3_moe_router')
    return dict(top_idx=top_idx, top_gate=top_gate, logits=logits, p=p_out, top_vals=top_vals, partials=partials,
                sigma=sigma, top_idx_m=top_idx_m)


def moe_plan(partials, *, T, E, k):
    lib = _lib.load()
    dev = partials.device
    max_tiles = (T * k + 127) // 128 + E
    f = torch.empty(2 * E + 1, device=dev, dtype=torch.float32)
    i = torch.empty(4 * E + max_tiles + 1, device=dev, dtype=torch.int32)
    importance, load, loss = f[:E], f[E:2 * E], f[2 * E:2 * E + 1]
    counts, seg_begin, seg_end, cursor = i[:E], i[E:2 * E], i[2 * E:3 * E], i[3 * E:4 * E]
    tile_group = i[4 * E:4 * E + max_tiles]
    num_m_tiles = i[4 * E + max_tiles:]
    a = _lib.PlanArgs()
    a.partials = _p(partials); a.T, a.E, a.k, a.max_m_tiles = T, E, k, max_tiles
    a.importance = importance.data_ptr(); a.load = load.data_ptr(); a.loss = loss.data_ptr()
    a.counts = counts.data_ptr(); a.seg_begin = seg_begin.data_ptr(); a.seg_end = seg_end.data_ptr()
    a.cursor = cursor.data_ptr(); a.tile_group = tile_group.data_ptr(); a.num_m_tiles = num_m_tiles.data_ptr()
    _lib.check(lib.sm3_moe_plan(C.byref(a), _stream()), 'sm3_moe_plan')
    return dict(importance=importance, load=load, loss=loss, counts=counts, seg_begin=seg_begin, seg_end=seg_end,
                cursor=cursor, tile_group=tile_group, num_m_tiles=num_m_tiles, max_rows=max_tiles * 128)


def moe_assign(top_idx, plan, *, T, E, k):
    lib = _lib.load()
# ... 242 lines not shown
```

Before: 104.1.

## Fuse GELU/dGELU activation packing into GEMM epilogue for MoE and FFN paths

Adds packing epilogues (EPI_PACK_K, EPI_PACK_MN) to the bf16x3 wgmma GEMM. The FFN1 GEMM then writes bias+GELU output directly as packed K-major bf16 hi/lo images, and the dgrad GEMM applies dGELU, column sums and writes the K-major and MN-major packed images directly. This removes the separate act_pack kernel launches and the fp32 round trip of the intermediate activations and gradients. In exchange the consumer warps get a larger register budget, the mainloop gains a per-k-block hook, and the epilogue does more work per tile.

```diff
diff --git a/include/sm3det_b200.h b/include/sm3det_b200.h
--- a/include/sm3det_b200.h
+++ b/include/sm3det_b200.h
@@ -30,7 +30,9 @@
   SM3_EPI_RESID = 32,
   SM3_EPI_ATOMIC = 64,
   SM3_EPI_AUXSTORE = 128,
-  SM3_EPI_COLSUM = 256
+  SM3_EPI_COLSUM = 256,
+  SM3_EPI_PACK_K = 512,
+  SM3_EPI_PACK_MN = 1024
 };
 typedef struct sm3_gemm_args {
   const float* A; int64_t a_stride_mn, a_stride_k;
@@ -56,6 +58,7 @@
   const float* resid; int64_t ld_resid;
   float* colsum; int64_t colsum_group_stride;
   int32_t mma_passes;
+  uint16_t* pack_k; uint16_t* pack_mn; uint16_t* pack_mn2;
 } sm3_gemm_args;
 int sm3_gemm(const sm3_gemm_args* args, void* stream);
 int64_t sm3_gemm_packed_elems(int32_t N, int32_t K);
diff --git a/sm3det_b200/_lib.py b/sm3det_b200/_lib.py
--- a/sm3det_b200/_lib.py
+++ b/sm3det_b200/_lib.py
@@ -28,6 +28,7 @@
         ('resid', c_f32p), ('ld_resid', C.c_int64),
         ('colsum', c_f32p), ('colsum_group_stride', C.c_int64),
         ('mma_passes', C.c_int32),
+        ('pack_k', C.c_void_p), ('pack_mn', C.c_void_p), ('pack_mn2', C.c_void_p),
     ]
 
 
diff --git a/sm3det_b200/csrc/capi.cu b/sm3det_b200/csrc/capi.cu
--- a/sm3det_b200/csrc/capi.cu
+++ b/sm3det_b200/csrc/capi.cu
@@ -39,6 +39,7 @@
   p.col_scale = a->col_scale; p.row_scale = a->row_scale;
   p.resid = a->resid; p.ld_resid = a->ld_resid;
   p.colsum = a->colsum; p.colsum_group_stride = a->colsum_group_stride;
+  p.pack_k = a->pack_k; p.pack_mn = a->pack_mn; p.pack_mn2 = a->pack_mn2;
   p.passes = (a->mma_passes == 1) ? 1 : 3;
   return gemm::launch(p, S(stream));
 }
diff --git a/sm3det_b200/csrc/ffn_fused.cu b/sm3det_b200/csrc/ffn_fused.cu
--- a/sm3det_b200/csrc/ffn_fused.cu
+++ b/sm3det_b200/csrc/ffn_fused.cu
@@ -224,38 +224,7 @@
               asm volatile("red.shared.add.f32 [%0], %1;" ::"r"(cs_base + 4u * (uint32_t)(col + 8 * ((lane >> 4) & 1) + 2 * (lane & 3) + ((lane >> 3) & 1))),
                            "f"(csum) : "memory");
             __syncwarp();
-            const int sr = lane >> 1, sc = 8 * (lane & 1);
-            const long long row = wrow0 + sr;
-            if (row < R_pad) {
-              float dv8[8], av8[8];
-              float4 x0, x1, z0, z1;
-              const uint32_t ro = stage_base + (uint32_t)(sr * EPI_STAGE_ROW_FLOATS + sc) * 4u;
-              asm volatile("ld.shared.v4.f32 {%0, %1, %2, %3}, [%4];" : "=f"(x0.x), "=f"(x0.y), "=f"(x0.z), "=f"(x0.w) : "r"(ro) : "memory");
-              asm volatile("ld.shared.v4.f32 {%0, %1, %2, %3}, [%4];" : "=f"(x1.x), "=f"(x1.y), "=f"(x1.z), "=f"(x1.w) : "r"(ro + 16u) : "memory");
-              asm volatile("ld.shared.v4.f32 {%0, %1, %2, %3}, [%4];" : "=f"(z0.x), "=f"(z0.y), "=f"(z0.z), "=f"(z0.w)
-                           : "r"(ro + 16u * EPI_STAGE_ROW_FLOATS * 4u) : "memory");
-              asm volatile("ld.shared.v4.f32 {%0, %1, %2, %3}, [%4];" : "=f"(z1.x), "=f"(z1.y), "=f"(z1.z), "=f"(z1.w)
-                           : "r"(ro + 16u * EPI_STAGE_ROW_FLOATS * 4u + 16u) : "memory");
-              const bool live = row < p.M;
-              dv8[0] = x0.x; dv8[1] = x0.y; dv8[2] = x0.z; dv8[3] = x0.w; dv8[4] = x1.x; dv8[5] = x1.y; dv8[6] = x1.z; dv8[7] = x1.w;
-              av8[0] = z0.x; av8[1] = z0.y; av8[2] = z0.z; av8[3] = z0.w; av8[4] = z1.x; av8[5] = z1.y; av8[6] = z1.z; av8[7] = z1.w;
-              uint32_t dh_[4], dl_[4], ah_[4], al_[4];
-#pragma unroll
-              for (int e = 0; e < 4; ++e) {
-                split2(live ? dv8[2 * e] : 0.f, live ? dv8[2 * e + 1] : 0.f, dh_[e], dl_[e]);
-                split2(live ? av8[2 * e] : 0.f, live ? av8[2 * e + 1] : 0.f, ah_[e], al_[e]);
-              }
-              constexpr uint32_t PB = 8192u;
-              const int n = col + sc;
-              const long long blk = ((long long)(n >> 7) * (R_pad >> 5) + (row >> 5)) * (2LL * PB);
-              const uint32_t o = mnmajor_sw128_offset((uint32_t)(row & 31), (uint32_t)((n & 127) >> 3));
-              uint8_t* dimg = reinterpret_cast<uint8_t*>(p.dh_mn) + blk + o;
-              uint8_t* aimg = reinterpret_cast<uint8_t*>(p.act_mn) + blk + o;
-              *reinterpret_cast<uint4*>(dimg) = make_uint4(dh_[0], dh_[1], dh_[2], dh_[3]);
-              *reinterpret_cast<uint4*>(dimg + PB) = make_uint4(dl_[0], dl_[1], dl_[2], dl_[3]);
-              *reinterpret_cast<uint4*>(aimg) = make_uint4(ah_[0], ah_[1], ah_[2], ah_[3]);
-              *reinterpret_cast<uint4*>(aimg + PB) = make_uint4(al_[0], al_[1], al_[2], al_[3]);
-            }
+            store_staged_images(stage_base, lane, wrow0, col, p.M, R_pad, p.H4, p.dh_mn, p.act_mn, 128, nullptr);
             __syncwarp();
           }
         } else {
diff --git a/sm3det_b200/csrc/gemm_tc.cu b/sm3det_b200/csrc/gemm_tc.cu
--- a/sm3det_b200/csrc/gemm_tc.cu
+++ b/sm3det_b200/csrc/gemm_tc.cu
@@ -180,7 +180,8 @@
 int launch(Params p, cudaStream_t stream) {
   if (p.b_packed && !p.B) p.B = reinterpret_cast<const float*>(p.b_packed);
   if (p.a_packed && !p.A) p.A = reinterpret_cast<const float*>(p.a_packed);
-  SM3_REQUIRE(p.A && p.B && p.D, SM3_ERR_INVALID_ARG, "gemm: null operand");
+  const bool pack = (p.epi & (EPI_PACK_K | EPI_PACK_MN)) != 0;
+  SM3_REQUIRE(p.A && p.B && (p.D || pack), SM3_ERR_INVALID_ARG, "gemm: null operand");
   SM3_REQUIRE(p.M > 0 && p.N > 0 && p.K >= 0, SM3_ERR_INVALID_ARG, "gemm: bad shape %d %d %d", p.M, p.N, p.K);
   SM3_REQUIRE((p.a_smn == 1) != (p.a_sk == 1) || (p.a_smn == 1 && p.M == 1), SM3_ERR_INVALID_ARG,
               "gemm: A needs exactly one unit stride");
@@ -196,7 +197,7 @@
   if (p.BN == 0) p.BN = pick_bn(p.N);
   SM3_REQUIRE(p.BN >= 32 && p.BN <= MAX_BN && p.BN % 32 == 0 && p.N % 8 == 0, SM3_ERR_UNSUPPORTED_SHAPE,
               "gemm: N=%d has no tile width (N a multiple of 8, tile width a multiple of 32 <= 128)", p.N);
-  SM3_REQUIRE(aligned16(p.A) && aligned16(p.B) && aligned16(p.D), SM3_ERR_INVALID_ARG, "gemm: pointers must be 16B aligned");
+  SM3_REQUIRE(aligned16(p.A) && aligned16(p.B) && (!p.D || aligned16(p.D)), SM3_ERR_INVALID_ARG, "gemm: pointers must be 16B aligned");
   if (!a_mn) SM3_REQUIRE(p.a_smn % 4 == 0 && p.K % 4 == 0, SM3_ERR_UNSUPPORTED_SHAPE, "gemm: K-major A needs K%%4==0, lda%%4==0");
   else       SM3_REQUIRE(p.a_sk % 4 == 0 && p.M % 8 == 0, SM3_ERR_UNSUPPORTED_SHAPE, "gemm: MN-major A needs M%%8==0, lda%%4==0");
   if (!b_mn) SM3_REQUIRE(p.b_smn % 4 == 0 && p.K % 4 == 0, SM3_ERR_UNSUPPORTED_SHAPE, "gemm: K-major B needs K%%4==0, ldb%%4==0");
@@ -255,7 +256,21 @@
     SM3_REQUIRE(aligned16(p.a_packed) && aligned16(p.b_packed) && (p.b_packed_group_stride % 8) == 0, SM3_ERR_INVALID_ARG,
                 "gemm: packed operands must be 16B aligned");
     constexpr int E_FFN2_TRAIN = EPI_BIAS | EPI_COLSCALE | EPI_RESID | EPI_AUXSTORE, E_FFN2_EVAL = EPI_BIAS | EPI_COLSCALE | EPI_RESID;
-    if (a_mn) {
+    constexpr int E_FFN1_PACK = EPI_BIAS | EPI_GELU | EPI_PACK_K;
+    constexpr int E_DGRAD2_PACK = EPI_DGELU | EPI_COLSUM | EPI_PACK_K | EPI_PACK_MN, E_DGRAD2_PACK_RS = E_DGRAD2_PACK | EPI_ROWSCALE;
+    if (pack) {
+      SM3_REQUIRE(!a_mn && (p.epi == E_FFN1_PACK || p.epi == E_DGRAD2_PACK || p.epi == E_DGRAD2_PACK_RS), SM3_ERR_INVALID_ARG,
+                  "gemm: packing epilogue flag set %d is not instantiated", p.epi);
+      SM3_REQUIRE(p.sched != SCHED_SPLITK && p.N % p.BN == 0 && p.pack_k && aligned16(p.pack_k), SM3_ERR_INVALID_ARG,
+                  "gemm: packing epilogue needs a dense / grouped schedule, no column tail and a 16B-aligned pack_k");
+      SM3_REQUIRE(!(p.epi & EPI_PACK_MN) || (p.pack_mn && p.pack_mn2 && aligned16(p.pack_mn) && aligned16(p.pack_mn2)),
+                  SM3_ERR_INVALID_ARG, "gemm: EPI_PACK_MN needs 16B-aligned pack_mn, pack_mn2");
+    }
+    if (pack) {
+      if (p.epi == E_FFN1_PACK) SM3_GEMM_LAUNCH_E(false, false, true, true, E_FFN1_PACK);
+      else if (p.epi == E_DGRAD2_PACK) SM3_GEMM_LAUNCH_E(false, false, true, true, E_DGRAD2_PACK);
+      else SM3_GEMM_LAUNCH_E(false, false, true, true, E_DGRAD2_PACK_RS);
+    } else if (a_mn) {
       if (p.epi == EPI_ATOMIC) SM3_GEMM_LAUNCH_E(true, true, true, true, EPI_ATOMIC);
       else if (p.epi == (EPI_ATOMIC | EPI_ROWSCALE)) SM3_GEMM_LAUNCH_E(true, true, true, true, EPI_ATOMIC | EPI_ROWSCALE);
       else SM3_GEMM_LAUNCH(true, true, true, true);
@@ -268,12 +283,14 @@
     }
   }
   else if (packed) {
+    SM3_REQUIRE(!pack, SM3_ERR_INVALID_ARG, "gemm: the packing epilogue needs both operands packed");
     SM3_REQUIRE(!a_mn && p.sched != SCHED_SPLITK && p.BN == pick_bn(p.N), SM3_ERR_INVALID_ARG,
                 "gemm: packed B needs K-major A, a dense/grouped schedule and the default tile width");
     SM3_REQUIRE((reinterpret_cast<uintptr_t>(p.b_packed) & 15u) == 0 && (p.b_packed_group_stride % 8) == 0,
                 SM3_ERR_INVALID_ARG, "gemm: packed B must be 16B aligned");
     SM3_GEMM_LAUNCH(false, false, true, false);
   }
+  else if (pack) SM3_REQUIRE(false, SM3_ERR_INVALID_ARG, "gemm: the packing epilogue needs both operands packed");
   else if (!a_mn && !b_mn) SM3_GEMM_LAUNCH(false, false, false, false);
   else if (!a_mn && b_mn) SM3_GEMM_LAUNCH(false, true, false, false);
   else if (a_mn && b_mn) SM3_GEMM_LAUNCH(true, true, false, false);
diff --git a/sm3det_b200/csrc/gemm_tc.cuh b/sm3det_b200/csrc/gemm_tc.cuh
--- a/sm3det_b200/csrc/gemm_tc.cuh
+++ b/sm3det_b200/csrc/gemm_tc.cuh
@@ -43,6 +43,8 @@
   EPI_ATOMIC = 64,
   EPI_AUXSTORE = 128,
   EPI_COLSUM = 256,
+  EPI_PACK_K = 512,
+  EPI_PACK_MN = 1024,
 };
 
 struct Params {
@@ -67,6 +69,7 @@
   const float* col_scale; const float* row_scale;
   const float* resid; long long ld_resid;
   float* colsum; long long colsum_group_stride;
+  uint16_t* pack_k; uint16_t* pack_mn; uint16_t* pack_mn2;
   int passes;
   int nstages; unsigned stage_bytes;
   int debug;
@@ -184,9 +187,59 @@
   l23 = __byte_perm(r2, r3, 0x7632);
 }
 
+__device__ __forceinline__ void store_staged_images(uint32_t stage, int lane, long long row0, int col0, long long live_rows,
+                                                    long long R_pad, int W, uint16_t* mn, uint16_t* mn2, int mn2_tile,
+                                                    uint16_t* kimg) {
+  const int sr = lane >> 1, sc = 8 * (lane & 1);
+  const long long row = row0 + sr;
+  if (row >= R_pad) return;
+  const bool live = row < live_rows;
+  const int n = col0 + sc;
+  auto load_split = [&](uint32_t addr, uint4& hi, uint4& lo) {
+    float4 x0 = make_float4(0.f, 0.f, 0.f, 0.f), x1 = x0;
+    if (live) {
+      asm volatile("ld.shared.v4.f32 {%0, %1, %2, %3}, [%4];" : "=f"(x0.x), "=f"(x0.y), "=f"(x0.z), "=f"(x0.w) : "r"(addr) : "memory");
+      asm volatile("ld.shared.v4.f32 {%0, %1, %2, %3}, [%4];" : "=f"(x1.x), "=f"(x1.y), "=f"(x1.z), "=f"(x1.w) : "r"(addr + 16u) : "memory");
+    }
+    split4(x0, hi.x, hi.y, lo.x, lo.y);
+    split4(x1, hi.z, hi.w, lo.z, lo.w);
+  };
+  const uint32_t ro = stage + (uint32_t)(sr * EPI_STAGE_ROW_FLOATS + sc) * 4u;
+  constexpr uint32_t PB = 8192u;
+  const long long blk = ((long long)(n >> 7) * (R_pad >> 5) + (row >> 5)) * (2LL * PB);
+  const uint32_t o = mnmajor_sw128_offset((uint32_t)(row & 31), (uint32_t)((n & 127) >> 3));
+  if (mn || kimg) {
+    uint4 hi, lo;
+    load_split(ro, hi, lo);
+    if (mn) {
+      uint8_t* d = reinterpret_cast<uint8_t*>(mn) + blk + o;
+      *reinterpret_cast<uint4*>(d) = hi;
+      *reinterpret_cast<uint4*>(d + PB) = lo;
+    }
+    if (kimg) {
+      uint8_t* d = reinterpret_cast<uint8_t*>(kimg) + ((row >> 7) * ((W + BK - 1) / BK) + (n >> 5)) * 16384LL +
+                   kmajor_sw64_offset((uint32_t)(row & 127), (uint32_t)((n & 31) >> 3));
+      *reinterpret_cast<uint4*>(d) = hi;
+      *reinterpret_cast<uint4*>(d + 8192) = lo;
+    }
+  }
+  if (mn2) {
+    uint4 hi, lo;
+    load_split(ro + 16u * EPI_STAGE_ROW_FLOATS * 4u, hi, lo);
+    const uint32_t pb2 = plane_bytes(mn2_tile, true);
+    uint8_t* d = reinterpret_cast<uint8_t*>(mn2) + ((long long)(n / mn2_tile) * (R_pad >> 5) + (row >> 5)) * (2LL * pb2) +
+                 mnmajor_sw128_offset((uint32_t)(row & 31), (uint32_t)((n % mn2_tile) >> 3));
+    *reinterpret_cast<uint4*>(d) = hi;
+    *reinterpret_cast<uint4*>(d + pb2) = lo;
+  }
+}
+
 template <bool A_MN, bool B_MN, bool B_PACKED, bool A_PACKED, int EPI_T>
 __global__ void __launch_bounds__(NUM_THREADS, 1) gemm_bf16x3_kernel(const __grid_constant__ Params p) {
   const int EPI = (EPI_T >= 0) ? EPI_T : p.epi;
+  constexpr bool PACK = EPI_T >= 0 && (EPI_T & (EPI_PACK_K | EPI_PACK_MN)) != 0;
+  constexpr bool PACK_MN = PACK && (EPI_T & EPI_PACK_MN) != 0;
+  constexpr int CREGS = PACK ? 232 : CONS_REGS, PREGS = PACK ? 24 : PROD_REGS;
   extern __shared__ uint8_t smem_raw[];
   const uint32_t smem_base = (smem_u32(smem_raw) + 1023u) & ~1023u;
   const uint32_t bar_base = smem_base + STAGES * STAGE_BYTES;
@@ -206,7 +259,7 @@
   const int ntiles = total_tiles(p);
 
   if (warp < NUM_CONS_WARPS) {
-    asm volatile("setmaxnreg.inc.sync.aligned.u32 %0;" ::"n"(CONS_REGS));
+    asm volatile("setmaxnreg.inc.sync.aligned.u32 %0;" ::"n"(CREGS));
     constexpr int NE = NUM_CONS_WARPS;
     const int wg = warp >> 2;
     const int nchunks = p.BN / EPI_CW;
@@ -237,6 +290,51 @@
     constexpr uint32_t b_kstep = B_MN ? 2u * MN_SBO_BYTES : 32u;
     const uint32_t b_lo_off = B_PACKED ? OFF_B_HI + plane_bytes(p.BN, B_MN) : OFF_B_LO;
     float acc[MAX_BN / 2];
+    const long long R_pad = ((long long)p.M + 31) / 32 * 32;
+    auto mainloop = [&](auto bn_c, int nkb, int& prev, auto&& hook) {
+      constexpr int N = decltype(bn_c)::value;
+      for (int kb = 0; kb < nkb; ++kb) {
+        mbar_wait(full_bar(stage), phase);
+        wg::fence();
+        const uint32_t sb = smem_base + stage * STB + (uint32_t)wg * WG_A_BYTES;
+        const uint32_t sbb = smem_base + stage * STB;
+#pragma unroll
+        for (int j = 0; j < BK / 16; ++j) {
+          const uint64_t ahi = make_smem_desc(sb + OFF_A_HI + j * a_kstep, A_MN);
+          const uint64_t alo = make_smem_desc(sb + OFF_A_LO + j * a_kstep, A_MN);
+          const uint64_t bhi = make_smem_desc(sbb + OFF_B_HI + j * b_kstep, B_MN);
+          const uint64_t blo = make_smem_desc(sbb + b_lo_off + j * b_kstep, B_MN);
+          if (!(p.debug & 4)) {
+            const uint32_t accum = (kb > 0 || j > 0) ? 1u : 0u;
+            if (p.passes == 1) {
+              wg::mma<N, A_MN, B_MN>(acc, ahi, bhi, accum);
+            } else {
+              wg::mma<N, A_MN, B_MN>(acc, alo, bhi, accum);
+              wg::mma<N, A_MN, B_MN>(acc, ahi, blo, 1u);
+              wg::mma<N, A_MN, B_MN>(acc, ahi, bhi, 1u);
+            }
+          }
+        }
+        wg::commit();
+        if (prev >= 0) {
+          wg::wait<1>();
+          __syncwarp();
+          if (lane == 0) mbar_arrive(empty_bar(prev));
+        }
+        hook(kb);
+        prev = stage;
+        if (++stage == NST) { stage = 0; phase ^= 1u; }
+      }
+    };
+    auto run_mainloop = [&](int nkb, int& prev, auto&& hook) {
+      switch (p.BN) {
+        case 32: mainloop(std::integral_constant<int, 32>{}, nkb, prev, hook); break;
+        case 64: mainloop(std::integral_constant<int, 64>{}, nkb, prev, hook); break;
+        case 96: mainloop(std::integral_constant<int, 96>{}, nkb, prev, hook); break;
+        default: mainloop(std::integral_constant<int, 128>{}, nkb, prev, hook); break;
+      }
+    };
+    if constexpr (!PACK) {
     for (int t = blockIdx.x; t < ntiles; t += gridDim.x) {
       const Tile tl = decode_tile(p, t);
       const int nkb = tl.nkb();
@@ -255,46 +353,7 @@
       if (EPI & EPI_RESID) load_resid(0, rr);
 
       int prev = -1;
-      auto mainloop = [&](auto bn_c) {
-        constexpr int N = decltype(bn_c)::value;
-        for (int kb = 0; kb < nkb; ++kb) {
-          mbar_wait(full_bar(stage), phase);
-          wg::fence();
-          const uint32_t sb = smem_base + stage * STB + (uint32_t)wg * WG_A_BYTES;
-          const uint32_t sbb = smem_base + stage * STB;
-#pragma unroll
-          for (int j = 0; j < BK / 16; ++j) {
-            const uint64_t ahi = make_smem_desc(sb + OFF_A_HI + j * a_kstep, A_MN);
-            const uint64_t alo = make_smem_desc(sb + OFF_A_LO + j * a_kstep, A_MN);
-            const uint64_t bhi = make_smem_desc(sbb + OFF_B_HI + j * b_kstep, B_MN);
-            const uint64_t blo = make_smem_desc(sbb + b_lo_off + j * b_kstep, B_MN);
-            if (!(p.debug & 4)) {
-              const uint32_t accum = (kb > 0 || j > 0) ? 1u : 0u;
-              if (p.passes == 1) {
-                wg::mma<N, A_MN, B_MN>(acc, ahi, bhi, accum);
-              } else {
-                wg::mma<N, A_MN, B_MN>(acc, alo, bhi, accum);
-                wg::mma<N, A_MN, B_MN>(acc, ahi, blo, 1u);
-                wg::mma<N, A_MN, B_MN>(acc, ahi, bhi, 1u);
-              }
-            }
-          }
-          wg::commit();
-          if (prev >= 0) {
-            wg::wait<1>();
-            __syncwarp();
-            if (lane == 0) mbar_arrive(empty_bar(prev));
-          }
-          prev = stage;
-          if (++stage == NST) { stage = 0; phase ^= 1u; }
-        }
-      };
-      switch (p.BN) {
-        case 32: mainloop(std::integral_constant<int, 32>{}); break;
-        case 64: mainloop(std::integral_constant<int, 64>{}); break;
-        case 96: mainloop(std::integral_constant<int, 96>{}); break;
-        default: mainloop(std::integral_constant<int, 128>{}); break;
-      }
+      run_mainloop(nkb, prev, [](int) {});
       wg::wait<0>();
       wg::fence_operand(acc);
       __syncwarp();
@@ -378,9 +437,134 @@
         }
       }
     }
+
+    } else {
+      float acc_p[MAX_BN / 2];
+      bool pend = false, p_dead = false;
+      int p_n0 = 0, p_group = 0, p_row0 = 0, p_mlim = 0, p_done = 0;
+      float4 ha[2], hn[2];
+      auto load_aux = [&](int c_, float4 (&dst)[2]) {
+        const int n_ = p_n0 + c_ * EPI_CW + c4;
+#pragma unroll
+        for (int it = 0; it < 2; ++it) {
+          const int row = p_row0 + it * 8 + rl;
+          dst[it] = (row < p_mlim && n_ < p.N) ? ldg_f4(p.aux_in + (long long)row * p.ld_aux + n_) : make_float4(0.f, 0.f, 0.f, 0.f);
+        }
+      };
+      auto run_chunk = [&](int c) {
+        __syncwarp();
+#pragma unroll
+        for (int qq = 0; qq < 2; ++qq)
+#pragma unroll
+          for (int h = 0; h < 2; ++h)
+            asm volatile("st.shared.v2.f32 [%0], {%1, %2};"
+                         ::"r"(stage_base + (uint32_t)((rl + 8 * h) * EPI_STAGE_ROW_FLOATS + 8 * qq + 2 * (lane & 3)) * 4u),
+                           "f"(acc_p[4 * qq + 2 * h]), "f"(acc_p[4 * qq + 2 * h + 1]) : "memory");
+#pragma unroll
+        for (int i = 0; i < MAX_BN / 2 - 8; ++i) acc_p[i] = acc_p[i + 8];
+        if (PACK_MN && (EPI & EPI_DGELU) && c + 1 < nchunks) load_aux(c + 1, hn);
+        __syncwarp();
+        const int n = p_n0 + c * EPI_CW + c4;
+        float4 bv = make_float4(0.f, 0.f, 0.f, 0.f);
+        if (EPI & EPI_BIAS) bv = ldg_f4(p.bias + (long long)p_group * p.bias_group_stride + n);
+        float4 cs = make_float4(0.f, 0.f, 0.f, 0.f);
+#pragma unroll
+        for (int it = 0; it < 2; ++it) {
+          const int r = it * 8 + rl;
+          const int row = p_row0 + r;
+          if (row >= p_mlim) continue;
+          float4 x;
+          asm volatile("ld.shared.v4.f32 {%0, %1, %2, %3}, [%4];"
+                       : "=f"(x.x), "=f"(x.y), "=f"(x.z), "=f"(x.w)
+                       : "r"(stage_base + (uint32_t)(r * EPI_STAGE_ROW_FLOATS + c4) * 4u) : "memory");
+          x.x += bv.x; x.y += bv.y; x.z += bv.z; x.w += bv.w;
+          if ((EPI & EPI_GELU) && p.aux_out) *reinterpret_cast<float4*>(p.aux_out + (long long)row * p.ld_aux + n) = x;
+          if (EPI & EPI_GELU) { x.x = gelu_fast(x.x); x.y = gelu_fast(x.y); x.z = gelu_fast(x.z); x.w = gelu_fast(x.w); }
+          if (EPI & EPI_ROWSCALE) { const float rs = __ldg(p.row_scale + row); x.x *= rs; x.y *= rs; x.z *= rs; x.w *= rs; }
+          float4 g2 = make_float4(0.f, 0.f, 0.f, 0.f);
+          if (PACK_MN && (EPI & EPI_DGELU)) {
+            const float4 hh = ha[it];
+            const float hv[4] = {hh.x, hh.y, hh.z, hh.w};
+            float xv[4] = {x.x, x.y, x.z, x.w}, av[4];
+#pragma unroll
+            for (int e = 0; e < 4; ++e) {
+              float Phi, ex;
+              phi_parts(hv[e], Phi, ex);
+              av[e] = hv[e] * Phi;
+              xv[e] *= fmaf(hv[e] * 0.39894228040143267794f, ex, Phi);
+            }
+            x = make_float4(xv[0], xv[1], xv[2], xv[3]);
+            g2 = make_float4(av[0], av[1], av[2], av[3]);
+          }
+          cs.x += x.x; cs.y += x.y; cs.z += x.z; cs.w += x.w;
+          const uint32_t so = stage_base + (uint32_t)(r * EPI_STAGE_ROW_FLOATS + c4) * 4u;
+          asm volatile("st.shared.v4.f32 [%0], {%1, %2, %3, %4};" ::"r"(so), "f"(x.x), "f"(x.y), "f"(x.z), "f"(x.w) : "memory");
+          if (PACK_MN)
+            asm volatile("st.shared.v4.f32 [%0], {%1, %2, %3, %4};" ::"r"(so + 16u * EPI_STAGE_ROW_FLOATS * 4u),
+                         "f"(g2.x), "f"(g2.y), "f"(g2.z), "f"(g2.w) : "memory");
+        }
+        if (PACK_MN && (EPI & EPI_DGELU)) {
+#pragma unroll
+          for (int it = 0; it < 2; ++it) ha[it] = hn[it];
+        }
+        __syncwarp();
+        store_staged_images(stage_base, lane, p_row0, p_n0 + c * EPI_CW, p_mlim, R_pad, p.N, PACK_MN ? p.pack_mn : nullptr,
+                            PACK_MN ? p.pack_mn2 : nullptr, p.BN, (EPI & EPI_PACK_K) ? p.pack_k : nullptr);
+        if ((EPI & EPI_COLSUM) && !p_dead) {
+#pragma unroll
+          for (int o = 4; o < 32; o <<= 1) {
+            cs.x += __shfl_xor_sync(0xffffffffu, cs.x, o); cs.y += __shfl_xor_sync(0xffffffffu, cs.y, o);
+            cs.z += __shfl_xor_sync(0xffffffffu, cs.z, o); cs.w += __shfl_xor_sync(0xffffffffu, cs.w, o);
+          }
+          if (lane < 4) {
+            if (cs_smem) {
+              const uint32_t sa = cs_base + 4u * (uint32_t)n;
+              asm volatile("red.shared.add.f32 [%0], %1;" ::"r"(sa), "f"(cs.x) : "memory");
+              asm volatile("red.shared.add.f32 [%0], %1;" ::"r"(sa + 4u), "f"(cs.y) : "memory");
+              asm volatile("red.shared.add.f32 [%0], %1;" ::"r"(sa + 8u), "f"(cs.z) : "memory");
+              asm volatile("red.shared.add.f32 [%0], %1;" ::"r"(sa + 12u), "f"(cs.w) : "memory");
+            } else {
+              float* cd = p.colsum + (long long)p_group * p.colsum_group_stride + n;
+              asm volatile("red.global.add.v4.f32 [%0], {%1, %2, %3, %4};" ::"l"(cd), "f"(cs.x), "f"(cs.y), "f"(cs.z), "f"(cs.w) : "memory");
+            }
+          }
+        }
+      };
+      auto drain = [&]() {
+        if (pend) for (; p_done < nchunks; ++p_done) run_chunk(p_done);
+        pend = false;
+      };
+      auto set_pending = [&](const Tile& tl, bool dead) {
+        p_n0 = tl.n0; p_group = tl.group; p_row0 = tl.m0 + wg * 64 + (warp & 3) * 16; p_mlim = dead ? 0 : p.M;
+        p_dead = dead; p_done = 0; pend = true;
+        if (cs_smem && !dead && tl.group != cs_group) { if (cs_group >= 0) cs_flush(cs_group); cs_group = tl.group; }
+        if (PACK_MN && (EPI & EPI_DGELU)) load_aux(0, ha);
+      };
+      const int ntiles_c = (p.sched == SCHED_GROUPED) ? p.num_tiles : ntiles;
+      for (int t = blockIdx.x; t < ntiles_c; t += gridDim.x) {
+        const bool dead = t >= ntiles;
+        Tile tl;
+        if (dead) { tl.m0 = t / p.n_tiles * BM; tl.n0 = t % p.n_tiles * p.BN; tl.group = 0; tl.k_begin = 0; tl.k_end = 0; }
+        else tl = decode_tile(p, t);
+        const int nkb = tl.nkb();
+        if (nkb == 0 && !dead) continue;
+        if (dead) { drain(); set_pending(tl, true); continue; }
+        int prev = -1;
+        run_mainloop(nkb, prev, [&](int) { if (pend && p_done < nchunks) run_chunk(p_done++); });
+        drain();
+        wg::wait<0>();
+        wg::fence_operand(acc);
+        __syncwarp();
+        if (lane == 0) mbar_arrive(empty_bar(prev));
+#pragma unroll
+        for (int i = 0; i < MAX_BN / 2; ++i) acc_p[i] = (p.debug & 4) ? 0.f : acc[i];
+        set_pending(tl, false);
+      }
+      drain();
+    }
     if (cs_smem && cs_group >= 0) cs_flush(cs_group);
   } else {
-    asm volatile("setmaxnreg.dec.sync.aligned.u32 %0;" ::"n"(PROD_REGS));
+    asm volatile("setmaxnreg.dec.sync.aligned.u32 %0;" ::"n"(PREGS));
     if (A_PACKED) {
       if (warp == FIRST_PROD_WARP && lane == 0) {
         const uint32_t a_bytes = 2u * plane_bytes(BM, A_MN), b_bytes = 2u * plane_bytes(p.BN, B_MN);
diff --git a/sm3det_b200/functional.py b/sm3det_b200/functional.py
--- a/sm3det_b200/functional.py
+++ b/sm3det_b200/functional.py
@@ -146,8 +146,7 @@
         res = ops.ffn_fused_fwd(v_img, packs['w1_c'][0], packs['w2_n'][0], b1, b2, T=T, C=C, chunk=fused['fwd'],
                                 gamma=gamma, row_scale=row_scale, resid=resid, want_aux=keep, want_h=want_h)
         return res[0], (res[2] if want_h else None), res[1]
-    h = ops.linear_fwd(v, w1, b1, packed=packs.get('w1'))
-    a_k, _, _ = ops.act_pack(h, rows=T, width=4 * C, mode=ops.ACT_GELU, want_k=True)
+    h, a_k = ops.linear_gelu_packed(v, w1, b1, packed=packs['w1'], want_h=keep)
     y2 = torch.empty((T, C), device=x.device, dtype=torch.float32) if keep else None
     epi = (EPI_COLSCALE | (EPI_RESID if resid is not None else 0) | (EPI_ROWSCALE if row_scale is not None else 0)
            | (EPI_AUXSTORE if keep else 0))
@@ -231,11 +230,8 @@
             del dz_img, h
         else:
             w2g = ops.scale_rows(w2, row_scale=gamma)
-            da = ops.linear_dgrad(dz, w2g, epilogue=(EPI_ROWSCALE if rs is not None else 0), row_scale=rs,
-                                  packed=ops.pack_weight(w2g, transposed=True))
-            dh_k, dh_mn, a_mn = ops.act_pack(h, rows=T, width=4 * C, mode=ops.ACT_BWD, da=da, want_k=True, mn_tile=128,
-                                          mn_tile2=ops._pick_bn(4 * C), colsum=db1)
-            del da
+            dh_k, dh_mn, a_mn = ops.linear_dgrad_dgelu_packed(dz, w2g, h, row_scale=rs, colsum=db1,
+                                                              packed=ops.pack_weight(w2g, transposed=True))
         dw2 = torch.zeros_like(w2)
         ops.linear_wgrad(dzs, None, dw2, rows=T, row_scale=gamma, x_packed=a_mn)
         del a_mn
@@ -260,9 +256,8 @@
 
 def _moe_experts(v, row_index, grouped, w1, b1, w2, b2, R, packs, out=None):
     C = v.shape[1]
-    h = ops.linear_fwd(v, w1, b1, row_index=row_index, rows=R, grouped=grouped, w_group_stride=4 * C * C,
-                       bias_group_stride=4 * C, packed=packs.get('w1'))
-    a_k, _, _ = ops.act_pack(h, rows=R, width=4 * C, mode=ops.ACT_GELU, want_k=True, live_tiles=grouped[1])
+    h, a_k = ops.linear_gelu_packed(v, w1, b1, row_index=row_index, rows=R, grouped=grouped, w_group_stride=4 * C * C,
+                                    bias_group_stride=4 * C, packed=packs['w1'])
     o = ops.linear_fwd(None, w2, b2, rows=R, a_packed=a_k, grouped=grouped, w_group_stride=4 * C * C,
                        bias_group_stride=C, packed=packs.get('w2'), out=out)
     return h, o
@@ -271,11 +266,9 @@
 def _moe_experts_bwd(d_o, v, h, row_index, grouped, segs, w1, w2, G, packs, dx_out=None):
     R, C = d_o.shape
     dev = d_o.device
-    da = ops.linear_dgrad(d_o, w2, grouped=grouped, w_group_stride=4 * C * C, packed=packs.get('w2_t'))
     db1s = torch.zeros((G, 4 * C), device=dev, dtype=torch.float32)
-    dh_k, dh_mn, a_mn = ops.act_pack(h, rows=R, width=4 * C, mode=ops.ACT_BWD, da=da, want_k=True, mn_tile=128,
-                                      mn_tile2=ops._pick_bn(4 * C), colsum=db1s, live_tiles=grouped[1], tile_group=grouped[0])
-    del da
+    dh_k, dh_mn, a_mn = ops.linear_dgrad_dgelu_packed(d_o, w2, h, rows=R, colsum=db1s, colsum_group_stride=4 * C,
+                                                      grouped=grouped, w_group_stride=4 * C * C, packed=packs['w2_t'])
     dw2s = torch.zeros((G, C, 4 * C), device=dev, dtype=torch.float32)
     ops.linear_wgrad(d_o, None, dw2s, rows=R, segs=segs, num_groups=G, x_packed=a_mn)
     del a_mn
diff --git a/sm3det_b200/ops.py b/sm3det_b200/ops.py
--- a/sm3det_b200/ops.py
+++ b/sm3det_b200/ops.py
@@ -8,6 +8,7 @@
 
 SCHED_DENSE, SCHED_GROUPED, SCHED_SPLITK = 0, 1, 2
 EPI_BIAS, EPI_GELU, EPI_DGELU, EPI_COLSCALE, EPI_ROWSCALE, EPI_RESID, EPI_ATOMIC, EPI_AUXSTORE, EPI_COLSUM = 1, 2, 4, 8, 16, 32, 64, 128, 256
+EPI_PACK_K, EPI_PACK_MN = 512, 1024
 LN_NHWC, LN_PATCH2, LN_NCHW = 0, 1, 2
 
 
@@ -91,12 +92,12 @@
     return torch.cuda.get_device_properties(torch.cuda.current_device()).multi_processor_count
 
 
-def gemm(*, A, a_smn, a_sk, B, b_smn, b_sk, M, N, K, D, ldd, b_group_stride=0, a_row_index=None, b_k_index=None,
-         sched=SCHED_DENSE, k_splits=1, num_groups=1, tile_group=None, num_m_tiles=None, seg_begin=None,
-         seg_end=None, d_group_stride=0, bias=None, bias_group_stride=0, epilogue=0, aux_out=None, aux_in=None,
-         ld_aux=0, col_scale=None, row_scale=None, resid=None, ld_resid=0, tile_n=0, b_packed=None,
-         b_packed_group_stride=0, colsum=None, colsum_group_stride=0, a_packed=None):
-    lib = _lib.load()
+def _gemm_args(*, A, a_smn, a_sk, B, b_smn, b_sk, M, N, K, D, ldd, b_group_stride=0, a_row_index=None, b_k_index=None,
+               sched=SCHED_DENSE, k_splits=1, num_groups=1, tile_group=None, num_m_tiles=None, seg_begin=None,
+               seg_end=None, d_group_stride=0, bias=None, bias_group_stride=0, epilogue=0, aux_out=None, aux_in=None,
+               ld_aux=0, col_scale=None, row_scale=None, resid=None, ld_resid=0, tile_n=0, b_packed=None,
+               b_packed_group_stride=0, colsum=None, colsum_group_stride=0, a_packed=None, pack_k=None, pack_mn=None,
+               pack_mn2=None):
     a = _lib.GemmArgs()
     a.A = _p(A); a.a_stride_mn = a_smn; a.a_stride_k = a_sk
     a.b_packed = None if b_packed is None else _p(b_packed, torch.int16); a.b_packed_group_stride = b_packed_group_stride
@@ -114,9 +115,22 @@
     a.col_scale = _p(col_scale); a.row_scale = _p(row_scale)
     a.resid = _p(resid); a.ld_resid = ld_resid
     a.colsum = _p(colsum); a.colsum_group_stride = colsum_group_stride
+    a.pack_k, a.pack_mn, a.pack_mn2 = (None if t is None else _p(t, torch.int16) for t in (pack_k, pack_mn, pack_mn2))
     a.mma_passes = current_passes()
-    _lib.check(lib.sm3_gemm(C.byref(a), _stream()), 'sm3_gemm')
-    return D
+    return a
+
+
+def gemm(**kw):
+    _lib.check(_lib.load().sm3_gemm(C.byref(_gemm_args(**kw)), _stream()), 'sm3_gemm')
+    return kw['D']
+
+
+def gemm_pack(*, pack_k, pack_mn=None, pack_mn2=None, **kw):
+    if not kw.get('epilogue', 0) & (EPI_PACK_K | EPI_PACK_MN):
+        raise ValueError('gemm_pack: the epilogue must include EPI_PACK_K or EPI_PACK_MN')
+    a = _gemm_args(D=None, pack_k=pack_k, pack_mn=pack_mn, pack_mn2=pack_mn2, **kw)
+    _lib.check(_lib.load().sm3_gemm(C.byref(a), _stream()), 'sm3_gemm(pack)')
+    return pack_k, pack_mn, pack_mn2
 
 
 def pack_weight(w, *, transposed: bool, groups: int = 1, out=None, tile: int = 0):
@@ -298,6 +312,38 @@
          epilogue=epilogue | (EPI_COLSUM if colsum is not None else 0), aux_in=aux_in, ld_aux=K, row_scale=row_scale,
          resid=resid, ld_resid=K, colsum=colsum, colsum_group_stride=colsum_group_stride, **kw)
     return out
+
+
+def linear_gelu_packed(x, w, bias, *, rows=None, row_index=None, grouped=None, w_group_stride=0, bias_group_stride=0,
+                       packed, want_h=True):
+    K, N = w.shape[-1], w.shape[-2]
+    M = rows if rows is not None else x.shape[0]
+    h = torch.empty((M, N), device=w.device, dtype=torch.float32) if want_h else None
+    a_k = torch.empty((_lib.load().sm3_gemm_packed_act_elems(M, N, 0, 128),), device=w.device, dtype=torch.int16)
+    kw = {} if grouped is None else dict(sched=SCHED_GROUPED, tile_group=grouped[0], num_m_tiles=grouped[1])
+    gemm_pack(A=None, a_smn=K, a_sk=1, B=None, b_smn=K, b_sk=1, b_group_stride=w_group_stride, M=M, N=N, K=K, ldd=N,
+              bias=bias, bias_group_stride=bias_group_stride, epilogue=EPI_BIAS | EPI_GELU | EPI_PACK_K, aux_out=h, ld_aux=N,
+              b_packed=packed[0], b_packed_group_stride=packed[1],
+              a_packed=pack_act(x, rows=M, cols=K, mn_major=False, row_index=row_index), pack_k=a_k, **kw)
+    return h, a_k
+
+
+def linear_dgrad_dgelu_packed(dy, w, h, *, rows=None, row_scale=None, colsum, colsum_group_stride=0, grouped=None,
+                              w_group_stride=0, packed):
+    K, N = w.shape[-1], w.shape[-2]
+    M = rows if rows is not None else dy.shape[0]
+    lib = _lib.load()
+    dev = w.device
+    dh_k = torch.empty((lib.sm3_gemm_packed_act_elems(M, K, 0, 128),), device=dev, dtype=torch.int16)
+    dh_mn = torch.empty((lib.sm3_gemm_packed_act_elems(M, K, 1, 128),), device=dev, dtype=torch.int16)
+    a_mn = torch.empty((lib.sm3_gemm_packed_act_elems(M, K, 1, _pick_bn(K)),), device=dev, dtype=torch.int16)
+    kw = {} if grouped is None else dict(sched=SCHED_GROUPED, tile_group=grouped[0], num_m_tiles=grouped[1])
+    epi = EPI_DGELU | EPI_COLSUM | EPI_PACK_K | EPI_PACK_MN | (EPI_ROWSCALE if row_scale is not None else 0)
+    gemm_pack(A=None, a_smn=N, a_sk=1, B=None, b_smn=1, b_sk=K, b_group_stride=w_group_stride, M=M, N=K, K=N, ldd=K,
+              epilogue=epi, aux_in=h, ld_aux=K, row_scale=row_scale, colsum=colsum, colsum_group_stride=colsum_group_stride,
+              b_packed=packed[0], b_packed_group_stride=packed[1], a_packed=pack_act(dy, rows=M, cols=N, mn_major=False),
+              pack_k=dh_k, pack_mn=dh_mn, pack_mn2=a_mn, **kw)
+    return dh_k, dh_mn, a_mn
 
 
 def linear_wgrad(dy, x, dw, *, rows=None, x_row_index=None, row_scale=None, segs=None, num_groups=1, dy_packed=None,
```

New measurement: 105.3 (median of 6 runs). 1.2% higher.
